# ku222/Attention-GAN

Hardware: AMD Instinct MI355X
Metric: train images/sec at 256×256 stage-3, batch 24/GPU, 1/2/4/8 MI355X (higher is better)
Workload: dtype f32; 1 GPU; full 3-stage AttnGAN 64->128->256 train step: G + 3xD updates + word attention + DAMSM words/sentence loss + KL + 4x fused Adam (BASELINE.json configs[2]); workload_key=full3, batch_per_gpu=24, global_batch=24, gf_dim=32, df_dim=64, emb_dim=256, seq_len=10, text_encoder=bypassed (frozen; N(0,1) embeddings), parallelism=dp1, discriminator_streams=3, launch=eager, gradient_exchange=none (one rank), losses_finite=True

## Files before the change

### attention-gan_amd/backend/functional.py

```python
from __future__ import annotations

import ctypes
import math
from ctypes import byref, c_void_p
from typing import Dict, Optional, Tuple

import contextlib
import os
import weakref

import torch
from torch import Tensor
from torch.autograd import Function
from torch.autograd.function import once_differentiable

from . import lib as L

_PRECISION = [L.PREC_F32]


def set_precision(p: int) -> None:
    if int(p) != _PRECISION[0]:
        for rng in _FLAT_RANGES:
            rng[3], rng[4] = [], None
# ... 35 lines not shown
def set_activation_storage(kind) -> None:
    dt = {None: L.DT_F32, "f32": L.DT_F32, "bf16": L.DT_BF16, "f16": L.DT_F16}[kind]
    _STORAGE[0] = dt


def get_activation_storage() -> int:
    dt = _STORAGE[0]
    if dt == L.DT_BF16 and _PRECISION[0] == L.PREC_BF16:
        return dt
    if dt == L.DT_F16 and _PRECISION[0] == L.PREC_F16:
        return dt
    return L.DT_F32


def _dt(t: Tensor) -> int:
    return L.DT_F32 if t.dtype == torch.float32 else _DT_OF[t.dtype]


def _act(t: Tensor, what: str) -> Tensor:
    if not t.is_cuda:
        raise L.AganError(f"{what}: tensor is on {t.device}; the AttnGAN HIP path runs on an MI355X only (no CPU fallback)")
    if t.dtype != torch.float32 and t.dtype not in _DT_OF:
        raise L.AganError(f"{what}: expected float32 / bfloat16 / float16, got {t.dtype}")
    return t.contiguous()


_DT_SUPPORT: dict = {}


def _gather_types(g: "L.ConvGeom", pe: int, x: Tensor, want_out: int):
    def ok(xin, out):
        if xin == L.DT_F32 and out == L.DT_F32:
            return True
        key = (g.B, g.Cin, g.IH, g.IW, g.Cout, g.OH, g.OW, g.R, g.S, g.OS, g.SY, g.DY, g.OY[0], g.OY[1], pe, xin, out)
        hit = _DT_SUPPORT.get(key)
        if hit is None:
            hit = _DT_SUPPORT[key] = bool(L.load().agan_conv_gather_dt_supported(byref(g), pe, xin, out))
        return hit
    outs = [want_out, L.DT_F32] if want_out != L.DT_F32 else [L.DT_F32]
    for out in outs:
        if ok(_dt(x), out):
            return x, out
    x = x.float()
    for out in outs:
        if ok(L.DT_F32, out):
            return x, out
    return x, L.DT_F32


def _ws(nbytes: int, like: Tensor) -> Tuple[Optional[Tensor], Optional[c_void_p]]:
    if nbytes <= 0:
        return None, None
    t = torch.empty(nbytes, dtype=torch.uint8, device=like.device)
    return t, c_void_p(t.data_ptr())


def grad_dst(param):
    return getattr(param, "_agan_grad_dst", None)


def _grad_out(dst, shape, like: Tensor):
    if dst is None:
        t = torch.empty(shape, dtype=torch.float32, device=like.device)
        return t, 0, t
    if dst.locked:
        raise L.AganError("a backward kernel is about to write into a flat gradient slice whose bucket is already being all-reduced: "
                          "call zero_grad() (and GradBuckets.arm()) before running another backward under data parallelism")
    view = dst.flat[dst.offset:dst.offset + dst.numel].view(shape)
    dst.edges += 1
    if dst.written:
        return view, 1, None
    dst.written = True
    return view, 0, view


class GradDst:
    __slots__ = ("flat", "offset", "numel", "written", "edges", "locked")

    def __init__(self, flat: Tensor, offset: int, numel: int):
        self.flat, self.offset, self.numel, self.written, self.edges, self.locked = flat, offset, numel, False, 0, False

    def reset(self) -> None:
        self.written, self.edges, self.locked = False, 0, False


def _geom(B, Cin, IH, IW, Cout, OH, OW, R, S, OS, SY, DY, OY) -> L.ConvGeom:
    g = L.ConvGeom()
    g.B, g.Cin, g.IH, g.IW, g.Cout, g.OH, g.OW = B, Cin, IH, IW, Cout, OH, OW
    g.R, g.S, g.OS, g.SY, g.DY = R, S, OS, SY, DY
    g.OY[0], g.OY[1] = OY
    return g


_GEOM_CACHE = {}


def conv_geoms(kind: str, B: int, Cin: int, H: int, W: int, Cout: int, k: int):
    key = (kind, B, Cin, H, W, Cout, k)
    hit = _GEOM_CACHE.get(key)
    if hit is not None:
        return hit
    if kind == "same":
        p = (k - 1) // 2
        out = (_geom(B, Cin, H, W, Cout, H, W, k, k, 1, 1, 1, (-p, -p)), L.PACK_FWD,
               _geom(B, Cout, H, W, Cin, H, W, k, k, 1, 1, 1, (-p, -p)), L.PACK_DGRAD_S1, (H, W))
    elif kind == "down":
        if k != 4 or H % 2 or W % 2:
            raise L.AganError(f"down conv needs k=4 and even H,W (got k={k}, {H}x{W})")
        out = (_geom(B, Cin, H, W, Cout, H // 2, W // 2, 4, 4, 1, 2, 1, (-1, -1)), L.PACK_FWD,
               _geom(B, Cout, H // 2, W // 2, Cin, H, W, 2, 2, 2, 1, -1, (0, 1)), L.PACK_DGRAD_4x4S2, (H // 2, W // 2))
    elif kind == "up":
        if k != 3:
            raise L.AganError("upsample conv needs k=3")
        out = (_geom(B, Cin, H, W, Cout, 2 * H, 2 * W, 2, 2, 2, 1, 1, (-1, 0)), L.PACK_UP_FWD,
               _geom(B, Cout, 2 * H, 2 * W, Cin, H, W, 4, 4, 1, 2, 1, (-1, -1)), L.PACK_UP_DGRAD, (2 * H, 2 * W))
    else:
        raise L.AganError(f"unknown conv kind {kind!r}")
    _GEOM_CACHE[key] = out
    return out


_WEIGHT_EPOCH = [0]
_FLAT_RANGES: list = []


def bump_weight_epoch() -> None:
    _WEIGHT_EPOCH[0] += 1


def register_flat(flat: Tensor) -> None:
    start = flat.data_ptr()
    end = start + flat.numel() * flat.element_size()
    top = max([r[2] for r in _FLAT_RANGES] + [0])
    _FLAT_RANGES[:] = [r for r in _FLAT_RANGES if r[1] <= start or r[0] >= end]
    _FLAT_RANGES.append([start, end, top + 1, [], None])


def unregister_flat(flat: Tensor) -> None:
    start = flat.data_ptr()
    _FLAT_RANGES[:] = [r for r in _FLAT_RANGES if r[0] != start]


def _flat_range(ptr: int):
    for r in _FLAT_RANGES:
        if r[0] <= ptr < r[1]:
            return r
    return None


_PACK_JOB_DTYPE = [("w", "<u8"), ("wk", "<u8"), ("mode", "<i4"), ("cout", "<i4"), ("cin", "<i4"), ("kh", "<i4"), ("kw", "<i4"),
                   ("first_block", "<i4")]


def _pack_table(rng, prec: int):
    import numpy as np
    entries = [e for e in rng[3] if e["prec"] == prec]
    if rng[4] is None:
        rng[4] = {}
    hit = rng[4].get(prec)
    if hit is None or hit[1] != len(entries):
        if torch.cuda.is_current_stream_capturing():
            raise L.AganError("packed-weight job table missing during HIP-graph capture: run a warm-up step and "
                              "build_pack_tables() first (GanTrainStep.capture does)")
        lib = L.load()
        jobs = np.zeros(len(entries), dtype=_PACK_JOB_DTYPE)
        first = 0
        for i, e in enumerate(entries):
            cout, cin, kh, kw = e["dims"]
            jobs[i] = (e["ptr"], e["wk"].data_ptr(), e["mode"], cout, cin, kh, kw, first)
            first += lib.agan_pack_job_blocks_prec(e["mode"], cout, cin, kh, kw, prec)
        table = torch.from_numpy(jobs.view(np.uint8).copy()).to(entries[0]["wk"].device)
        hit = rng[4][prec] = (table, len(entries), first)
    return hit


def build_pack_tables() -> None:
    for rng in _FLAT_RANGES:
        for prec in sorted({e["prec"] for e in rng[3]}):
            _pack_table(rng, prec)


def _repack_group(rng, prec: int) -> None:
    table, n, total = _pack_table(rng, prec)
    L.call("agan_pack_weights", _p(table), n, total, prec, _stream())
    for e in rng[3]:
        if e["prec"] == prec:
            e["cache"][e["key"]] = ((e["ptr"], e["tver"], _WEIGHT_EPOCH[0], rng[2]) + e["dims"], e["wk"], rng)


_EFF_PREC = {}


def effective_precision(g: L.ConvGeom) -> int:
    prec = _PRECISION[0]
    if prec == L.PREC_F32:
        return prec
    key = (prec, g.B, g.Cin, g.IH, g.IW, g.Cout, g.OH, g.OW, g.R, g.S, g.OS, g.SY, g.DY, g.OY[0], g.OY[1])
    hit = _EFF_PREC.get(key)
    if hit is None:
        hit = _EFF_PREC[key] = int(L.load().agan_conv_effective_prec(byref(g), prec))
    return hit


_EFF_WPREC = {}


def wgrad_effective_precision(g: L.ConvGeom, pack_mode: int) -> int:
    prec = _PRECISION[0]
    if prec == L.PREC_F32:
        return prec
    key = (prec, pack_mode, g.B, g.Cin, g.IH, g.IW, g.Cout, g.OH, g.OW, g.R, g.S, g.OS, g.SY, g.DY, g.OY[0], g.OY[1])
    hit = _EFF_WPREC.get(key)
    if hit is None:
        hit = _EFF_WPREC[key] = int(L.load().agan_conv_wgrad_effective_prec(byref(g), pack_mode, prec))
    return hit


def packed_weight(w: Tensor, mode: int, cache: Optional[dict] = None, prec: Optional[int] = None) -> Tensor:
    cout, cin, kh, kw = w.shape
    if prec is None:
        prec = _PRECISION[0]
    key = (mode, prec)
    hit = cache.get(key) if cache is not None else None
    ptr = w.data_ptr()
    rng = hit[2] if (hit is not None and hit[0][0] == ptr) else _flat_range(ptr)
    ver = (ptr, w._version, _WEIGHT_EPOCH[0], rng[2] if rng is not None else -1, cout, cin, kh, kw)
    if hit is not None and hit[0] == ver:
        return hit[1]
    if hit is not None and rng is not None and hit[0][:2] == ver[:2] and hit[0][4:] == ver[4:] \
            and any(e["cache"] is cache and e["key"] == key for e in rng[3]):
        _repack_group(rng, prec)
        hit = cache[key]
        if hit[0] == ver:
            return hit[1]
    n = L.load().agan_packed_weight_bytes(mode, cout, cin, kh, kw, prec)
    if n == 0:
        raise L.AganError(f"pack mode {mode} / precision {prec} does not take a {kh}x{kw} kernel")
    reuse = hit is not None and hit[1].numel() == n and hit[1].device == w.device
    wk = hit[1] if reuse else torch.empty(n, dtype=torch.uint8, device=w.device)
    L.call("agan_pack_weight", _p(w), _p(wk), mode, cout, cin, kh, kw, prec, _stream())
    if cache is not None:
        cache[key] = (ver, wk, rng)
        if rng is not None:
            ent = next((e for e in rng[3] if e["cache"] is cache and e["key"] == key), None)
            if ent is None:
                ent = {"cache": cache, "key": key}
                rng[3].append(ent)
            ent.update(ptr=ptr, tver=w._version, dims=(cout, cin, kh, kw), mode=mode, wk=wk, prec=prec)
            rng[4] = None
    return wk


_KTABLE_CACHE = {}


def ktable(g: L.ConvGeom, device) -> Tensor:
    key = (g.Cin, g.IH, g.IW, g.R, g.S, g.DY, str(device))
    t = _KTABLE_CACHE.get(key)
    if t is None:
        n = L.load().agan_conv_ktable_elems(byref(g))
        t = torch.empty(n, dtype=torch.int32, device=device)
        L.call("agan_conv_ktable", byref(g), _p(t), _stream())
        _KTABLE_CACHE[key] = t
    return t


_OBSERVER = [None]


def set_launch_observer(obs) -> None:
    _OBSERVER[0] = obs


_AMAX_REG: dict = {}
_AMAX_ARENA: dict = {}
_AMAX_WINDOW, _AMAX_WINDOWS = 1024, 4


def _needs_amax() -> bool:
    return _PRECISION[0] in (L.PREC_F16X3, L.PREC_BF16X6)


def amax_begin_step(device) -> None:
    if not _needs_amax():
        return
    ent = _AMAX_ARENA.get(device)
    if ent is None:
        ent = _AMAX_ARENA[device] = [torch.zeros(_AMAX_WINDOWS * _AMAX_WINDOW * L.AMAX_SLOT, dtype=torch.float32, device=device), -1, 0, 0]
    ent[1] = (ent[1] + 1) % _AMAX_WINDOWS
    lo = ent[1] * _AMAX_WINDOW * L.AMAX_SLOT
    ent[0][lo:lo + _AMAX_WINDOW * L.AMAX_SLOT].zero_()
    ent[2], ent[3] = ent[1] * _AMAX_WINDOW, (ent[1] + 1) * _AMAX_WINDOW


def _amax_new(device) -> Tensor:
    ent = _AMAX_ARENA.get(device)
    if ent is not None and ent[2] < ent[3]:
        i = ent[2]
        ent[2] += 1
        return ent[0][i * L.AMAX_SLOT:(i + 1) * L.AMAX_SLOT]
    return torch.zeros(L.AMAX_SLOT, dtype=torch.float32, device=device)


def _amax_put(t: Tensor, slot: Tensor) -> None:
    k = id(t)
    _AMAX_REG[k] = (weakref.ref(t, lambda _r, k=k: _AMAX_REG.pop(k, None)), slot)


def amax_of(t: Tensor) -> Tensor:
    e = _AMAX_REG.get(id(t))
    if e is not None and e[0]() is t:
        return e[1]
    slot = _amax_new(t.device)
    L.call("agan_absmax", _p(t), t.numel(), _p(slot), _stream())
    _amax_put(t, slot)
    return slot


_AMAX_FUSE_MIN = int(os.environ.get("AGAN_AMAX_FUSE_MIN", 1 << 22))


def _amax_out(t: Tensor) -> Optional[Tensor]:
    if not _needs_amax() or t.numel() < _AMAX_FUSE_MIN:
        return None
    slot = _amax_new(t.device)
    _amax_put(t, slot)
    return slot


def _gather(x: Tensor, wk: Tensor, bias: Optional[Tensor], g: L.ConvGeom, out: Tensor, kind: str = "", phase: str = "",
            act: int = 0, lrelu_mask: Optional[Tensor] = None, prec: int = L.PREC_F32, in_amax: Optional[Tensor] = None) -> None:
    lib = L.load()
    nbytes = lib.agan_conv_gather_ws_bytes(byref(g), prec)
    ws, wsp = _ws(nbytes, x)
    kt = ktable(g, x.device)
    obs = _OBSERVER[0]
    if obs is not None:
        obs.begin(kind, phase, g, x.element_size(), out.element_size())
    out_amax = _amax_out(out) if prec != L.PREC_F32 else None
    L.call("agan_conv_gather_dt", _p(x), _p(wk), _p(bias), _p(out), byref(g), _p(kt), prec, act, _p(lrelu_mask), wsp, nbytes,
           _stream(), _p(in_amax), _p(out_amax), _dt(x), _dt(out))
    if obs is not None:
        obs.end()


_SIDE_STREAMS: Dict[int, "torch.cuda.Stream"] = {}
_SIDE_DIRTY: Dict[int, bool] = {}
_WGRAD_SIDE = [False]


def set_wgrad_side_stream(flag: bool) -> bool:
    old = _WGRAD_SIDE[0]
    _WGRAD_SIDE[0] = bool(flag)
    return old


def wgrad_side_stream_enabled() -> bool:
    return _WGRAD_SIDE[0]


def join_all_side_streams(target) -> None:
    for key, side in _SIDE_STREAMS.items():
        if _SIDE_DIRTY.get(key):
            target.wait_stream(side)


def set_side_stream_for(stream, side) -> None:
    _SIDE_STREAMS[stream.cuda_stream] = side


def _fork_side_stream():
    cur = torch.cuda.current_stream()
    key = cur.cuda_stream
    side = _SIDE_STREAMS.get(key)
    if side is None:
        side = _SIDE_STREAMS[key] = torch.cuda.Stream(device=cur.device)
    side.wait_stream(cur)
    _SIDE_DIRTY[key] = True
    return side


def join_side_stream() -> None:
    if not torch.cuda.is_available():
        return
    cur = torch.cuda.current_stream()
    key = cur.cuda_stream
    if _SIDE_DIRTY.get(key):
        cur.wait_stream(_SIDE_STREAMS[key])
        _SIDE_DIRTY[key] = False


class ActHandoff:
    __slots__ = ("masked",)

    def __init__(self):
        self.masked = False


class _ConvFn(Function):
    @staticmethod
    def forward(ctx, x: Tensor, weight: Tensor, bias: Optional[Tensor], kind: str, cache: Optional[dict], wdst, bdst, act: int = 0,
                handoff_out: Optional[ActHandoff] = None, handoff_in: Optional[ActHandoff] = None):
        x = _act(x, "conv input")
        w = _dev(weight.detach(), "conv weight")
        B, Cin, H, W = x.shape
        Cout, Cin_w, kh, kw = w.shape
        if Cin != Cin_w or kh != kw:
            raise L.AganError(f"conv: input has {Cin} channels, weight {tuple(w.shape)}")
        gf, pf, gd, pd, (OH, OW) = conv_geoms(kind, B, Cin, H, W, Cout, kh)
        pe = effective_precision(gf)
        x, odt = _gather_types(gf, pe, x, get_activation_storage())
        out = torch.empty((B, Cout, OH, OW), dtype=_TORCH_OF[odt], device=x.device)
        b = _dev(bias.detach(), "conv bias") if bias is not None else None
        need_xs = pe == L.PREC_F16X3 or (ctx.needs_input_grad[1] and _needs_amax() and wgrad_effective_precision(gf, pf) == L.PREC_F16X3)
        xs = amax_of(x) if need_xs else None
        _gather(x, packed_weight(w, pf, cache, pe), b, gf, out, kind, "fwd", act, None, pe, xs)
        ctx.x_scale = xs
        if act == L.ACT_NONE:
            ctx.save_for_backward(x, w)
        else:
            ctx.save_for_backward(x, w, out)
        ctx.kind, ctx.has_bias, ctx.cache, ctx.wdst, ctx.bdst, ctx.act = kind, bias is not None, cache, wdst, bdst, act
        ctx.handoff_out = handoff_out if act != L.ACT_NONE else None
        ctx.handoff_in = handoff_in if (handoff_in is not None and Cin > 4) else None
        return out

    @staticmethod
    @once_differentiable
    def backward(ctx, dy: Tensor):
        x, w = ctx.saved_tensors[:2]
        dy = _act(dy, "conv grad")
        if ctx.act != L.ACT_NONE:
            if ctx.handoff_out is not None and ctx.handoff_out.masked:
                ctx.handoff_out.masked = False
            else:
                out = _dev(ctx.saved_tensors[2], "conv output")
                dy = _dev(dy, "conv grad")
                dz = torch.empty_like(dy)
                L.call("agan_act_bwd", _p(out), _p(dy), _p(dz), out.numel(), ctx.act, _stream())
                dy = dz
        B, Cin, H, W = x.shape
        Cout, _, kh, kw = w.shape
        gf, pf, gd, pd, _ = conv_geoms(ctx.kind, B, Cin, H, W, Cout, kh)
        dx = dw = db = None
        want_w, want_b = ctx.needs_input_grad[1], ctx.has_bias and ctx.needs_input_grad[2]
        pe_d = effective_precision(gd) if ctx.needs_input_grad[0] else L.PREC_F32
        pe_w = wgrad_effective_precision(gf, pf)
        scaled_w = want_w and pe_w == L.PREC_F16X3
        dys = amax_of(dy) if (pe_d == L.PREC_F16X3 or scaled_w) else None
        side = None
        if _WGRAD_SIDE[0] and want_w and ctx.wdst is not None and (not want_b or ctx.bdst is not None):
            kt = ktable(gf, x.device)
            side = _fork_side_stream()
            x.record_stream(side)
            dy.record_stream(side)
        with (torch.cuda.stream(side) if side is not None else contextlib.nullcontext()):
            if want_w:
                dwbuf, wacc, dw = _grad_out(ctx.wdst, w.shape, x)
                lib = L.load()
                nbytes = lib.agan_conv_wgrad_ws_bytes(byref(gf))
                ws, wsp = _ws(nbytes, x)
                kt = ktable(gf, x.device)
                obs = _OBSERVER[0]
                if obs is not None:
                    obs.begin(ctx.kind, "wgrad", gf, x.element_size(), dy.element_size())
                xs = None
                if scaled_w:
                    xs = ctx.x_scale if ctx.x_scale is not None else amax_of(x)
                xw, dyw = x, dy
                if (xw.dtype != torch.float32 or dyw.dtype != torch.float32) and not lib.agan_conv_wgrad_dt_supported(
                        byref(gf), pf, _PRECISION[0], _dt(xw), _dt(dyw)):
                    xw, dyw = xw.float(), dyw.float()
                L.call("agan_conv_wgrad_dt", _p(xw), _p(dyw), _p(dwbuf), byref(gf), _p(kt), pf, kh, kw, pe_w, wacc, wsp, nbytes,
                       _stream(), _p(xs), _p(dys if scaled_w else None), _dt(xw), _dt(dyw))
                if obs is not None:
                    obs.end()
            if want_b:
                dbbuf, bacc, db = _grad_out(ctx.bdst, (Cout,), x)
                L.call("agan_bias_grad", _p(_dev(dy, "conv grad")), _p(dbbuf), B, Cout, dy.shape[2] * dy.shape[3], bacc, _stream())
        if ctx.needs_input_grad[0]:
            dyg, ddt = _gather_types(gd, pe_d, dy, _dt(x))
            dx = torch.empty(x.shape, dtype=_TORCH_OF[ddt], device=x.device)
            mask = x if ctx.handoff_in is not None else None
            if mask is not None and mask.dtype != dx.dtype:
                mask = mask.to(dx.dtype)
            _gather(dyg, packed_weight(w, pd, ctx.cache, pe_d), None, gd, dx, ctx.kind, "dgrad", L.ACT_NONE, mask, pe_d,
                    dys if pe_d == L.PREC_F16X3 else None)
            if mask is not None:
                ctx.handoff_in.masked = True
        return dx, dw, db, None, None, None, None, None, None, None


_ANY_DESCS = {}


def conv_any_desc(B: int, Cin: int, H: int, W: int, Cout: int, k, stride, padding):
    key = (B, Cin, H, W, Cout, tuple(k), tuple(stride), tuple(padding))
    hit = _ANY_DESCS.get(key)
    if hit is not None:
        return hit
    (kh, kw), (sh, sw), (ph, pw) = k, stride, padding
    oh, ow = (H + 2 * ph - kh) // sh + 1, (W + 2 * pw - kw) // sw + 1
    d = L.Conv2dDesc(B, Cin, H, W, Cout, oh, ow, kh, kw, sh, sw, ph, pw, 0, Cin, 0, Cout)
    lib = L.load()
    if not lib.agan_conv2d_train_supported(byref(d)):
        raise L.AganError(f"conv k={k} s={stride} p={padding} on {Cin}x{H}x{W}: {lib.agan_last_error().decode()}")
    g = _geom(B, Cin, H, W, Cout, oh, ow, kh, kw, 1, sh, 1, (-ph, -pw))
    hit = _ANY_DESCS[key] = (d, g, tuple(lib.agan_conv2d_train_ws_bytes(byref(d), i) for i in range(3)))
    return hit


class _ConvAnyFn(Function):

    @staticmethod
    def forward(ctx, x: Tensor, weight: Tensor, bias: Optional[Tensor], stride, padding, wdst, bdst):
        ctx.x_dtype = x.dtype
        x = _dev(x, "conv input")
        w = _dev(weight.detach(), "conv weight")
        B, Cin, H, W = x.shape
        Cout, Cin_w, kh, kw = w.shape
        if Cin != Cin_w:
            raise L.AganError(f"conv: input has {Cin} channels, weight {tuple(w.shape)}")
        d, g, nbytes = conv_any_desc(B, Cin, H, W, Cout, (kh, kw), stride, padding)
        b = _dev(bias.detach(), "conv bias") if bias is not None else None
        out = torch.empty((B, Cout, d.OH, d.OW), dtype=torch.float32, device=x.device)
        ws, wsp = _ws(nbytes[0], x)
        obs = _OBSERVER[0]
        if obs is not None:
            obs.begin("any", "fwd", g, 4, 4)
        L.call("agan_conv2d_train_fwd", _p(x), _p(w), _p(b), _p(out), byref(d), wsp, nbytes[0], _stream())
        if obs is not None:
            obs.end()
        ctx.save_for_backward(x, w)
        ctx.stride, ctx.padding, ctx.has_bias, ctx.wdst, ctx.bdst = stride, padding, bias is not None, wdst, bdst
        return out

    @staticmethod
    @once_differentiable
    def backward(ctx, dy: Tensor):
        x, w = ctx.saved_tensors
        dy = _dev(dy, "conv grad")
        B, Cin, H, W = x.shape
        Cout, _, kh, kw = w.shape
        d, g, nbytes = conv_any_desc(B, Cin, H, W, Cout, (kh, kw), ctx.stride, ctx.padding)
        dx = dw = db = None
        want_w, want_b = ctx.needs_input_grad[1], ctx.has_bias and ctx.needs_input_grad[2]
        obs = _OBSERVER[0]
        side = None
        if _WGRAD_SIDE[0] and want_w and ctx.wdst is not None and (not want_b or ctx.bdst is not None):
            side = _fork_side_stream()
            x.record_stream(side)
            dy.record_stream(side)
        with (torch.cuda.stream(side) if side is not None else contextlib.nullcontext()):
            if want_w:
                dwbuf, wacc, dw = _grad_out(ctx.wdst, w.shape, x)
                ws, wsp = _ws(nbytes[2], x)
                if obs is not None:
                    obs.begin("any", "wgrad", g, 4, 4)
                L.call("agan_conv2d_train_wgrad", _p(x), _p(dy), _p(dwbuf), byref(d), wacc, wsp, nbytes[2], _stream())
                if obs is not None:
                    obs.end()
            if want_b:
                dbbuf, bacc, db = _grad_out(ctx.bdst, (Cout,), x)
                L.call("agan_bias_grad", _p(dy), _p(dbbuf), B, Cout, dy.shape[2] * dy.shape[3], bacc, _stream())
        if ctx.needs_input_grad[0]:
            dx = torch.empty(x.shape, dtype=torch.float32, device=x.device)
            ws, wsp = _ws(nbytes[1], x)
            if obs is not None:
                obs.begin("any", "dgrad", g, 4, 4)
            L.call("agan_conv2d_train_dgrad", _p(dy), _p(w), _p(dx), byref(d), 0, wsp, nbytes[1], _stream())
            if obs is not None:
                obs.end()
            if ctx.x_dtype != torch.float32:
                dx = dx.to(ctx.x_dtype)
        return dx, dw, db, None, None, None, None


def conv_fuses_activation(act: int, cout: int, kind: Optional[str] = None) -> bool:
    return act == L.ACT_LRELU and cout > 4 and kind != "any"


def conv2d(x: Tensor, weight: Tensor, bias: Optional[Tensor] = None, kind: str = "same", cache: Optional[dict] = None,
           wdst=None, bdst=None, act: int = 0, handoff_out: Optional[ActHandoff] = None,
           handoff_in: Optional[ActHandoff] = None, stride=(1, 1), padding=(0, 0)) -> Tensor:
    if kind == "any":
        if act != L.ACT_NONE or handoff_out is not None:
            raise L.AganError("conv2d(kind='any') has no fused activation: run HF.activation / HF.bn_act after it")
        return _ConvAnyFn.apply(x, weight, bias, tuple(stride), tuple(padding), wdst, bdst)
    return _ConvFn.apply(x, weight, bias, kind, cache, wdst, bdst, act, handoff_out, handoff_in)


def linear(x: Tensor, weight: Tensor, bias: Optional[Tensor] = None, cache: Optional[dict] = None, wdst=None, bdst=None) -> Tensor:
    B, Cin = x.shape
    y = _ConvFn.apply(x.reshape(B, Cin, 1, 1), weight.view(weight.shape[0], Cin, 1, 1), bias, "same", cache, wdst, bdst)
    return y.view(B, weight.shape[0])


_BN_GROUPS = [1]


@contextlib.contextmanager
def bn_groups(groups: int):
    old = _BN_GROUPS[0]
    _BN_GROUPS[0] = int(groups)
    try:
        yield
    finally:
        _BN_GROUPS[0] = old


class _BnActFn(Function):
    @staticmethod
    def forward(ctx, x, gamma, beta, residual, running_mean, running_var, nbt, training, act, eps, momentum, gdst, bdst, groups):
        x = _act(x, "bn input")
        shape = x.shape
        B, C = shape[0], shape[1]
        HW = x.numel() // (B * C)
        if not training:
            groups = 1
        if B % groups:
            raise L.AganError(f"BatchNorm: batch {B} does not split into {groups} groups")
        Bg = B // groups
        g, b = _dev(gamma.detach(), "bn weight"), _dev(beta.detach(), "bn bias")
        lib = L.load()
        co = C // 2 if act == L.ACT_GLU else C
        odt = get_activation_storage() if HW > 1 else L.DT_F32
        if x.dtype != torch.float32 and _dt(x) != odt:
            x = x.float()
        xdt = _dt(x)
        out = torch.empty((B, co) + tuple(shape[2:]), dtype=_TORCH_OF[odt], device=x.device)
        res = _act(residual, "bn residual") if residual is not None else None
        if res is not None and res.dtype != out.dtype:
            res = res.to(out.dtype)
        if training:
            mean = torch.empty((groups, C), dtype=torch.float32, device=x.device)
            invstd = torch.empty_like(mean)
            nbytes = lib.agan_bn_train_fwd_ws_bytes(Bg, C, HW)
            ws, wsp = _ws(nbytes, x)
            L.call("agan_bn_train_fwd_dt", _p(x), _p(g), _p(b), _p(res), _p(out), _p(mean), _p(invstd), _p(running_mean),
                   _p(running_var), _p(nbt), B, C, HW, float(eps), float(momentum), act, groups, wsp, nbytes, _stream(),
# ... 1191 lines not shown
```

### attention-gan_amd/backend/lib.py

```python
from __future__ import annotations

import ctypes
import os
from ctypes import POINTER, Structure, c_char_p, c_double, c_float, c_int, c_int32, c_int64, c_size_t, c_void_p

_HERE = os.path.dirname(os.path.abspath(__file__))
LIB_PATH = os.environ.get("AGAN_LIB") or os.path.join(os.path.dirname(_HERE), "csrc", "libagan_hip.so")

PREC_F32, PREC_BF16, PREC_BF16X3, PREC_F16, PREC_BF16X6, PREC_F16X3 = 0, 1, 2, 3, 4, 5
PRECISIONS = {"f32": PREC_F32, "bf16": PREC_BF16, "bf16x3": PREC_BF16X3, "f16": PREC_F16, "bf16x6": PREC_BF16X6, "f16x3": PREC_F16X3}
PACK_FWD, PACK_DGRAD_S1, PACK_DGRAD_4x4S2, PACK_UP_FWD, PACK_UP_DGRAD, PACK_DGRAD_3x3S2 = 0, 1, 2, 3, 4, 5
ACT_NONE, ACT_GLU, ACT_LRELU, ACT_TANH, ACT_SIGMOID, ACT_RELU = 0, 1, 2, 3, 4, 5
COMM_ID_BYTES = 128
DT_F32, DT_BF16, DT_F16 = 0, 1, 2
AMAX_SLOT = 256
EINVAL, EWORKSPACE = -1, -2
DIFFAUG_COLOR, DIFFAUG_TRANSLATION, DIFFAUG_CUTOUT = 1, 2, 4
ADA_STATE_WORDS, ADA_P_WORD, ADA_SLOT_WORD = 16, 4, 8
ABI_VERSION = 101


class ConvGeom(Structure):
    _fields_ = [("B", c_int32), ("Cin", c_int32), ("IH", c_int32), ("IW", c_int32),
                ("Cout", c_int32), ("OH", c_int32), ("OW", c_int32), ("R", c_int32), ("S", c_int32),
                ("OS", c_int32), ("SY", c_int32), ("DY", c_int32), ("OY", c_int32 * 2)]


class Conv2dDesc(Structure):
    _fields_ = [(n, c_int32) for n in ("B", "Cin", "IH", "IW", "Cout", "OH", "OW", "KH", "KW", "SH", "SW", "PH", "PW",
                                       "in_c0", "in_ctot", "out_c0", "out_ctot")]


class ImagePlane(Structure):
    _fields_ = [("src", c_void_p), ("dst", c_void_p), ("H", c_int32), ("W", c_int32)]


_P = c_void_p
_SIGNATURES = {
    "agan_version": (c_int, []),
    "agan_last_error": (c_char_p, []),
    "agan_packed_weight_bytes": (c_size_t, [c_int] * 6),
    "agan_timer_create": (c_int, [_P]),
    "agan_timer_destroy": (c_int, [_P]),
    "agan_timer_arm": (c_int, [_P, _P]),
    "agan_timer_elapsed_ms": (c_int, [_P, _P, _P]),
    "agan_timer_last_kernel": (c_int, [_P, c_size_t]),
    "agan_timer_last_split": (c_int, []),
    "agan_comm_unique_id": (c_int, [_P]),
    "agan_comm_init": (c_int, [_P, c_int, c_int, _P]),
    "agan_comm_destroy": (c_int, [_P]),
    "agan_allreduce_bucket": (c_int, [_P, _P, c_size_t, _P]),
    "agan_allreduce_chunk_elems": (c_size_t, [c_size_t, c_int]),
    "agan_allreduce_scratch_bytes": (c_size_t, [c_size_t, c_int, c_int]),
    "agan_allreduce_bucket_dt": (c_int, [_P, _P, c_size_t, c_int, _P, c_size_t, _P]),
    "agan_exchange_wire_elems": (c_size_t, [c_size_t, c_int]),
    "agan_exchange_pack_bf16": (c_int, [_P, _P, c_size_t, c_size_t, _P]),
    "agan_exchange_sum_bf16": (c_int, [_P, c_int, c_size_t, _P, _P]),
    "agan_exchange_unpack_bf16": (c_int, [_P, _P, c_size_t, _P]),
    "agan_pack_job_blocks": (c_int, [c_int] * 5),
    "agan_pack_job_blocks_prec": (c_int, [c_int] * 6),
    "agan_pack_weights": (c_int, [_P, c_int, c_int, c_int, _P]),
    "agan_pack_weight": (c_int, [_P, _P, c_int, c_int, c_int, c_int, c_int, c_int, _P]),
    "agan_conv_effective_prec": (c_int, [POINTER(ConvGeom), c_int]),
    "agan_conv_wgrad_effective_prec": (c_int, [POINTER(ConvGeom), c_int, c_int]),
    "agan_conv_executed_fraction": (c_double, [POINTER(ConvGeom), c_int, c_int, c_int]),
    "agan_conv_gather_ws_bytes": (c_size_t, [POINTER(ConvGeom), c_int]),
    "agan_conv_ktable_elems": (c_size_t, [POINTER(ConvGeom)]),
    "agan_conv_ktable": (c_int, [POINTER(ConvGeom), _P, _P]),
    "agan_conv_gather": (c_int, [_P, _P, _P, _P, POINTER(ConvGeom), _P, c_int, c_int, _P, _P, c_size_t, _P, _P, _P]),
    "agan_conv_gather_dt": (c_int, [_P, _P, _P, _P, POINTER(ConvGeom), _P, c_int, c_int, _P, _P, c_size_t, _P, _P, _P, c_int, c_int]),
    "agan_conv_gather_dt_supported": (c_int, [POINTER(ConvGeom), c_int, c_int, c_int]),
    "agan_conv_wgrad_dt_supported": (c_int, [POINTER(ConvGeom), c_int, c_int, c_int, c_int]),
    "agan_conv_wgrad_dt": (c_int, [_P, _P, _P, POINTER(ConvGeom), _P, c_int, c_int, c_int, c_int, c_int, _P, c_size_t, _P, _P, _P, c_int, c_int]),
    "agan_bn_stats_dt": (c_int, [_P, c_int, c_int, c_int, c_float, _P, _P, _P, _P, _P, c_float, _P, c_size_t, _P, c_int]),
    "agan_bn_act_fwd_dt": (c_int, [_P, _P, _P, _P, _P, _P, _P, c_int, c_int, c_int, c_int, _P, _P, c_int, c_int]),
    "agan_bn_train_fwd_dt": (c_int, [_P, _P, _P, _P, _P, _P, _P, _P, _P, _P, c_int, c_int, c_int, c_float, c_float, c_int, c_int, _P, c_size_t, _P, _P, c_int, c_int]),
    "agan_bn_act_bwd_dt": (c_int, [_P, _P, _P, _P, _P, _P, _P, _P, _P, c_int, c_int, c_int, c_int, c_int, c_int, _P, c_size_t, _P, _P, c_int, c_int]),
    "agan_absmax": (c_int, [_P, c_size_t, _P, _P]),
    "agan_conv_wgrad_ws_bytes": (c_size_t, [POINTER(ConvGeom)]),
    "agan_conv_wgrad": (c_int, [_P, _P, _P, POINTER(ConvGeom), _P, c_int, c_int, c_int, c_int, c_int, _P, c_size_t, _P, _P, _P]),
    "agan_bias_grad": (c_int, [_P, _P, c_int, c_int, c_int, c_int, _P]),
    "agan_bn_stats_ws_bytes": (c_size_t, [c_int, c_int, c_int]),
    "agan_bn_stats": (c_int, [_P, c_int, c_int, c_int, c_float, _P, _P, _P, _P, _P, c_float, _P, c_size_t, _P]),
    "agan_bn_train_fwd_ws_bytes": (c_size_t, [c_int, c_int, c_int]),
    "agan_bn_train_fwd": (c_int, [_P] * 10 + [c_int, c_int, c_int, c_float, c_float, c_int, c_int, _P, c_size_t, _P, _P]),
    "agan_bn_act_fwd": (c_int, [_P, _P, _P, _P, _P, _P, _P, c_int, c_int, c_int, c_int, _P, _P]),
    "agan_bn_act_bwd_ws_bytes": (c_size_t, [c_int, c_int, c_int]),
    "agan_bn_act_bwd": (c_int, [_P] * 9 + [c_int, c_int, c_int, c_int, c_int, c_int, _P, c_size_t, _P, _P]),
    "agan_act_fwd": (c_int, [_P, _P, c_size_t, c_int, _P]),
    "agan_act_bwd": (c_int, [_P, _P, _P, c_size_t, c_int, _P]),
    "agan_glu_fwd": (c_int, [_P, _P, c_int, c_int, c_int, _P]),
    "agan_glu_bwd": (c_int, [_P, _P, _P, c_int, c_int, c_int, _P]),
    "agan_bn_last_launch": (c_int, [_P, c_int]),
    "agan_attn_fwd": (c_int, [_P, _P, _P, _P, c_float, _P, _P, _P, c_int, c_int, c_int, c_int, c_int, _P]),
    "agan_attn_bwd_ws_bytes": (c_size_t, [c_int, c_int, c_int, c_int]),
    "agan_attn_bwd": (c_int, [_P] * 7 + [c_float, _P, _P, _P, c_int, c_int, c_int, c_int, c_int, c_int, _P, c_size_t, _P]),
    "agan_attn_fwd_dt": (c_int, [_P, _P, _P, _P, c_float, _P, _P, _P, c_int, c_int, c_int, c_int, c_int, _P, c_int]),
    "agan_attn_bwd_dt": (c_int, [_P] * 7 + [c_float, _P, _P, _P, c_int, c_int, c_int, c_int, c_int, c_int, _P, c_size_t, _P, c_int]),
    "agan_func_attention_fwd": (c_int, [_P, _P, c_float, c_float, _P, _P, c_int, c_int, c_int, c_int, _P]),
    "agan_func_attention_bwd": (c_int, [_P, _P, _P, _P, c_float, c_float, _P, _P, c_int, c_int, c_int, c_int, _P]),
    "agan_words_loss_save_elems": (c_size_t, [c_int, c_int, c_int, c_int]),
    "agan_words_loss_fwd": (c_int, [_P, _P, _P, _P, _P, c_float, c_float, c_float, c_float, _P, _P, _P, _P, c_int, c_int, c_int, c_int, _P]),
    "agan_words_loss_bwd_ws_bytes": (c_size_t, [c_int, c_int, c_int, c_int]),
    "agan_words_loss_bwd": (c_int, [_P, _P, _P, _P, _P, c_float, c_float, c_float, c_float, _P, _P, c_int, c_int, c_int, c_int, _P, c_size_t, _P]),
    "agan_sent_loss_fwd": (c_int, [_P, _P, _P, _P, c_float, c_float, c_float, _P, _P, c_int, c_int, _P]),
    "agan_sent_loss_bwd": (c_int, [_P, _P, _P, _P, c_float, c_float, c_float, _P, _P, c_int, c_int, _P]),
    "agan_disc_loss": (c_int, [_P, _P, _P, _P, _P, c_int, _P]),
    "agan_gen_loss": (c_int, [_P, _P, _P, c_int, _P]),
    "agan_kl_loss": (c_int, [_P, _P, _P, _P, _P, c_int, _P]),
    "agan_reparam_fwd": (c_int, [_P, _P, _P, _P, c_int, _P]),
    "agan_reparam_bwd": (c_int, [_P, _P, _P, _P, _P, c_int, _P]),
    "agan_conv2d_pack_mode": (c_int, [POINTER(Conv2dDesc), c_int]),
    "agan_conv2d_effective_prec": (c_int, [POINTER(Conv2dDesc), c_int]),
    "agan_conv2d_ws_bytes": (c_size_t, [POINTER(Conv2dDesc), c_int]),
    "agan_conv2d_ktable_elems": (c_size_t, [POINTER(Conv2dDesc), c_int]),
    "agan_conv2d_ktable": (c_int, [POINTER(Conv2dDesc), c_int, _P, _P]),
    "agan_conv2d_fwd": (c_int, [_P, _P, _P, _P, POINTER(Conv2dDesc), _P, c_int, _P, c_size_t, _P]),
    "agan_conv2d_dgrad": (c_int, [_P, _P, _P, POINTER(Conv2dDesc), _P, _P, c_int, _P, c_size_t, _P]),
    "agan_conv2d_train_supported": (c_int, [POINTER(Conv2dDesc)]),
    "agan_conv2d_train_slabs": (c_int, [POINTER(Conv2dDesc)]),
    "agan_conv2d_train_ws_bytes": (c_size_t, [POINTER(Conv2dDesc), c_int]),
    "agan_conv2d_train_fwd": (c_int, [_P, _P, _P, _P, POINTER(Conv2dDesc), _P, c_size_t, _P]),
    "agan_conv2d_train_dgrad": (c_int, [_P, _P, _P, POINTER(Conv2dDesc), c_int, _P, c_size_t, _P]),
    "agan_conv2d_train_wgrad": (c_int, [_P, _P, _P, POINTER(Conv2dDesc), c_int, _P, c_size_t, _P]),
    "agan_maxpool3s2_fwd": (c_int, [_P, _P, _P] + [c_int] * 6 + [_P]),
    "agan_maxpool3s2_bwd": (c_int, [_P, _P, _P, _P] + [c_int] * 7 + [_P]),
    "agan_avgpool3s1_fwd": (c_int, [_P, _P] + [c_int] * 4 + [_P]),
    "agan_avgpool3s1_bwd": (c_int, [_P, _P, _P] + [c_int] * 5 + [_P]),
    "agan_global_avgpool_fwd": (c_int, [_P, _P] + [c_int] * 3 + [_P]),
    "agan_global_avgpool_bwd": (c_int, [_P, _P, _P] + [c_int] * 4 + [_P]),
    "agan_resize_bilinear_fwd": (c_int, [_P, _P] + [c_int] * 6 + [_P]),
    "agan_resize_bilinear_bwd": (c_int, [_P, _P] + [c_int] * 6 + [_P]),
    "agan_relu_bwd": (c_int, [_P, _P, _P, c_size_t, c_int, _P]),
    "agan_bn_relu_slice_fwd_ws_bytes": (c_size_t, [c_int] * 3),
    "agan_bn_relu_slice_fwd": (c_int, [_P] * 4 + [c_int] * 2 + [_P] * 5 + [c_int] * 3 + [c_float] * 2 + [_P, c_size_t, _P]),
    "agan_bn_slice_bwd_ws_bytes": (c_size_t, [c_int] * 3),
    "agan_bn_slice_bwd": (c_int, [_P, _P, c_int, c_int, _P, _P, _P, _P] + [c_int] * 3 + [_P, c_size_t, _P]),
    "agan_embedding_fwd": (c_int, [_P, c_int, _P, _P] + [c_int] * 4 + [_P]),
    "agan_embedding_bwd": (c_int, [_P, c_int, _P, _P] + [c_int] * 4 + [_P]),
    "agan_lstm_fwd": (c_int, [_P] * 11 + [c_int] * 4 + [_P]),
    "agan_lstm_bwd": (c_int, [_P] * 9 + [c_int] * 4 + [_P]),
    "agan_lstm_wgrad": (c_int, [_P] * 5 + [c_int] * 4 + [_P]),
    "agan_image_prep": (c_int, [POINTER(ImagePlane), c_int, _P, _P, c_int, c_int, c_int, _P]),
    "agan_kmeans_assign_ws_bytes": (c_size_t, [c_int] * 3),
    "agan_kmeans_assign": (c_int, [_P] * 6 + [c_int] * 3 + [_P, c_size_t, _P]),
    "agan_kmeans_update_ws_bytes": (c_size_t, [c_int] * 3),
    "agan_kmeans_update": (c_int, [_P] * 4 + [c_int] * 3 + [_P, c_size_t, _P]),
    "agan_moments_update_ws_bytes": (c_size_t, [c_int] * 2),
    "agan_moments_update": (c_int, [_P, c_int, c_int, _P, _P, _P, c_size_t, _P]),
    "agan_moments_finish": (c_int, [_P, _P, c_int64, c_int, _P, _P, _P]),
    "agan_retrieval_rank": (c_int, [_P, _P, _P] + [c_int] * 4 + [_P, _P, _P]),
    "agan_diffaug_ws_bytes": (c_size_t, [c_int] * 4),
    "agan_diffaug_fwd": (c_int, [_P, _P, c_int, c_int, _P, c_int, _P, c_int, c_int, c_int, _P, c_size_t, _P]),
    "agan_diffaug_bwd": (c_int, [_P, _P, c_int, _P, c_int, c_int, c_int, c_int, _P, c_size_t, _P]),
    "agan_diffaug_gated_fwd": (c_int, [_P, _P, c_int, c_int, _P, _P, _P, c_int, _P, c_int, c_int, c_int, _P, c_size_t, _P]),
    "agan_diffaug_gated_bwd": (c_int, [_P, _P, _P, _P, c_int, _P, c_int, c_int, c_int, c_int, _P, c_size_t, _P]),
    "agan_ada_observe": (c_int, [_P, c_int, c_float, _P, _P]),
    "agan_ada_update": (c_int, [_P, c_int, c_int, c_double, c_double, c_double, _P]),
    "agan_ema_plan": (c_int, [_P, c_int]),
    "agan_ema_update": (c_int, [_P, c_int, c_int, _P, c_double, c_int, _P]),
    "agan_adam_step": (c_int, [_P, _P, _P, _P, c_size_t, _P, c_double, c_double, c_double, c_double, c_float, _P]),
    "agan_knn_radius_ws_bytes": (c_size_t, [c_int] * 3),
    "agan_knn_radius": (c_int, [_P, c_int, c_int, c_int, _P, _P, c_size_t, _P]),
    "agan_manifold_scan_ws_bytes": (c_size_t, [c_int] * 3),
    "agan_manifold_scan": (c_int, [_P, _P, _P] + [c_int] * 3 + [_P, _P, _P, _P, c_size_t, _P]),
    "agan_poly_kernel_sum_ws_bytes": (c_size_t, [c_int] * 3),
    "agan_poly_kernel_sum": (c_int, [_P, _P] + [c_int] * 4 + [_P, _P, c_size_t, _P]),
}

EXPORTED_SYMBOLS = tuple(_SIGNATURES)

_lib = None


class AganError(RuntimeError):
    pass


def load():
    global _lib
    if _lib is not None:
        return _lib
    if not os.path.exists(LIB_PATH):
        raise AganError(f"{LIB_PATH} not found: build it with `python -c 'import __graft_entry__ as g; g.build()'` "
                        f"(or `make -C attention-gan_amd/csrc`). There is no CPU fallback.")
    lib = ctypes.CDLL(LIB_PATH)
    for name, (res, args) in _SIGNATURES.items():
        fn = getattr(lib, name)
        fn.restype, fn.argtypes = res, args
    if lib.agan_version() != ABI_VERSION:
        raise AganError(f"{LIB_PATH} reports C-ABI version {lib.agan_version()}, this binding is written against {ABI_VERSION} "
                        f"(include/agan.h: argument lists differ between versions) -- rebuild with `make -C attention-gan_amd/csrc`")
    _lib = lib
    return lib


def check(code: int, what: str = "") -> None:
    if code != 0:
        msg = load().agan_last_error()
        raise AganError(f"{what or 'agan'} failed ({code}): {msg.decode() if msg else ''}")


def call(name: str, *args) -> None:
    check(getattr(load(), name)(*args), name)
```

### attention-gan_amd/csrc/conv.hip

```cpp
#include "conv_common.h"

#include <cxxabi.h>
#include <cstdlib>


using namespace agan;

using namespace agan::conv;

namespace {

__global__ __launch_bounds__(256) void ktable_kernel(int2* __restrict__ tab, int n, int K, int RS, int S, int IHW, int IW, int DY) {
    const int k = blockIdx.x * 256 + threadIdx.x;
    if (k >= n) return;
    int2 a, b;
    if (k < K) {
        const int c = k / RS, rs = k - c * RS, r = rs / S, q = rs - r * S;
        const int dy = r * DY, dx = q * DY;
        a.x = c * IHW + dy * IW + dx;
        a.y = (dy & 0xFFFF) | (dx << 16);
        b.x = c * IHW * 4;
        b.y = rs * kTapRowBytes;
    } else {
        a.x = 0;
// ... 505 lines not shown
#pragma unroll
        for (int t = 0; t < TI; ++t) av[0][t] = Xs[buf][wi * (BI / 2) + t * 32 + pl][half];
#pragma unroll
        for (int t = 0; t < TJ; ++t) bv[0][t] = Ys[buf][wj * (BJ / 2) + t * 32 + pl][half];
#pragma unroll
        for (int pp = 0; pp < BP; pp += 2) {
            const int c = (pp >> 1) & 1, q = pp >> 1;
            if (pp + 2 < BP) {
#pragma unroll
                for (int t = 0; t < TI; ++t) av[c ^ 1][t] = Xs[buf][wi * (BI / 2) + t * 32 + pl][pp + 2 + half];
#pragma unroll
                for (int t = 0; t < TJ; ++t) bv[c ^ 1][t] = Ys[buf][wj * (BJ / 2) + t * 32 + pl][pp + 2 + half];
            }
#pragma unroll
            for (int a = 0; a < TJ; ++a)
#pragma unroll
                for (int b = 0; b < TI; ++b)
                    acc[a][b] = __builtin_amdgcn_mfma_f32_32x32x2f32(bv[c][a], av[c][b], acc[a][b], 0, 0, 0);
#pragma unroll
            for (int it = q * L / NS; it < (q + 1) * L / NS; ++it) {
                if (it < XR) {
                    if (do_store) Xs[buf ^ 1][wave * (BI / 4) + 2 * it + half][pl] = xreg[PN][it];
                    if (do_load) xreg[PC][it] = buf_load(rx, xo[it]);
                } else {
                    const int jj = it - XR;
                    if (do_store) Ys[buf ^ 1][wave * (BJ / 4) + 2 * jj + half][pl] = yreg[PN][jj];
                    if (do_load) yreg[PC][jj] = buf_load(rdy, doff + ynoff[jj]);
                }
            }
        }
        __syncthreads();
    };

    fill_offsets(0);
    fill_offsets(1);
    __syncthreads();
    if (npt > 0) load_tile(S0{}, 0);
    if (npt > 1) load_tile(S1{}, 1);
    __syncthreads();
    fill_offsets(2);
    if (npt > 0) store_tile(S0{}, 0);
    __syncthreads();
    int pt = 0;
    for (; pt + 3 < npt; pt += 2) {
        step(std::true_type{}, S0{}, S1{}, pt, 0);
        step(std::true_type{}, S1{}, S0{}, pt + 1, 1);
    }
    for (; pt < npt; pt += 2) {
        step(std::false_type{}, S0{}, S1{}, pt, 0);
        if (pt + 1 < npt) step(std::false_type{}, S1{}, S0{}, pt + 1, 1);
    }

    float* o = dst + (size_t)split * slab + (size_t)cls * g.Cout * g.K;
    const __amdgpu_buffer_rsrc_t ro = make_rsrc(o, (size_t)g.Cout * g.K * sizeof(float));
#pragma unroll
    for (int tj = 0; tj < TJ; ++tj)
#pragma unroll
        for (int ti = 0; ti < TI; ++ti) {
            const int i = i0 + wi * (BI / 2) + ti * 32 + pl;
#pragma unroll
            for (int r = 0; r < 16; ++r) {
                const int n = j0 + wj * (BJ / 2) + tj * 32 + (r & 3) + 8 * (r >> 2) + 4 * half;
                const unsigned off = ((i < g.K) & (n < g.Cout)) ? (unsigned)(n * g.K + i) * 4u : kOOB;
                float v = acc[tj][ti][r];
                if (accumulate) v += buf_load(ro, off);
                buf_store(ro, off, v);
            }
        }
}

__device__ __forceinline__ void pack_fwd_tile(const float* __restrict__ w, float* __restrict__ wk, int cout, int K, int Nld, int bx, int by,
                                              float (*tile)[65]) {
    const int k0 = bx * 64, n0 = by * 64;
    const int tx = threadIdx.x & 63, ty = threadIdx.x >> 6;
    float v[16];
#pragma unroll
    for (int j = 0; j < 16; ++j) {
        const int n = n0 + ty + j * 4, k = k0 + tx;
        v[j] = (n < cout && k < K) ? w[(size_t)n * K + k] : 0.f;
    }
#pragma unroll
    for (int j = 0; j < 16; ++j) tile[ty + j * 4][tx] = v[j];
    __syncthreads();
#pragma unroll
    for (int j = 0; j < 16; ++j) {
        const int k = k0 + ty + j * 4, n = n0 + tx;
        if (k < K && n < Nld) wk[(size_t)k * Nld + n] = tile[tx][ty + j * 4];
    }
}
__global__ __launch_bounds__(256) void pack_fwd_tiled_kernel(const float* __restrict__ w, float* __restrict__ wk, int cout, int K, int Nld) {
    __shared__ float tile[64][65];
    pack_fwd_tile(w, wk, cout, K, Nld, blockIdx.x, blockIdx.y, tile);
}

constexpr int kPackCo = 4;
constexpr int kPackSlab = 64 * 16 + 64;
template <int MODE>
__device__ __forceinline__ void pack_dgrad_tile(const float* __restrict__ w, float* __restrict__ wk, int cout, int cin, int kh, int kw, int Nld,
                                                int cog, int cblk, float* sl , bool zero_pad) {
    const int T = kh * kw;
    const int c0 = cblk * 64;
    const int nc = min(64, cin - c0);
#pragma unroll
    for (int q = 0; q < kPackCo; ++q) {
        const int co = cog * kPackCo + q;
        if (co < cout) {
            const float* src = w + ((size_t)co * cin + c0) * T;
            for (int i = threadIdx.x; i < nc * T; i += 256) sl[q * kPackSlab + (i / T) * (T + 1) + (i % T)] = src[i];
        }
    }
    __syncthreads();
    const int cend = (zero_pad && c0 + 64 >= cin) ? Nld - c0 : nc;
#pragma unroll
    for (int q = 0; q < kPackCo; ++q) {
        const int co = cog * kPackCo + q;
        if (co >= cout) break;
        const float* s1 = sl + q * kPackSlab;
        if (MODE == AGAN_PACK_DGRAD_S1) {
            for (int i = threadIdx.x; i < T * 64; i += 256) {
                const int t = i / 64, c = i - t * 64;
                if (c < cend) wk[((size_t)co * T + t) * Nld + c0 + c] = c < nc ? s1[c * (T + 1) + (T - 1 - t)] : 0.f;
            }
        } else {
            const int K = cout * 4;
            for (int i = threadIdx.x; i < 16 * 64; i += 256) {
                const int qq = i / 64, c = i - qq * 64;
                const int cls = qq >> 2, r = (qq >> 1) & 1, sx = qq & 1, py = cls >> 1, px = cls & 1;
                const int th = ((py + 1) & 1) + 2 * r, tw = ((px + 1) & 1) + 2 * sx;
                if (c < cend) wk[((size_t)cls * K + co * 4 + r * 2 + sx) * Nld + c0 + c] = c < nc ? s1[c * 17 + th * 4 + tw] : 0.f;
            }
        }
    }
}
template <int MODE>
__global__ __launch_bounds__(256) void pack_dgrad_tiled_kernel(const float* __restrict__ w, float* __restrict__ wk, int cout, int cin,
                                                               int kh, int kw, int Nld) {
    __shared__ float sl[kPackCo * kPackSlab];
    pack_dgrad_tile<MODE>(w, wk, cout, cin, kh, kw, Nld, blockIdx.x, blockIdx.y, sl, false);
}

__global__ __launch_bounds__(256) void pack_weight_kernel(const float* __restrict__ w, float* __restrict__ wk, int mode,
                                                          int cout, int cin, int kh, int kw, int K, int Nld, int ncls) {
    const size_t total = (size_t)ncls * K * Nld;
    for (size_t e = (size_t)blockIdx.x * blockDim.x + threadIdx.x; e < total; e += (size_t)gridDim.x * blockDim.x) {
        const int n = (int)(e % Nld);
        const size_t t = e / Nld;
        const int k = (int)(t % K), cls = (int)(t / K);
        wk[e] = packed_weight_value(w, mode, cls, k, n, cout, cin, kh, kw);
    }
}

__host__ __device__ inline int pack_job_blocks(int mode, int cout, int cin, int kh, int kw) {
    int ncls, K, N;
    if (pack_dims(mode, cout, cin, kh, kw, ncls, K, N)) return 0;
    const int Nld = ((N + 31) / 32 * 32);
    if (mode == AGAN_PACK_FWD) return cdiv(K, 64) * cdiv(Nld, 64);
    if ((mode == AGAN_PACK_DGRAD_S1 && kh * kw <= 16) || mode == AGAN_PACK_DGRAD_4x4S2) return cdiv(cout, kPackCo) * cdiv(cin, 64);
    const size_t total = (size_t)ncls * K * Nld;
    return (int)(total / 1024 < 1 ? 1 : (total / 1024 > 2048 ? 2048 : total / 1024));
}

__global__ __launch_bounds__(256) void pack_jobs_kernel(const agan_pack_job* __restrict__ jobs, int njobs) {
    __shared__ float buf[kPackCo * kPackSlab > 64 * 65 ? kPackCo * kPackSlab : 64 * 65];
    __shared__ int which;
    const int b = blockIdx.x;
    for (int t = threadIdx.x; t < njobs; t += 256) {
        const int lo = jobs[t].first_block, hi = t + 1 < njobs ? jobs[t + 1].first_block : 0x7fffffff;
        if (b >= lo && b < hi) which = t;
    }
    __syncthreads();
    const agan_pack_job j = jobs[which];
    const int local = b - j.first_block;
    float* wk = static_cast<float*>(j.wk);
    int ncls, K, N;
    pack_dims(j.mode, j.cout, j.cin, j.kh, j.kw, ncls, K, N);
    const int Nld = ((N + 31) / 32 * 32);
    if (j.mode == AGAN_PACK_FWD) {
        const int kt = cdiv(K, 64);
        pack_fwd_tile(j.w, wk, j.cout, K, Nld, local % kt, local / kt, reinterpret_cast<float (*)[65]>(buf));
    } else if (j.mode == AGAN_PACK_DGRAD_S1 && j.kh * j.kw <= 16) {
        const int cg = cdiv(j.cout, kPackCo);
        pack_dgrad_tile<AGAN_PACK_DGRAD_S1>(j.w, wk, j.cout, j.cin, j.kh, j.kw, Nld, local % cg, local / cg, buf, true);
    } else if (j.mode == AGAN_PACK_DGRAD_4x4S2) {
        const int cg = cdiv(j.cout, kPackCo);
        pack_dgrad_tile<AGAN_PACK_DGRAD_4x4S2>(j.w, wk, j.cout, j.cin, j.kh, j.kw, Nld, local % cg, local / cg, buf, true);
    } else {
        const int nb = pack_job_blocks(j.mode, j.cout, j.cin, j.kh, j.kw);
        const size_t total = (size_t)ncls * K * Nld;
        for (size_t e = (size_t)local * 256 + threadIdx.x; e < total; e += (size_t)nb * 256) {
            const int n = (int)(e % Nld);
            const size_t t = e / Nld;
            wk[e] = packed_weight_value(j.w, j.mode, (int)(t / K), (int)(t % K), n, j.cout, j.cin, j.kh, j.kw);
        }
    }
}

__global__ __launch_bounds__(256) void unpack_wgrad_up_kernel(const float* __restrict__ dwk, float* __restrict__ dw, int cout, int cin,
                                                              int accumulate) {
    const int K = cin * 4;
    const size_t total = (size_t)cout * cin * 9;
    for (size_t e = (size_t)blockIdx.x * blockDim.x + threadIdx.x; e < total; e += (size_t)gridDim.x * blockDim.x) {
        const int ab = (int)(e % 9), a = ab / 3, b = ab - a * 3;
        const size_t t = e / 9;
        const int ci = (int)(t % cin), co = (int)(t / cin);
        float v = 0.f;
        for (int py = 0; py < 2; ++py)
            for (int r = 0; r < 2; ++r) {
                int rl, rh;
                up_fwd_taps(py, r, rl, rh);
                if (a < rl || a > rh) continue;
                for (int px = 0; px < 2; ++px)
                    for (int q = 0; q < 2; ++q) {
                        int sl, sh;
                        up_fwd_taps(px, q, sl, sh);
                        if (b < sl || b > sh) continue;
                        v += dwk[((size_t)(py * 2 + px) * cout + co) * K + (ci * 4 + r * 2 + q)];
                    }
            }
        dw[e] = accumulate ? dw[e] + v : v;
    }
}

__global__ __launch_bounds__(256) void bias_grad_kernel(const float* __restrict__ dy, float* __restrict__ db, int B, int C,
                                                        int HW, int accumulate) {
    __shared__ float red[4];
    const int c = blockIdx.x;
    float s = 0.f;
    for (int b = 0; b < B; ++b) {
        const float* p = dy + ((size_t)b * C + c) * HW;
        for (int i = threadIdx.x; i < HW; i += 256) s += p[i];
    }
    s = block_sum<256>(s, red);
    if (threadIdx.x == 0) db[c] = accumulate ? db[c] + s : s;
}

}

static thread_local hipEvent_t g_timer_start = nullptr, g_timer_stop = nullptr;
static thread_local const void* g_timed_kernel = nullptr;
static thread_local int g_timed_split = 0;
namespace agan { namespace conv { thread_local const void* g_noted_kernel = nullptr; } }
static inline void timer_begin(hipStream_t st) {
    if (g_timer_start) (void)hipEventRecord(g_timer_start, st);
}
static inline void timer_end(hipStream_t st, int split) {
    if (g_timer_stop) {
        (void)hipEventRecord(g_timer_stop, st);
        g_timed_kernel = agan::conv::g_noted_kernel;
        g_timed_split = split;
    }
    g_timer_start = g_timer_stop = nullptr;
}
namespace agan { namespace conv {
void timed_begin(hipStream_t st) { timer_begin(st); }
void timed_end(hipStream_t st, int split) { timer_end(st, split); }
} }

static bool dt16(int dt) { return dt == AGAN_DT_BF16 || dt == AGAN_DT_F16; }
static int mode_dtype(int mode) { return mode == AGAN_PREC_BF16 ? AGAN_DT_BF16 : (mode == AGAN_PREC_F16 ? AGAN_DT_F16 : AGAN_DT_F32); }

enum class GatherPath { none, p16, patch, winograd, small_n, direct };
struct GatherRoute {
    int mode = AGAN_PREC_F32;
    GatherPath path = GatherPath::none;
    P16Plan p16{};
    PatchPlan pp{};
    PatchGather patch{};
    WinoPlan wino{};
    GatherPlan direct{};
    size_t ws_bytes = 0;
    int split = 1;
};

static GatherRoute route_gather(const agan_conv_geom* gg, int prec, int in_dtype, int out_dtype, bool epilogue) {
    GatherRoute r;
    auto take = [&r](GatherPath path, size_t ws_bytes, int split) {
        r.path = path;
        r.ws_bytes = ws_bytes;
        r.split = split;
        return r;
    };
    if (check_geom(gg)) return r;
    const Geom g = make_geom(gg);
    if (prec_planes(prec) > 0 && patch_supported(g)) r.mode = prec;
    const bool f32io = in_dtype == AGAN_DT_F32 && out_dtype == AGAN_DT_F32;
    if (const int want = mode_dtype(r.mode)) {
        if ((in_dtype == AGAN_DT_F32 || in_dtype == want) && (out_dtype == AGAN_DT_F32 || out_dtype == want)) {
            r.p16 = plan_p16(g, in_dtype != AGAN_DT_F32);
            if (r.p16.ok) return take(GatherPath::p16, r.p16.ws_bytes, r.p16.ksplit);
        }
    }
    if (r.mode != AGAN_PREC_F32) {
        if (!f32io) return r;
        r.pp = make_patch_plan(g);
        r.patch = plan_patch_gather(g, r.pp);
        return take(GatherPath::patch, r.patch.ws_bytes, r.patch.ksplit);
    }
    if (f32io && !epilogue) {
        r.wino = plan_wino(g);
        if (r.wino.ok) return take(GatherPath::winograd, r.wino.ws_bytes, r.wino.ksplit);
    }
    if (small_n_gather_supported(g)) {
        const bool linear = g.RS == 1 && g.IH == 1 && g.IW == 1;
        if ((in_dtype == AGAN_DT_F32 || (dt16(in_dtype) && !linear)) && out_dtype == AGAN_DT_F32) return take(GatherPath::small_n, 0, 1);
        return r;
    }
    if (in_dtype == AGAN_DT_F32 && (out_dtype == AGAN_DT_F32 || dt16(out_dtype))) {
        r.direct = plan_gather(g, AGAN_PREC_F32);
        return take(GatherPath::direct, r.direct.ws_bytes, r.direct.ksplit);
    }
    return r;
}

enum class WgradPath { none, winograd, rows, patch, small_n, direct };
struct WgradRoute {
    int mode = AGAN_PREC_F32;
    WgradPath path = WgradPath::none;
    WinoWgradPlan wino{};
    RowsPlan rows{};
    PatchPlan pp{};
    PatchWgrad patch{};
    SmallWgradPlan small{};
    WgradPlan direct{};
    size_t ws_bytes = 0;
    int split = 1;
};

static WgradRoute route_wgrad(const agan_conv_geom* gg, int pack_mode, int prec, int x_dtype, int dy_dtype) {
    WgradRoute r;
    auto take = [&r](WgradPath path, size_t ws_bytes, int split) {
        r.path = path;
        r.ws_bytes = ws_bytes;
        r.split = split;
        return r;
    };
    if (check_geom(gg)) return r;
    const Geom g = make_geom(gg);
    const bool up = pack_mode == AGAN_PACK_UP_FWD, x16 = x_dtype != AGAN_DT_F32, y16 = dy_dtype != AGAN_DT_F32;
    if (prec_planes(prec) > 0 && patch_supported(g)) {
        r.mode = prec;
        if (prec == AGAN_PREC_BF16X6) r.mode = AGAN_PREC_F16X3;
        if (up && !plan_rows_wgrad(g, r.mode, false, false, true).ok) r.mode = AGAN_PREC_F32;
    }
    if (x16 || y16) {
        const int want = mode_dtype(r.mode);
        const bool ok = r.mode == AGAN_PREC_F32
                            ? pack_mode == AGAN_PACK_FWD && small_n_wgrad_supported(g) && dt16(x_dtype) && !y16
                            : want != AGAN_DT_F32 && (!x16 || x_dtype == want) && (!y16 || dy_dtype == want);
        if (!ok) return r;
    }
    if (r.mode == AGAN_PREC_F32 && !up && !x16 && !y16) {
        r.wino = plan_wino_wgrad(g);
        if (r.wino.ok) return take(WgradPath::winograd, r.wino.ws_bytes, r.wino.psplit);
    }
    if (!(r.mode == AGAN_PREC_F32 && small_n_wgrad_supported(g))) {
        r.rows = plan_rows_wgrad(g, r.mode, x16, y16, up);
        if (r.rows.ok) return take(WgradPath::rows, r.rows.ws_bytes, r.rows.psplit);
    }
    if (r.mode != AGAN_PREC_F32) {
        r.pp = make_patch_plan(g);
        r.patch = plan_patch_wgrad(g, r.pp, r.mode);
        return take(WgradPath::patch, r.patch.ws_bytes, r.patch.psplit);
    }
    if (!up && small_n_wgrad_supported(g)) {
        r.small = plan_wgrad_small_n(g);
        return take(WgradPath::small_n, r.small.ws_bytes, r.small.nchunk);
    }
    if (!x16 && !y16) {
        r.direct = plan_wgrad(g, up);
        return take(WgradPath::direct, r.direct.ws_bytes, r.direct.psplit);
    }
    return r;
}

static int check_ws(const char* who, size_t need, const void* ws, size_t ws_bytes) {
    if (need > ws_bytes || (need && !ws)) {
        set_error("%s: workspace %zu < %zu", who, ws_bytes, need);
        return AGAN_EWORKSPACE;
    }
    return AGAN_OK;
}

template <class Launch>
static int launch_main(hipStream_t st, int split, const char* what, Launch&& launch) {
    timer_begin(st);
    launch();
    timer_end(st, split);
    return check_launch(what);
}

extern "C" {

int agan_timer_last_kernel(char* name, size_t capacity) {
    AGAN_REQUIRE(name && capacity > 1, "timer_last_kernel: bad argument");
    name[0] = 0;
    if (!g_timed_kernel) return AGAN_OK;
    const char* mangled = hipKernelNameRefByPtr(g_timed_kernel, nullptr);
    if (!mangled) return AGAN_OK;
    int status = 0;
    char* dem = abi::__cxa_demangle(mangled, nullptr, nullptr, &status);
    const char* src = (status == 0 && dem) ? dem : mangled;
    strncpy(name, src, capacity - 1);
    name[capacity - 1] = 0;
    free(dem);
    return AGAN_OK;
}

int agan_timer_last_split(void) { return g_timed_kernel ? g_timed_split : 0; }

int agan_timer_create(void** event) {
    AGAN_REQUIRE(event != nullptr, "timer_create: null pointer");
    hipEvent_t e;
    if (hipEventCreate(&e) != hipSuccess) {
        set_error("timer_create: hipEventCreate failed");
        return AGAN_ELAUNCH;
    }
    *event = e;
    return AGAN_OK;
}
int agan_timer_destroy(void* event) { return (event && hipEventDestroy(static_cast<hipEvent_t>(event)) != hipSuccess) ? AGAN_ELAUNCH : AGAN_OK; }
int agan_timer_arm(void* start, void* stop) {
    g_timer_start = static_cast<hipEvent_t>(start);
    g_timer_stop = static_cast<hipEvent_t>(stop);
    return AGAN_OK;
}
int agan_timer_elapsed_ms(void* start, void* stop, float* ms) {
    AGAN_REQUIRE(start && stop && ms, "timer_elapsed_ms: null pointer");
    if (hipEventElapsedTime(ms, static_cast<hipEvent_t>(start), static_cast<hipEvent_t>(stop)) != hipSuccess) {
        set_error("timer_elapsed_ms: events not complete");
        return AGAN_ELAUNCH;
    }
    return AGAN_OK;
}

size_t agan_packed_weight_bytes(int mode, int cout, int cin, int kh, int kw, int prec) {
    int ncls, K, N;
    if (pack_dims(mode, cout, cin, kh, kw, ncls, K, N)) return 0;
    if (prec == AGAN_PREC_F32) return (size_t)ncls * K * ((N + 31) / 32 * 32) * sizeof(float);
    if (mode == AGAN_PACK_DGRAD_3x3S2) return 0;
    if (prec_planes(prec) > 0) return patch_packed_weight_bytes(mode, cout, cin, kh, kw, prec);
    return 0;
}

int agan_pack_weight(const float* w, void* wkv, int mode, int cout, int cin, int kh, int kw, int prec, void* stream) {
    int ncls, K, N;
    AGAN_REQUIRE(w && wkv, "pack_weight: null pointer");
    AGAN_REQUIRE(prec == AGAN_PREC_F32 || prec_planes(prec) > 0, "pack_weight: unknown precision mode %d", prec);
    if (prec != AGAN_PREC_F32) {
        AGAN_REQUIRE(mode != AGAN_PACK_DGRAD_3x3S2, "pack_weight: AGAN_PACK_DGRAD_3x3S2 has an fp32 layout only");
        AGAN_REQUIRE(pack_dims(mode, cout, cin, kh, kw, ncls, K, N) == 0, "pack_weight: mode %d does not take %dx%d", mode, kh, kw);
        return pack_weight_patch(w, wkv, mode, cout, cin, kh, kw, prec, as_stream(stream));
    }
    float* wk = static_cast<float*>(wkv);
    AGAN_REQUIRE(pack_dims(mode, cout, cin, kh, kw, ncls, K, N) == 0, "pack_weight: mode %d does not take %dx%d", mode, kh, kw);
    const int Nld = ((N + 31) / 32 * 32);
    const size_t total = (size_t)ncls * K * Nld;
    const int blocks = (int)std::min<size_t>(cdivz(total, 256), 8192);
    hipStream_t pst = as_stream(stream);
    if (mode == AGAN_PACK_FWD) {
        AGAN_LAUNCH(pack_fwd_tiled_kernel, dim3(cdiv(K, 64), cdiv(Nld, 64)), dim3(256), 0, pst, w, wk, cout, K, Nld);
        return check_launch("pack_weight/fwd");
    }
    if ((mode == AGAN_PACK_DGRAD_S1 && kh * kw <= 16) || mode == AGAN_PACK_DGRAD_4x4S2) {
        if (Nld != cin) (void)hipMemsetAsync(wk, 0, total * sizeof(float), pst);
        dim3 grid(cdiv(cout, kPackCo), cdiv(cin, 64));
        if (mode == AGAN_PACK_DGRAD_S1) AGAN_LAUNCH((pack_dgrad_tiled_kernel<AGAN_PACK_DGRAD_S1>), grid, dim3(256), 0, pst, w, wk, cout, cin, kh, kw, Nld);
        else AGAN_LAUNCH((pack_dgrad_tiled_kernel<AGAN_PACK_DGRAD_4x4S2>), grid, dim3(256), 0, pst, w, wk, cout, cin, kh, kw, Nld);
        return check_launch("pack_weight/dgrad");
    }
    AGAN_LAUNCH(pack_weight_kernel, dim3(blocks), dim3(256), 0, as_stream(stream), w, wk, mode, cout, cin, kh, kw, K,
                       Nld, ncls);
    return check_launch("pack_weight");
}

int agan_pack_job_blocks(int mode, int cout, int cin, int kh, int kw) { return pack_job_blocks(mode, cout, cin, kh, kw); }
int agan_pack_job_blocks_prec(int mode, int cout, int cin, int kh, int kw, int prec) {
    return prec == AGAN_PREC_F32 ? pack_job_blocks(mode, cout, cin, kh, kw) : (prec_planes(prec) > 0 ? pack_job_blocks_patch(mode, cout, cin, kh, kw) : 0);
}

int agan_pack_weights(const agan_pack_job* jobs, int njobs, int total_blocks, int prec, void* stream) {
    AGAN_REQUIRE(jobs && njobs > 0 && total_blocks > 0, "pack_weights: empty job list");
    AGAN_REQUIRE(prec == AGAN_PREC_F32 || prec_planes(prec) > 0, "pack_weights: unknown precision mode %d", prec);
    if (prec != AGAN_PREC_F32) return pack_weights_patch(jobs, njobs, total_blocks, prec, as_stream(stream));
    AGAN_LAUNCH(pack_jobs_kernel, dim3(total_blocks), dim3(256), 0, as_stream(stream), jobs, njobs);
    return check_launch("pack_weights");
}

int agan_conv_effective_prec(const agan_conv_geom* g, int prec) { return route_gather(g, prec, AGAN_DT_F32, AGAN_DT_F32, false).mode; }

int agan_conv_wgrad_effective_prec(const agan_conv_geom* g, int pack_mode, int prec) {
    return route_wgrad(g, pack_mode, prec, AGAN_DT_F32, AGAN_DT_F32).mode;
}

double agan_conv_executed_fraction(const agan_conv_geom* g, int prec, int wgrad, int plain_epilogue) {
    if (prec != AGAN_PREC_F32) return 1.0;
    if (wgrad)
        return route_wgrad(g, AGAN_PACK_FWD, prec, AGAN_DT_F32, AGAN_DT_F32).path == WgradPath::winograd ? 16.0 / 36.0 : 1.0;
    const GatherRoute r = route_gather(g, prec, AGAN_DT_F32, AGAN_DT_F32, !plain_epilogue);
    if (r.path != GatherPath::winograd) return 1.0;
    switch (r.wino.kind) {
    case WinoKind::conv4x4_s2: return 36.0 / 64.0;
    case WinoKind::dgrad2x2_class: return 9.0 / 16.0;
    case WinoKind::conv3x3:
    case WinoKind::conv3x3_half: break;
    }
    return 16.0 / 36.0;
}

static const int kDtypes[] = {AGAN_DT_F32, AGAN_DT_BF16, AGAN_DT_F16};

size_t agan_conv_gather_ws_bytes(const agan_conv_geom* g, int prec) {
    size_t a = 0;
    for (int in_dtype : kDtypes)
        for (int out_dtype : kDtypes)
            for (int epilogue = 0; epilogue < 2; ++epilogue) a = std::max(a, route_gather(g, prec, in_dtype, out_dtype, epilogue != 0).ws_bytes);
    return a;
}

size_t agan_conv_ktable_elems(const agan_conv_geom* g) {
    if (check_geom(g)) return 0;
    return (size_t)ktable_entries(g->Cin * g->R * g->S) * 4;
}

int agan_conv_ktable(const agan_conv_geom* gg, int32_t* table, void* stream) {
    if (int e = check_geom(gg)) return e;
    AGAN_REQUIRE(table != nullptr, "conv_ktable: null pointer");
    const Geom g = make_geom(gg);
    const int n = ktable_entries(g.K);
    AGAN_LAUNCH(ktable_kernel, dim3(cdiv(n, 256)), dim3(256), 0, as_stream(stream), reinterpret_cast<int2*>(table), n, g.K, g.RS,
                       g.S, g.IH * g.IW, g.IW, g.DY);
    return check_launch("conv_ktable");
}

int agan_conv_gather_dt_supported(const agan_conv_geom* gg, int prec, int in_dtype, int out_dtype) {
    return route_gather(gg, prec, in_dtype, out_dtype, false).path != GatherPath::none ? 1 : 0;
}

int agan_conv_gather_dt(const void* in_v, const void* wkv, const float* bias, void* out_v, const agan_conv_geom* gg, const int32_t* ktable,
                        int prec, int act, const void* lrelu_mask_v, void* ws, size_t ws_bytes, void* stream, const float* in_scale,
                        float* out_amax, int in_dtype, int out_dtype) {
    if (int e = check_geom(gg)) return e;
    AGAN_REQUIRE(in_v && wkv && out_v && ktable, "conv_gather: null pointer");
    AGAN_REQUIRE(act == AGAN_ACT_NONE || (act == AGAN_ACT_LRELU && gg->Cout > 4),
                 "conv_gather: fused activation %d not available for this call (MFMA paths, LeakyReLU only)", act);
    AGAN_REQUIRE(!lrelu_mask_v || (gg->Cout > 4 && act == AGAN_ACT_NONE),
                 "conv_gather: the LeakyReLU-derivative mask needs an MFMA path and no other activation");
    AGAN_REQUIRE(prec == AGAN_PREC_F32 || prec_planes(prec) > 0, "conv_gather: unknown precision mode %d", prec);
    const GatherRoute r = route_gather(gg, prec, in_dtype, out_dtype, bias || act != AGAN_ACT_NONE || lrelu_mask_v);
    AGAN_REQUIRE(r.mode == prec,
                 "conv_gather: precision mode %d does not take this geometry (agan_conv_effective_prec says which one does)", prec);
    AGAN_REQUIRE(r.path != GatherPath::none,
                 "conv_gather: 16-bit activation storage (%d -> %d) is not available for this geometry / precision %d "
                 "(agan_conv_gather_dt_supported)", in_dtype, out_dtype, prec);
    AGAN_REQUIRE(prec != AGAN_PREC_F16X3 || in_scale != nullptr, "conv_gather: AGAN_PREC_F16X3 needs the operand's agan_absmax_scale pair");
    if (int e = check_ws("conv_gather", r.ws_bytes, ws, ws_bytes)) return e;
    const Geom g = make_geom(gg);
    hipStream_t st = as_stream(stream);
    const float* in = static_cast<const float*>(in_v);
    const float* wk = static_cast<const float*>(wkv);
    const float* lrelu_mask = static_cast<const float*>(lrelu_mask_v);
    void* dst = r.split > 1 ? ws : out_v;
    const float* slabs = static_cast<const float*>(ws);
    size_t slab = 0;
    float* sum_amax = nullptr;
    int e = AGAN_OK;
    switch (r.path) {
        case GatherPath::p16:
            slab = r.p16.slab;
            e = launch_main(st, r.split, "conv_gather/p16", [&] {
                launch_p16_gather(in_v, wkv, bias, dst, g, r.p16, prec, act, lrelu_mask_v, st, in_dtype != AGAN_DT_F32, out_dtype != AGAN_DT_F32);
            });
            break;
        case GatherPath::patch:
            slab = r.patch.slab;
            sum_amax = out_amax;
            e = launch_main(st, r.split, "conv_gather/patch", [&] {
                launch_patch_gather(in, wkv, bias, static_cast<float*>(dst), g, r.pp, r.patch, prec, act, lrelu_mask, st, in_scale, out_amax);
            });
            break;
        case GatherPath::winograd:
            slab = r.wino.slab;
            slabs = reinterpret_cast<const float*>(static_cast<const char*>(ws) + r.wino.u_bytes);
            e = launch_main(st, r.split, "conv_gather/winograd", [&] { launch_wino(in, wk, static_cast<float*>(out_v), g, r.wino, ws, st); });
            break;
        case GatherPath::small_n:
            e = launch_main(st, r.split, "conv_gather/small_n", [&] { launch_gather_small_n(in_v, wk, bias, static_cast<float*>(out_v), g, st, in_dtype); });
            break;
        default: {
            const GatherPlan& p = r.direct;
            slab = p.slab;
            const int2* ktab = reinterpret_cast<const int2*>(ktable);
            e = launch_main(st, r.split, "conv_gather", [&] { launch_gather(in, wk, bias, dst, ktab, g, p, act, lrelu_mask_v, st, out_dtype); });
        }
    }
    if (e || r.split == 1) return e;
    launch_sum_slabs(slabs, r.split, (size_t)g.B * g.Cout * g.OH * g.OW, slab, bias, g.Cout, g.OH * g.OW, out_v, 0, act, lrelu_mask_v, sum_amax, st,
                     out_dtype);
    return check_launch("conv_gather/sum_slabs");
}

int agan_conv_gather(const float* in, const void* wkv, const float* bias, float* out, const agan_conv_geom* gg, const int32_t* ktable,
                     int prec, int act, const float* lrelu_mask, void* ws, size_t ws_bytes, void* stream, const float* in_scale,
                     float* out_amax) {
    return agan_conv_gather_dt(in, wkv, bias, out, gg, ktable, prec, act, lrelu_mask, ws, ws_bytes, stream, in_scale, out_amax,
                               AGAN_DT_F32, AGAN_DT_F32);
}

static const int kPrecs[] = {AGAN_PREC_F32, AGAN_PREC_BF16, AGAN_PREC_BF16X3, AGAN_PREC_F16, AGAN_PREC_BF16X6, AGAN_PREC_F16X3};

size_t agan_conv_wgrad_ws_bytes(const agan_conv_geom* g) {
    if (check_geom(g)) return 0;
    const int pack_mode = g->OS == 2 ? AGAN_PACK_UP_FWD : AGAN_PACK_FWD;
    size_t a = 0;
    for (int prec : kPrecs)
        for (int x_dtype : kDtypes)
            for (int dy_dtype : kDtypes) a = std::max(a, route_wgrad(g, pack_mode, prec, x_dtype, dy_dtype).ws_bytes);
    return a;
}

int agan_conv_wgrad_dt_supported(const agan_conv_geom* gg, int pack_mode, int prec, int x_dtype, int dy_dtype) {
    return route_wgrad(gg, pack_mode, prec, x_dtype, dy_dtype).path != WgradPath::none ? 1 : 0;
}

int agan_conv_wgrad(const float* x, const float* dy, float* dw, const agan_conv_geom* gg, const int32_t* ktable, int pack_mode,
                    int kh, int kw, int prec, int accumulate, void* ws, size_t ws_bytes, void* stream, const float* x_scale,
                    const float* dy_scale) {
    return agan_conv_wgrad_dt(x, dy, dw, gg, ktable, pack_mode, kh, kw, prec, accumulate, ws, ws_bytes, stream, x_scale, dy_scale,
                              AGAN_DT_F32, AGAN_DT_F32);
}

int agan_conv_wgrad_dt(const void* x_v, const void* dy_v, float* dw, const agan_conv_geom* gg, const int32_t* ktable, int pack_mode,
                       int kh, int kw, int prec, int accumulate, void* ws, size_t ws_bytes, void* stream, const float* x_scale,
                       const float* dy_scale, int x_dtype, int dy_dtype) {
    const WgradRoute r = route_wgrad(gg, pack_mode, prec, x_dtype, dy_dtype);
    AGAN_REQUIRE(r.path != WgradPath::none,
                 "conv_wgrad: 16-bit activation storage (%d, %d) is not available for this geometry / precision %d", x_dtype, dy_dtype, prec);
    AGAN_REQUIRE(x_v && dy_v && dw && ktable, "conv_wgrad: null pointer");
    AGAN_REQUIRE(prec == AGAN_PREC_F32 || prec_planes(prec) > 0, "conv_wgrad: unknown precision mode %d", prec);
    AGAN_REQUIRE(pack_mode == AGAN_PACK_FWD || pack_mode == AGAN_PACK_UP_FWD, "conv_wgrad: pack mode %d is not a forward mode", pack_mode);
    const Geom g = make_geom(gg);
    const bool up = pack_mode == AGAN_PACK_UP_FWD;
    AGAN_REQUIRE(1LL * g.B * g.Cin * g.IH * g.IW < (1LL << 29) && 1LL * g.B * g.Cout * g.OH * g.OW < (1LL << 29),
                 "conv_wgrad: tensor exceeds 2^29 elements");
    if (!up) AGAN_REQUIRE(g.R == kh && g.S == kw && g.OS == 1, "conv_wgrad: geometry is not a direct %dx%d conv", kh, kw);
    else AGAN_REQUIRE(g.R == 2 && g.S == 2 && g.OS == 2 && kh == 3 && kw == 3, "conv_wgrad: geometry is not the folded upsample conv");
    AGAN_REQUIRE(r.mode != AGAN_PREC_F16X3 || (x_scale && dy_scale),
                 "conv_wgrad: precision mode %d runs this weight gradient as AGAN_PREC_F16X3 (agan_conv_wgrad_effective_prec), which needs the "
                 "amax slots of x and dy (x_amax / dy_amax)", prec);
    if (int e = check_ws("conv_wgrad", r.ws_bytes, ws, ws_bytes)) return e;
    hipStream_t st = as_stream(stream);
    const float* x = static_cast<const float*>(x_v);
    const float* dy = static_cast<const float*>(dy_v);
    float* wsf = static_cast<float*>(ws);
    const bool x16 = x_dtype != AGAN_DT_F32, y16 = dy_dtype != AGAN_DT_F32;
    switch (r.path) {
        case WgradPath::winograd:
            if (int e = launch_main(st, r.split, "conv_wgrad/winograd", [&] { launch_wino_wgrad(x, dy, wsf, g, r.wino, st); })) return e;
            launch_wino_wgrad_sum(wsf, g, r.wino, dw, accumulate ? 1 : 0, st);
            return check_launch("conv_wgrad/winograd/sum");
        case WgradPath::rows:
        case WgradPath::patch: {
            const bool rows = r.path == WgradPath::rows;
            int e;
            if (rows) e = launch_main(st, r.split, "conv_wgrad/rows", [&] {
                launch_rows_wgrad(x_v, dy_v, wsf, g, r.rows, r.mode, st, x_scale, dy_scale, x16, y16);
            });
            else e = launch_main(st, r.split, "conv_wgrad/patch", [&] {
                launch_patch_wgrad(x_v, dy_v, wsf, g, r.pp, r.patch, r.mode, st, x_scale, dy_scale, x16, y16);
            });
            if (e) return e;
            const size_t slab = rows ? r.rows.slab : r.patch.slab;
            const int NPH = rows ? r.rows.NPH : r.pp.NPH, NT = rows ? r.rows.NT : r.pp.NT, Kp = rows ? r.rows.Kp : r.patch.Kp;
            const int ncls = rows ? 1 : r.patch.ncls;
            const bool unfold = up && !rows;
            float* reduced = r.split > 1 ? wsf + slab * r.split : wsf;
            const bool sum_first = unfold ? r.split > 1 : r.split > 4;
            if (sum_first) {
                launch_sum_slabs(wsf, r.split, (size_t)ncls * g.Cout * Kp, slab, nullptr, 1, 1, reduced, 0, AGAN_ACT_NONE, nullptr, nullptr, st);
                if (int e2 = check_launch("conv_wgrad/sum_slabs")) return e2;
            }
            if (unfold) launch_patch_wgrad_unpack(reduced, dw, g.Cout, g.Cin, kh, kw, up, r.pp, r.patch, accumulate, st);
            else launch_wgrad_sum_unpack(sum_first ? reduced : wsf, sum_first ? 1 : r.split, slab, dw, g.Cout, g.Cin, kh, kw, NPH, NT, Kp, accumulate, st);
            return check_launch("conv_wgrad/unpack");
        }
        case WgradPath::small_n: {
            if (int e = launch_main(st, r.split, "conv_wgrad/small_n", [&] { launch_wgrad_small_n(x_v, dy, wsf, g, r.small, st, x_dtype); })) return e;
            launch_sum_slabs(wsf, r.split, (size_t)g.Cout * g.K, r.small.slab, nullptr, 1, 1, dw, accumulate, AGAN_ACT_NONE, nullptr, nullptr, st);
            return check_launch("conv_wgrad/small_n/sum_slabs");
        }
        default: {
            const WgradPlan& p = r.direct;
            const int acc_in_kernel = (accumulate && !up && p.psplit == 1) ? 1 : 0;
            const bool via_sum = p.psplit > 1 || (accumulate && !up && !acc_in_kernel);
            float* reduced = up ? wsf + (p.psplit > 1 ? p.slab * p.psplit : 0) : dw;
            float* part = via_sum ? wsf : reduced;
            const int2* ktab = reinterpret_cast<const int2*>(ktable);
            dim3 grid(p.itiles, p.jtiles, p.ncls * p.psplit);
            const int e = launch_main(st, r.split, "conv_wgrad", [&] {
                with_bool(p.bi == 128, [&](auto I128) { with_bool(p.bj == 128, [&](auto J128) {
                    AGAN_LAUNCH((conv_wgrad_f32_kernel<I128() ? 128 : 64, J128() ? 128 : 64>), grid, dim3(256), 0, st, x, dy, part, ktab, g, p.psplit, p.pchunk,
                                p.slab, acc_in_kernel);
                }); });
            });
            if (e) return e;
            if (via_sum) {
                launch_sum_slabs(part, p.psplit, (size_t)p.ncls * g.Cout * g.K, p.slab, nullptr, 1, 1, reduced, (accumulate && !up) ? 1 : 0,
                                 AGAN_ACT_NONE, nullptr, nullptr, st);
                if (int e2 = check_launch("conv_wgrad/sum_slabs")) return e2;
            }
            if (up) {
                const size_t total = (size_t)g.Cout * g.Cin * 9;
                AGAN_LAUNCH(unpack_wgrad_up_kernel, dim3((unsigned)std::min<size_t>(cdivz(total, 256), 4096)), dim3(256), 0, st,
                            reduced, dw, g.Cout, g.Cin, accumulate);
                return check_launch("conv_wgrad/unpack");
            }
            return AGAN_OK;
        }
    }
}

int agan_bias_grad(const float* dy, float* dbias, int B, int C, int HW, int accumulate, void* stream) {
    AGAN_REQUIRE(dy && dbias && B > 0 && C > 0 && HW > 0, "bias_grad: bad argument");
    AGAN_LAUNCH(bias_grad_kernel, dim3(C), dim3(256), 0, as_stream(stream), dy, dbias, B, C, HW, accumulate);
    return check_launch("bias_grad");
}

static int conv2d_geom(const agan_conv2d_desc* d, int dgrad, Geom& g, int& pack_mode) {
    AGAN_REQUIRE(d != nullptr, "conv2d: null descriptor");
    AGAN_REQUIRE(d->B > 0 && d->Cin > 0 && d->IH > 0 && d->IW > 0 && d->Cout > 0 && d->OH > 0 && d->OW > 0, "conv2d: non-positive dimension");
    AGAN_REQUIRE(d->KH > 0 && d->KW > 0 && d->KH * d->KW <= kMaxTaps2d, "conv2d: %dx%d taps unsupported (at most %d)", d->KH, d->KW, kMaxTaps2d);
    AGAN_REQUIRE((d->SH == 1 || d->SH == 2) && (d->SW == 1 || d->SW == 2), "conv2d: strides %dx%d unsupported (1 or 2 per axis)", d->SH, d->SW);
    AGAN_REQUIRE(d->PH >= 0 && d->PW >= 0 && d->PH < d->KH && d->PW < d->KW, "conv2d: padding %dx%d unsupported for %dx%d taps", d->PH, d->PW,
                 d->KH, d->KW);
    AGAN_REQUIRE(d->OH == (d->IH + 2 * d->PH - d->KH) / d->SH + 1 && d->OW == (d->IW + 2 * d->PW - d->KW) / d->SW + 1 &&
                     d->IH + 2 * d->PH >= d->KH && d->IW + 2 * d->PW >= d->KW,
                 "conv2d: output %dx%d does not match input %dx%d, taps %dx%d, stride %dx%d, padding %dx%d", d->OH, d->OW, d->IH, d->IW, d->KH,
// ... 107 lines not shown
```

### attention-gan_amd/csrc/conv_common.h

```cpp
#pragma once
#include "agan_common.h"
#include "dispatch.h"

#include <algorithm>

namespace agan {
namespace conv {

typedef float f32x16 __attribute__((ext_vector_type(16)));

extern thread_local const void* g_noted_kernel;
#define AGAN_LAUNCH(kernel, ...)                                                   \
    do {                                                                           \
        ::agan::conv::g_noted_kernel = reinterpret_cast<const void*>(kernel);      \
        hipLaunchKernelGGL(kernel, __VA_ARGS__);                                   \
    } while (0)
void timed_begin(hipStream_t st);
void timed_end(hipStream_t st, int split);


struct FastDiv {
    unsigned mul, shift;
    __device__ __forceinline__ int div(int n) const { return (int)((__umulhi(mul, (unsigned)n) + (unsigned)n) >> shift); }
};
// ... 151 lines not shown
}

struct GatherPlan {
    int bn, mtiles, ntiles, ncls, ksplit, kchunk;
    size_t slab, ws_bytes;
};

inline GatherPlan plan_gather(const Geom& g, int prec) {
    const int bk = prec == AGAN_PREC_F32 ? 16 : 32;
    const int slots = prec == AGAN_PREC_F32 ? 768 : 512;
    GatherPlan p;
    p.bn = g.Cout >= 96 ? 128 : (g.Cout >= 48 ? 64 : 32);
    p.mtiles = cdiv(g.Mtot, 128);
    p.ntiles = cdiv(g.Cout, p.bn);
    p.ncls = g.OS * g.OS;
    const int tiles = p.mtiles * p.ntiles * p.ncls;
    const int ktiles = cdiv(g.K, bk);
    int ks = 1;
    if (tiles < slots) ks = std::max(1, std::min({slots / tiles, std::max(1, ktiles / 16), 32}));
    p.kchunk = cdiv(ktiles, ks) * bk;
    p.ksplit = cdiv(g.K, p.kchunk);
    p.slab = (size_t)g.B * g.Cout * g.OH * g.OW;
    p.slab = (p.slab + 3) / 4 * 4;
    p.ws_bytes = p.ksplit > 1 ? p.slab * p.ksplit * sizeof(float) : 0;
    return p;
}

struct WgradPlan {
    int bi, bj, itiles, jtiles, ncls, psplit, pchunk;
    size_t slab, ws_bytes;
};

inline WgradPlan plan_wgrad(const Geom& g, bool needs_combine) {
    WgradPlan p;
    p.bi = (g.K >= 96 && cdiv(g.K, 128) * 128 <= cdiv(g.K, 64) * 64) ? 128 : 64;
    p.bj = g.Cout >= 96 ? 128 : 64;
    p.itiles = cdiv(g.K, p.bi);
    p.jtiles = cdiv(g.Cout, p.bj);
    p.ncls = g.OS * g.OS;
    const int tiles = p.itiles * p.jtiles * p.ncls;
    const int ptiles = cdiv(g.Mtot, 32);
    int ps = 1;
    if (tiles < 512) {
        const int cap = std::max(1, ptiles / 4);
        const int ps1 = std::max(1, std::min(512 / tiles, cap)), ps2 = std::max(1, std::min(1024 / tiles, cap));
        const double fill1 = (double)tiles * ps1 / 512.0, fill2 = (double)tiles * ps2 / 1024.0;
        ps = std::min(fill2 > fill1 + 1e-9 ? ps2 : ps1, 2048);
    }
    p.pchunk = cdiv(ptiles, ps) * 32;
    p.psplit = cdiv(g.Mtot, p.pchunk);
    p.slab = ((size_t)p.ncls * g.Cout * g.K + 3) / 4 * 4;
    const size_t nslabs = p.psplit + (needs_combine ? 1 : 0);
    p.ws_bytes = p.slab * nslabs * sizeof(float);
    return p;
}

struct SmallWgradPlan {
    int pchunk, nchunk;
    size_t slab, ws_bytes;
};
bool small_n_gather_supported(const Geom& g);
void launch_gather_small_n(const void* in, const float* wk, const float* bias, float* out, const Geom& g, hipStream_t st, int in_dtype = AGAN_DT_F32);
bool small_n_wgrad_supported(const Geom& g);
SmallWgradPlan plan_wgrad_small_n(const Geom& g);
void launch_wgrad_small_n(const void* x, const float* dy, float* part, const Geom& g, const SmallWgradPlan& p, hipStream_t st, int x_dtype = AGAN_DT_F32);

__host__ __device__ inline void pack_taps(int mode, int kh, int kw, int& R, int& S, int& SY) {
    switch (mode) {
        case AGAN_PACK_DGRAD_4x4S2: case AGAN_PACK_UP_FWD: R = S = 2; SY = 1; return;
        case AGAN_PACK_UP_DGRAD: R = S = 4; SY = 2; return;
        default: R = kh; S = kw; SY = (kh == 4) ? 2 : 1; return;
    }
}
struct PatchPlan {
    int twl, thl;
    int tiles_x, tiles_y, tiles_b, mtiles;
    int PW, PH, PHW, PP;
    int NPH, NT, IS;
    int nchunks, nstages, nsteps;
    int tapoff[9];
    int tappos[9];
    int base_y[2][2], base_x[2][2];
    FastDiv dPP, dPHW, dPW;
    FastDiv dNT, dNCLS, dMT, dTX, dTY, dNPH, dNPH2;
    int g_ntiles, g_ncls;
};
struct PatchGather {
    int bn, ntiles, ncls, ksplit, stages_per_split;
    size_t slab, ws_bytes;
};
struct PatchWgrad {
    int bj, jtiles, ncls, psplit, tiles_per_split, Kp;
    size_t slab, ws_bytes;
};
struct P16Plan {
    int ok;
    int gk;
    int twl, thl, TB;
    int tiles_x, tiles_y, tiles_b, mtiles;
    int PH, PW, LW, NXB, PXB, CHS;
    int nitems, NI;
    int nstages, wsteps;
    int bn, ntiles, ncls, ksplit, stages_per_split;
    int buf_bytes, smem_bytes;
    int lds_epi;
    int px2;
    int wc, lp;
    size_t slab, ws_bytes;
    FastDiv dNXB, dPH, dTB, dNT, dNCLS, dMT, dTX, dTY;
};
P16Plan plan_p16(const Geom& g, bool in16);
void launch_p16_gather(const void* in, const void* wk, const float* bias, void* dst, const Geom& g, const P16Plan& p, int prec, int act,
                       const void* lrelu_mask, hipStream_t st, bool in16, bool out16);
struct RowsPlan {
    int ok, gk, ci2, ups;
    int twl, thl, tbl;
    int tiles_x, tiles_y, tiles_b, mtiles;
    int XR, XRT;
    int rowb, cpitch;
    int halo, NBY, drowb, dpitch;
    int plane_bytes, smem_bytes, pc;
    int nxbl, nxitems, nyitems;
    int bj, jtiles, nchunks, ngroups, psplit, tiles_per_split;
    int NPH, NT, Kp;
    size_t slab, ws_bytes;
    FastDiv dXRT, dXR, dNBY;
};
enum class WinoKind : int {
    conv3x3,
    conv3x3_half,
    conv4x4_s2,
    dgrad2x2_class,
};
struct WinoPlan {
    int ok;
    WinoKind kind;
    int txl, tyl;
    int blocks_x, blocks_y, blocks_b, mtiles;
    int nf, ntiles;
    int pcp, raw_items, raw_bytes;
    int mpc, mpr;
    int smem_bytes;
    int ksplit, chunks_per_split;
    size_t u_bytes, slab, ws_bytes;
};
struct WinoWgradPlan {
    int ok, noct, jtiles, itiles, psplit, octs_per_split, smem_bytes;
    size_t slab, ws_bytes;
};
WinoWgradPlan plan_wino_wgrad(const Geom& g);
void launch_wino_wgrad(const float* x, const float* dy, float* part, const Geom& g, const WinoWgradPlan& p, hipStream_t st);
void launch_wino_wgrad_sum(const float* part, const Geom& g, const WinoWgradPlan& p, float* dw, int accumulate, hipStream_t st);
WinoPlan plan_wino(const Geom& g);
void launch_wino(const float* in, const float* wk, float* out, const Geom& g, const WinoPlan& p, void* ws, hipStream_t st);
int prec_planes(int prec);
RowsPlan plan_rows_wgrad(const Geom& g, int prec, bool x16, bool y16, bool up = false);
void launch_rows_wgrad(const void* x, const void* dy, float* part, const Geom& g, const RowsPlan& p, int prec, hipStream_t st,
                       const float* x_scale, const float* dy_scale, bool x16, bool y16);
void launch_patch_wgrad_unpack(const float* red, float* dw, int cout, int cin, int kh, int kw, bool up, int NPH, int NT, int Kp, int accumulate,
                               hipStream_t st);
void launch_wgrad_sum_unpack(const float* slabs, int nslabs, size_t slab, float* dw, int cout, int cin, int kh, int kw, int NPH, int NT, int Kp,
                             int accumulate, hipStream_t st);
PatchWgrad plan_patch_wgrad(const Geom& g, const PatchPlan& pp, int prec);
void launch_patch_wgrad(const void* x, const void* dy, float* part, const Geom& g, const PatchPlan& pp, const PatchWgrad& p, int prec,
                        hipStream_t st, const float* x_scale = nullptr, const float* dy_scale = nullptr, bool x16 = false, bool y16 = false);
constexpr float kF16WeightScale = 2048.f;
void launch_patch_wgrad_unpack(const float* red, float* dw, int cout, int cin, int kh, int kw, bool up, const PatchPlan& pp, const PatchWgrad& p,
                               int accumulate, hipStream_t st);
bool patch_supported(const Geom& g);
PatchPlan make_patch_plan(const Geom& g);
PatchGather plan_patch_gather(const Geom& g, const PatchPlan& pp);
size_t patch_packed_weight_bytes(int mode, int cout, int cin, int kh, int kw, int prec);
int pack_weight_patch(const float* w, void* wk, int mode, int cout, int cin, int kh, int kw, int prec, hipStream_t st);
int pack_job_blocks_patch(int mode, int cout, int cin, int kh, int kw);
int pack_weights_patch(const agan_pack_job* jobs, int njobs, int total_blocks, int prec, hipStream_t st);
void launch_patch_gather(const float* in, const void* wk, const float* bias, float* dst, const Geom& g, const PatchPlan& pp,
                         const PatchGather& p, int prec, int act, const float* lrelu_mask, hipStream_t st, const float* in_amax = nullptr,
                         float* out_amax = nullptr);

}
}
```

### attention-gan_amd/csrc/conv_wino.hip

```cpp
#include "conv_common.h"

#include <cstring>

using namespace agan;
using namespace agan::conv;

namespace {

typedef unsigned u32x4 __attribute__((ext_vector_type(4)));

__device__ __forceinline__ void lds_barrier_w() { asm volatile("s_waitcnt lgkmcnt(0)\n\ts_barrier" ::: "memory"); }

__global__ __launch_bounds__(256) void wino_weight_transform_kernel(const float* __restrict__ wk, float* __restrict__ U, int Kin, int Nld, int N) {
    const int total = Kin * Nld;
    for (int e = blockIdx.x * 256 + threadIdx.x; e < total; e += gridDim.x * 256) {
        const int n = e % Nld, c = e / Nld;
        float gk[3][3];
#pragma unroll
        for (int r = 0; r < 3; ++r)
#pragma unroll
            for (int s = 0; s < 3; ++s) gk[r][s] = n < N ? wk[(size_t)(c * 9 + r * 3 + s) * Nld + n] : 0.f;
        float t[4][3];
#pragma unroll
        for (int s = 0; s < 3; ++s) {
            t[0][s] = gk[0][s];
            t[1][s] = 0.5f * (gk[0][s] + gk[1][s] + gk[2][s]);
            t[2][s] = 0.5f * (gk[0][s] - gk[1][s] + gk[2][s]);
            t[3][s] = gk[2][s];
        }
        const int nch8 = Kin >> 3;
#pragma unroll
        for (int xi = 0; xi < 4; ++xi) {
            const float u0 = t[xi][0], u1 = 0.5f * (t[xi][0] + t[xi][1] + t[xi][2]), u2 = 0.5f * (t[xi][0] - t[xi][1] + t[xi][2]), u3 = t[xi][2];
            const float u[4] = {u0, u1, u2, u3};
#pragma unroll
            for (int nu = 0; nu < 4; ++nu) U[((size_t)((xi * 4 + nu) * nch8 + (c >> 3)) * Nld + n) * 8 + (c & 7)] = u[nu];
        }
    }
}

struct WinoTraits {
    int step, extra, origin;
    int cch;
    int planes, classes;
    int stages, nacc;
    int vfrags;
    int pieces;
    int ni32, ni64;
    int lds_cap;
    int s_u_second, s_raw_load, s_u_next, s_transform, s_raw_store;
    bool mulshift;
    bool store1_late;
};
constexpr WinoTraits wino_traits(WinoKind k) {
    WinoTraits t{};
    t.origin = -1; t.classes = 1; t.lds_cap = 160 * 1024; t.s_u_second = 0; t.s_raw_load = 1;
    switch (k) {
    case WinoKind::conv3x3:
        t.step = 2; t.extra = 2; t.cch = 8; t.planes = 16; t.stages = 16; t.nacc = 16; t.vfrags = 16; t.pieces = 4; t.ni32 = 7; t.ni64 = 11;
        t.s_u_next = 8; t.s_transform = 1; t.s_raw_store = 14;
        break;
    case WinoKind::conv3x3_half:
        t.step = 2; t.extra = 2; t.cch = 8; t.planes = 16; t.stages = 8; t.nacc = 8; t.vfrags = 16; t.pieces = 4; t.ni32 = 7;
        t.s_u_next = 4; t.s_transform = 1; t.s_raw_store = 6; t.lds_cap = 80 * 1024; t.mulshift = true;
        break;
    case WinoKind::conv4x4_s2:
        t.step = 4; t.extra = 2; t.cch = 8; t.planes = 36; t.stages = 36; t.nacc = 9; t.vfrags = 36; t.pieces = 4; t.ni32 = 21;
        t.s_u_next = 18; t.s_transform = 2; t.s_raw_store = 32; t.store1_late = true;
        break;
    case WinoKind::dgrad2x2_class:
        t.step = 2; t.extra = 1; t.cch = 16; t.planes = 36; t.classes = 4; t.stages = 18; t.nacc = 9; t.vfrags = 18; t.pieces = 2; t.ni32 = 11;
        t.s_u_next = 9; t.s_transform = 2; t.s_raw_store = 15; t.store1_late = true;
        break;
    }
    return t;
}

template <int D>
__device__ __forceinline__ void wino_input_f22(const float* src, int pcp, float* o, int pp) {
    float t[3][3];
#pragma unroll
    for (int j = 0; j < 3; ++j) {
        const float d0 = src[D * j], d1 = src[D * pcp + D * j], d2 = src[2 * D * pcp + D * j];
        t[0][j] = d0 - d1; t[1][j] = d1; t[2][j] = d2 - d1;
    }
#pragma unroll
    for (int xi = 0; xi < 3; ++xi) {
        o[(xi * 3 + 0) * pp] = t[xi][0] - t[xi][1]; o[(xi * 3 + 1) * pp] = t[xi][1]; o[(xi * 3 + 2) * pp] = t[xi][2] - t[xi][1];
    }
}

template <int NACC>
__device__ __forceinline__ void wino_output_2x2(const f32x16 (&acc)[NACC], int r, float (&y)[4]) {
    if constexpr (NACC == 16) {
        float c0[4], c1[4];
#pragma unroll
        for (int nu = 0; nu < 4; ++nu) {
            c0[nu] = acc[0 + nu][r] + acc[4 + nu][r] + acc[8 + nu][r];
            c1[nu] = acc[4 + nu][r] - acc[8 + nu][r] - acc[12 + nu][r];
        }
        y[0] = c0[0] + c0[1] + c0[2]; y[1] = c0[1] - c0[2] - c0[3];
        y[2] = c1[0] + c1[1] + c1[2]; y[3] = c1[1] - c1[2] - c1[3];
    } else {
        static_assert(NACC == 9, "F(2x2, 3x3) or F(2x2, 2x2)");
        float c0[3], c1[3];
#pragma unroll
        for (int nu = 0; nu < 3; ++nu) {
            c0[nu] = acc[nu][r] + acc[3 + nu][r];
            c1[nu] = acc[3 + nu][r] + acc[6 + nu][r];
        }
        y[0] = c0[0] + c0[1]; y[1] = c0[1] + c0[2];
        y[2] = c1[0] + c1[1]; y[3] = c1[1] + c1[2];
    }
}

template <WinoKind K, int NTG>
struct WinoGather {
    static constexpr WinoTraits T = wino_traits(K);
    static constexpr bool kHalf = K == WinoKind::conv3x3_half, kS2 = K == WinoKind::conv4x4_s2, kCls = K == WinoKind::dgrad2x2_class;
    static constexpr bool k3x3 = T.nacc != 9;
    static constexpr int NFW = kHalf ? 2 : 4 / NTG;
    static constexpr int NTL = 32 * NTG, LT = NTG == 1 ? 5 : 6;
    static constexpr int NI = NTG == 1 ? T.ni32 : T.ni64;
    static constexpr int CCH = T.cch, C8 = T.cch / 8;
    static constexpr int S = T.stages, SH = T.stages / 2, NACC = T.nacc;
    static constexpr int NPIECE = T.pieces * NTG;
    static constexpr int VBUF = T.vfrags * NTL * 8;
    static constexpr int STEP = T.step;
    static_assert(NI > 0, "this block size of the variant is not built: plan_wino must not route to it");
    static_assert(T.s_u_next == SH && T.s_transform + NPIECE <= S && T.s_raw_store < S, "slots of the chunk loop");

    const Geom& g;
    const WinoPlan& wp;
    int tid, lane, w, fw, tg, hh, l31, lh;
    int mt, nt, ks, py, px;
    int n0, txl, tyl, TX, TY, tx0, ty0, tb0, ihw, ohw, PR, PC, PCP, RAWBUF;
    float *raw, *V;
    __amdgpu_buffer_rsrc_t rx, rU;
    int nch8, c_beg, nch;
    int iy0, ix0;

    __device__ __forceinline__ WinoGather(const float* x, const float* U, const Geom& g_, const WinoPlan& wp_) : g(g_), wp(wp_) {
        extern __shared__ __attribute__((aligned(16))) unsigned char lds[];
        tid = threadIdx.x; lane = tid & 63;
        w = __builtin_amdgcn_readfirstlane(tid >> 6);
        fw = w % NFW; tg = kHalf ? 0 : w / NFW; hh = kHalf ? w / NFW : 0;
        l31 = lane & 31; lh = lane >> 5;
        ks = py = px = 0;
        {
            int F = xcd_contiguous(linear_block_id(), wp.mtiles * wp.ntiles * (kS2 ? wp.ksplit : T.classes));
            nt = F % wp.ntiles; F /= wp.ntiles;
            if constexpr (kS2) { mt = F % wp.mtiles; ks = F / wp.mtiles; }
            else if constexpr (kCls) { py = (F & 3) >> 1; px = F & 1; mt = F >> 2; }
            else mt = F;
        }
        n0 = nt * (NFW * 32);
        txl = wp.txl; tyl = wp.tyl;
        TX = 1 << txl; TY = 1 << tyl;
        const int bxi = mt % wp.blocks_x, byi = (mt / wp.blocks_x) % wp.blocks_y, bbi = mt / (wp.blocks_x * wp.blocks_y);
        tx0 = bxi << txl; ty0 = byi << tyl; tb0 = bbi << (LT - txl - tyl);
        ihw = g.IH * g.IW; ohw = g.OH * g.OW;
        PR = STEP * TY + T.extra; PC = STEP * TX + T.extra;
        PCP = wp.pcp;
        raw = reinterpret_cast<float*>(lds);
        RAWBUF = wp.raw_bytes >> 2;
        V = reinterpret_cast<float*>(lds + 2 * wp.raw_bytes);
        nch8 = g.Cin >> 3;
        if constexpr (kS2) { c_beg = ks * wp.chunks_per_split; nch = min(nch8, c_beg + wp.chunks_per_split) - c_beg; }
        else { c_beg = 0; nch = g.Cin >> (CCH == 8 ? 3 : 4); }
        constexpr int PPC = T.planes / T.classes;
        rx = make_rsrc(x, (size_t)g.B * g.Cin * ihw * sizeof(float));
        rU = make_rsrc(U + (size_t)(py * 2 + px) * PPC * nch8 * g.Nld * 8, (size_t)PPC * nch8 * g.Nld * 8 * sizeof(float));
        iy0 = STEP * ty0 + T.origin + py; ix0 = STEP * tx0 + T.origin + px;
    }

    __device__ __forceinline__ void stage_items(int (&it_off)[NI], unsigned (&it_lds)[NI]) const {
#pragma unroll
        for (int i = 0; i < NI; ++i) {
            const int e = tid + i * 256;
            int col, row, t2;
            if constexpr (T.mulshift) {
                const int t1 = (int)(__umul24(e, wp.mpc) >> 16);
                col = e - (int)__umul24(t1, PC);
                t2 = (int)(__umul24(t1, wp.mpr) >> 16); row = t1 - (int)__umul24(t2, PR);
            } else {
                col = e % PC; const int t1 = e / PC;
                row = t1 % PR; t2 = t1 / PR;
            }
            const int ci = t2 & (CCH - 1), b = tb0 + (t2 >> (CCH == 8 ? 3 : 4)), iy = iy0 + row, ix = ix0 + col;
            const bool ok = (e < wp.raw_items) & (b < g.B) & ((unsigned)iy < (unsigned)g.IH) & ((unsigned)ix < (unsigned)g.IW);
            if constexpr (T.mulshift) {
// ... 84 lines not shown
            for (int pi = 0; pi < NPIECE; ++pi) transform_piece(raw, V, pi, td);
            if (T.store1_late && nch > 1) store_raw(it_lds, 1, rawv);
            lds_barrier_w();
        }
#pragma unroll 1
        for (int ch = 0; ch < nch; ++ch) {
            const float* Vc = V + (ch & 1) * VBUF;
            float* Vn = V + ((ch + 1) & 1) * VBUF;
            const float* rn = raw + ((ch + 1) & 1) * RAWBUF;
            const bool more = ch + 1 < nch;
            const unsigned vlane = (unsigned)(hh * S * NTL * 8 + (tg * 32 + l31) * CCH + lh * 4);
            u32x4 vf[2];
            vf[0] = *reinterpret_cast<const u32x4*>(Vc + vlane);
#pragma unroll
            for (int st = 0; st < S; ++st) {
                if (st + 1 < S) vf[(st + 1) & 1] = *reinterpret_cast<const u32x4*>(Vc + ((st + 1) / C8) * NTL * CCH + ((st + 1) % C8) * 8 + vlane);
                if (st == T.s_u_second) load_u(ch, 1, ub);
                if (st == T.s_raw_load && ch + 2 < nch) load_raw(it_off, ch + 2, rawv);
                if (st == T.s_u_next) load_u(ch + 1, 0, ua);
                if (more && st >= T.s_transform && st < T.s_transform + NPIECE) transform_piece(rn, Vn, st - T.s_transform, td);
                if (st == T.s_raw_store && ch + 2 < nch) store_raw(it_lds, ch + 2, rawv);
                const u32x4 uf = st < SH ? ua[st % SH] : ub[st % SH];
                const int a = kS2 ? st % NACC : st / C8;
#pragma unroll
                for (int j = 0; j < 4; ++j)
                    acc[a] = __builtin_amdgcn_mfma_f32_32x32x2f32(__uint_as_float(uf[j]), __uint_as_float(vf[st & 1][j]), acc[a], 0, 0, 0);
                __builtin_amdgcn_sched_barrier(0);
            }
            lds_barrier_w();
        }
    }

    __device__ __forceinline__ void epilogue(const f32x16 (&acc)[NACC], float* out) const {
        typedef float f32x2_ __attribute__((ext_vector_type(2)));
        typedef unsigned u32x2_ __attribute__((ext_vector_type(2)));
        const int lt = tg * 32 + l31;
        const int tx = lt & (TX - 1), ty = (lt >> txl) & (TY - 1), tb = lt >> (txl + tyl);
        const int b = tb0 + tb, oy = 2 * (ty0 + ty), ox = 2 * (tx0 + tx);
        const bool pvalid = (b < g.B) & (oy < (kCls ? g.OHs : g.OH)) & (ox < (kCls ? g.OWs : g.OW));
        const __amdgpu_buffer_rsrc_t ro = make_rsrc(out + (size_t)ks * wp.slab, (size_t)g.B * g.Cout * ohw * sizeof(float));
        const int nw = n0 + fw * 32;
#pragma unroll
        for (int r = 0; r < 16; ++r) {
            float y[4];
            wino_output_2x2(acc, r, y);
            const int n = nw + (r & 3) + 8 * (r >> 2) + 4 * lh;
            const bool ok = pvalid & (n < g.Cout);
            if constexpr (kCls) {
                const unsigned off = (unsigned)((b * g.Cout + n) * ohw + (2 * oy + py) * g.OW + 2 * ox + px) * 4u;
                buf_store(ro, ok ? off : kOOB, y[0]);
                buf_store(ro, ok ? off + 8u : kOOB, y[1]);
                buf_store(ro, ok ? off + (unsigned)(2 * g.OW) * 4u : kOOB, y[2]);
                buf_store(ro, ok ? off + (unsigned)(2 * g.OW + 2) * 4u : kOOB, y[3]);
            } else {
                const unsigned off = (unsigned)((b * g.Cout + n) * ohw + oy * g.OW + ox) * 4u;
                __builtin_amdgcn_raw_buffer_store_b64(__builtin_bit_cast(u32x2_, f32x2_{y[0], y[1]}), ro, ok ? off : kOOB, 0, 0);
                __builtin_amdgcn_raw_buffer_store_b64(__builtin_bit_cast(u32x2_, f32x2_{y[2], y[3]}), ro, ok ? off + (unsigned)g.OW * 4u : kOOB, 0, 0);
            }
        }
    }
};

template <int NFW>
__global__ __launch_bounds__(256, 1) void conv_wino_f32_kernel(const float* __restrict__ x, const float* __restrict__ U, float* __restrict__ out,
                                                               const Geom g, const WinoPlan wp) {
    WinoGather<WinoKind::conv3x3, 4 / NFW> k(x, U, g, wp);
    f32x16 acc[k.NACC];
    k.accumulate(acc);
    k.epilogue(acc, out);
}

__global__ __launch_bounds__(256, 2) void conv_wino_h_f32_kernel(const float* __restrict__ x, const float* __restrict__ U, float* __restrict__ out,
                                                                 const Geom g, const WinoPlan wp) {
    WinoGather<WinoKind::conv3x3_half, 1> k(x, U, g, wp);
    f32x16 acc[8];
    k.accumulate(acc);

    const int w = k.w, lane = k.lane, hh = k.hh, ohw = k.ohw;
    float* const X = k.raw;
    typedef float f32x2_ __attribute__((ext_vector_type(2)));
    typedef unsigned u32x2_ __attribute__((ext_vector_type(2)));
    const int tx = k.l31 & (k.TX - 1), ty = (k.l31 >> k.txl) & (k.TY - 1), tb = k.l31 >> (k.txl + k.tyl);
    const int b = k.tb0 + tb, oy = 2 * (k.ty0 + ty) + hh, ox = 2 * (k.tx0 + tx);
    const bool pvalid = (b < g.B) & (oy < g.OH) & (ox < g.OW);
    const __amdgpu_buffer_rsrc_t ro = make_rsrc(out, (size_t)g.B * g.Cout * ohw * sizeof(float));
    const int nw = k.n0 + k.fw * 32, pw = w ^ 2;
    const unsigned vo = pvalid ? (unsigned)((b * g.Cout + nw + 4 * k.lh) * ohw + oy * g.OW + ox) * 4u : kOOB;
    auto finish = [&](auto hc) {
        constexpr int HH = decltype(hc)::value;
        f32x2_ keep[8][2];
#pragma unroll
        for (int rp = 0; rp < 8; ++rp) {
            f32x2_ t[2][2];
#pragma unroll
            for (int x2 = 0; x2 < 2; ++x2) {
                const f32x2_ m0 = {acc[x2 * 4 + 0][2 * rp], acc[x2 * 4 + 0][2 * rp + 1]};
                const f32x2_ m1 = {acc[x2 * 4 + 1][2 * rp], acc[x2 * 4 + 1][2 * rp + 1]};
                const f32x2_ m2 = {acc[x2 * 4 + 2][2 * rp], acc[x2 * 4 + 2][2 * rp + 1]};
                const f32x2_ m3 = {acc[x2 * 4 + 3][2 * rp], acc[x2 * 4 + 3][2 * rp + 1]};
                t[x2][0] = m0 + m1 + m2;
                t[x2][1] = m1 - m2 - m3;
            }
#pragma unroll
            for (int c = 0; c < 2; ++c) {
                keep[rp][c] = t[0][c] + t[1][c];
                const f32x2_ send = HH == 0 ? t[1][c] : t[0][c];
                X[(w * 32 + (2 * rp) * 2 + c) * 64 + lane] = send[0];
                X[(w * 32 + (2 * rp + 1) * 2 + c) * 64 + lane] = send[1];
            }
        }
        lds_barrier_w();
#pragma unroll
        for (int r = 0; r < 16; ++r) {
            if (nw + 8 * (r >> 2) < g.Cout) {
                const float x0 = X[(pw * 32 + r * 2 + 0) * 64 + lane], x1 = X[(pw * 32 + r * 2 + 1) * 64 + lane];
                const float k0 = keep[r >> 1][0][r & 1], k1 = keep[r >> 1][1][r & 1];
                const f32x2_ y = HH == 0 ? f32x2_{x0 + k0, x1 + k1} : f32x2_{x0 - k0, x1 - k1};
                __builtin_amdgcn_raw_buffer_store_b64(__builtin_bit_cast(u32x2_, y), ro, vo, (unsigned)(((r & 3) + 8 * (r >> 2)) * ohw) * 4u, 0);
            }
        }
    };
    if (hh == 0) finish(std::integral_constant<int, 0>{});
    else finish(std::integral_constant<int, 1>{});
}

template <int NFW>
__global__ __launch_bounds__(256, 1) void conv_wino_s2_f32_kernel(const float* __restrict__ x, const float* __restrict__ U, float* __restrict__ out,
                                                                  const Geom g, const WinoPlan wp) {
    WinoGather<WinoKind::conv4x4_s2, 4 / NFW> k(x, U, g, wp);
    f32x16 acc[k.NACC];
    k.accumulate(acc);
    k.epilogue(acc, out);
}

template <int NFW>
__global__ __launch_bounds__(256, 1) void conv_wino_cls_f32_kernel(const float* __restrict__ x, const float* __restrict__ U, float* __restrict__ out,
                                                                   const Geom g, const WinoPlan wp) {
    WinoGather<WinoKind::dgrad2x2_class, 4 / NFW> k(x, U, g, wp);
    f32x16 acc[k.NACC];
    k.accumulate(acc);
    k.epilogue(acc, out);
}

__device__ __forceinline__ void wino_weights_f22(const float (&gk)[2][2], float* o, size_t pp) {
    const float t[3][2] = {{gk[0][0], gk[0][1]}, {gk[0][0] + gk[1][0], gk[0][1] + gk[1][1]}, {gk[1][0], gk[1][1]}};
#pragma unroll
    for (int xi = 0; xi < 3; ++xi) {
        const float u[3] = {t[xi][0], t[xi][0] + t[xi][1], t[xi][1]};
#pragma unroll
        for (int nu = 0; nu < 3; ++nu) o[(xi * 3 + nu) * pp] = u[nu];
    }
}

__global__ __launch_bounds__(256) void wino_cls_weight_transform_kernel(const float* __restrict__ wk, float* __restrict__ U, int Kin, int Nld, int N) {
    const int total = 4 * Kin * Nld, nch8 = Kin >> 3;
    for (int e = blockIdx.x * 256 + threadIdx.x; e < total; e += gridDim.x * 256) {
        const int n = e % Nld, t1 = e / Nld, c = t1 % Kin, cls = t1 / Kin;
        const float* wc = wk + (size_t)cls * Kin * 4 * Nld;
        float gk[2][2];
#pragma unroll
        for (int a = 0; a < 2; ++a)
#pragma unroll
            for (int b = 0; b < 2; ++b) gk[a][b] = n < N ? wc[(size_t)(c * 4 + (1 - a) * 2 + (1 - b)) * Nld + n] : 0.f;
        wino_weights_f22(gk, U + ((size_t)(cls * 9 * nch8 + (c >> 3)) * Nld + n) * 8 + (c & 7), (size_t)nch8 * Nld * 8);
    }
}

__global__ __launch_bounds__(256) void wino_s2_weight_transform_kernel(const float* __restrict__ wk, float* __restrict__ U, int Kin, int Nld, int N) {
    const int total = Kin * Nld, nch8 = Kin >> 3;
    for (int e = blockIdx.x * 256 + threadIdx.x; e < total; e += gridDim.x * 256) {
        const int n = e % Nld, c = e / Nld;
#pragma unroll
        for (int p = 0; p < 2; ++p)
#pragma unroll
            for (int q = 0; q < 2; ++q) {
                float gk[2][2];
#pragma unroll
                for (int a = 0; a < 2; ++a)
#pragma unroll
                    for (int b = 0; b < 2; ++b) gk[a][b] = n < N ? wk[(size_t)(c * 16 + (2 * a + p) * 4 + 2 * b + q) * Nld + n] : 0.f;
                wino_weights_f22(gk, U + ((size_t)((p * 2 + q) * 9 * nch8 + (c >> 3)) * Nld + n) * 8 + (c & 7), (size_t)nch8 * Nld * 8);
            }
    }
}

__global__ __launch_bounds__(256, 1) void conv_wino_wgrad_f32_kernel(const float* __restrict__ x, const float* __restrict__ dy, float* __restrict__ part,
                                                                     const Geom g, const WinoWgradPlan wp) {
    extern __shared__ __attribute__((aligned(16))) unsigned char lds[];
    constexpr int ZV = 16 * 64 * 8;
    float* const L = reinterpret_cast<float*>(lds);
    const int tid = threadIdx.x, lane = tid & 63;
    const int w = __builtin_amdgcn_readfirstlane(tid >> 6);
    const int fj = w & 1, fi = w >> 1;
    const int l31 = lane & 31, lh = lane >> 5;
    int jt, it, split;
    {
        int F = xcd_contiguous(linear_block_id(), wp.jtiles * wp.itiles * wp.psplit);
        jt = F % wp.jtiles; F /= wp.jtiles;
        it = F % wp.itiles; split = F / wp.itiles;
    }
    const int j0 = jt * 64, i0 = it * 64;
    const int ihw = g.IH * g.IW;
    const int o_beg = split * wp.octs_per_split, o_end = min(wp.noct, o_beg + wp.octs_per_split);
    const __amdgpu_buffer_rsrc_t rx = make_rsrc(x, (size_t)g.B * g.Cin * ihw * sizeof(float));
    const __amdgpu_buffer_rsrc_t rd = make_rsrc(dy, (size_t)g.B * g.Cout * ihw * sizeof(float));
    const int tw8 = g.OW >> 4, th = g.OH >> 1;

    const int tj = tid & 7, tc = tid >> 3;
    float xr[2][16];
    float2 dr[2][2];
    auto load_piece = [&](int o, int lp) {
        const bool ov = o < o_end;
        const int txo = o % tw8, t1 = o / tw8;
        const int ty = t1 % th, b = t1 / th;
        const int tx = txo * 8 + tj;
        const int k = lp >> 1, half = lp & 1;
        const int ci = i0 + tc + 32 * k, co = j0 + tc + 32 * k;
        const bool cv = ov & (ci < g.Cin);
        const int xbase = (b * g.Cin + ci) * ihw + 2 * tx - 1;
        const bool c0ok = tx > 0, c3ok = 2 * tx + 2 < g.IW;
#pragma unroll
        for (int ii = 0; ii < 2; ++ii) {
            const int i = 2 * half + ii;
            const int iy = 2 * ty - 1 + i;
            const bool rv = cv & ((unsigned)iy < (unsigned)g.IH);
            const unsigned ro = (unsigned)(xbase + iy * g.IW) * 4u;
            xr[k][i * 4 + 0] = buf_load(rx, (rv & c0ok) ? ro : kOOB);
            xr[k][i * 4 + 1] = buf_load(rx, rv ? ro + 4u : kOOB);
            xr[k][i * 4 + 2] = buf_load(rx, rv ? ro + 8u : kOOB);
            xr[k][i * 4 + 3] = buf_load(rx, (rv & c3ok) ? ro + 12u : kOOB);
        }
        if (half == 0) {
            const bool dv = ov & (co < g.Cout);
            const int dbase = (b * g.Cout + co) * ihw + 2 * ty * g.OW + 2 * tx;
#pragma unroll
            for (int a = 0; a < 2; ++a)
                dr[k][a] = __builtin_bit_cast(float2, __builtin_amdgcn_raw_buffer_load_b64(rd, dv ? (unsigned)(dbase + a * g.OW) * 4u : kOOB, 0, 0));
        }
    };
    auto load_oct = [&](int o) {
#pragma unroll
        for (int lp = 0; lp < 4; ++lp) load_piece(o, lp);
    };
    float tt_[2][4][4];
    auto transform_piece = [&](float* buf, int tp) {
        const int k = tp >> 2, sub = tp & 3;
        const int ch = tc + 32 * k;
        if (sub == 0) {
#pragma unroll
            for (int c = 0; c < 4; ++c) {
                const float d0 = xr[k][c], d1 = xr[k][4 + c], d2 = xr[k][8 + c], d3 = xr[k][12 + c];
                tt_[k][0][c] = d0 - d2; tt_[k][1][c] = d1 + d2; tt_[k][2][c] = d2 - d1; tt_[k][3][c] = d3 - d1;
            }
        }
        if (sub < 2) {
#pragma unroll
            for (int x2 = 0; x2 < 2; ++x2) {
                const int xi = 2 * sub + x2;
                const float* t = tt_[k][xi];
                float* o = buf + ZV + ((xi * 4) * 64 + ch) * 8 + tj;
                o[0] = t[0] - t[2]; o[64 * 8] = t[1] + t[2]; o[2 * 64 * 8] = t[2] - t[1]; o[3 * 64 * 8] = t[3] - t[1];
            }
        } else {
            const float e00 = dr[k][0].x, e01 = dr[k][0].y, e10 = dr[k][1].x, e11 = dr[k][1].y;
#pragma unroll
            for (int x2 = 0; x2 < 2; ++x2) {
                const int xi = 2 * (sub - 2) + x2;
                const float u0 = xi == 0 ? e00 : (xi == 1 ? 0.5f * (e00 + e10) : (xi == 2 ? 0.5f * (e00 - e10) : e10));
                const float u1 = xi == 0 ? e01 : (xi == 1 ? 0.5f * (e01 + e11) : (xi == 2 ? 0.5f * (e01 - e11) : e11));
                float* o = buf + ((xi * 4) * 64 + ch) * 8 + tj;
                o[0] = u0; o[64 * 8] = 0.5f * (u0 + u1); o[2 * 64 * 8] = 0.5f * (u0 - u1); o[3 * 64 * 8] = u1;
            }
        }
    };
    auto transform_store = [&](float* buf) {
#pragma unroll
        for (int tp = 0; tp < 8; ++tp) transform_piece(buf, tp);
    };

    f32x16 acc[16];
#pragma unroll
    for (int q = 0; q < 16; ++q)
#pragma unroll
        for (int r = 0; r < 16; ++r) acc[q][r] = 0.f;

    if (o_beg < o_end) {
        load_oct(o_beg);
        transform_store(L);
        load_oct(o_beg + 1);
        lds_barrier_w();
        const unsigned zl = (unsigned)((fj * 32 + l31) * 8 + lh * 4), vl = (unsigned)(ZV + (fi * 32 + l31) * 8 + lh * 4);
        for (int o = o_beg; o < o_end; ++o) {
            const float* cur = L + ((o - o_beg) & 1) * (2 * ZV);
            float* nxt = L + (((o - o_beg) & 1) ^ 1) * (2 * ZV);
            u32x4 zf[2], vf[2];
            zf[0] = *reinterpret_cast<const u32x4*>(cur + zl);
            vf[0] = *reinterpret_cast<const u32x4*>(cur + vl);
#pragma unroll
            for (int pos = 0; pos < 16; ++pos) {
                if (pos + 1 < 16) {
                    zf[(pos + 1) & 1] = *reinterpret_cast<const u32x4*>(cur + (pos + 1) * 64 * 8 + zl);
                    vf[(pos + 1) & 1] = *reinterpret_cast<const u32x4*>(cur + (pos + 1) * 64 * 8 + vl);
                }
                if (pos >= 1 && pos <= 8) transform_piece(nxt, pos - 1);
                if (pos >= 9 && pos <= 12) load_piece(o + 2, pos - 9);
#pragma unroll
                for (int j = 0; j < 4; ++j)
                    acc[pos] = __builtin_amdgcn_mfma_f32_32x32x2f32(__uint_as_float(zf[pos & 1][j]), __uint_as_float(vf[pos & 1][j]), acc[pos], 0, 0, 0);
#pragma unroll
                for (int j = 0; j < 4; ++j) {
                    __builtin_amdgcn_sched_group_barrier(0x008, 1, 0);
                    __builtin_amdgcn_sched_group_barrier(0x100, 1, 0);
                    __builtin_amdgcn_sched_group_barrier(0x002, 8, 0);
                    __builtin_amdgcn_sched_group_barrier(0x020, 3, 0);
                    __builtin_amdgcn_sched_group_barrier(0x200, 1, 0);
                }
                __builtin_amdgcn_sched_barrier(0);
            }
            lds_barrier_w();
        }
    }

    float* const o = part + (size_t)split * wp.slab;
    const __amdgpu_buffer_rsrc_t ro = make_rsrc(o, (size_t)9 * g.Cout * g.Cin * sizeof(float));
    const int ci = i0 + fi * 32 + l31;
    const int cob = j0 + fj * 32;
    const unsigned vo = ci < g.Cin ? (unsigned)(4 * lh * g.Cin + ci) * 4u : kOOB;
    const unsigned tapb = (unsigned)(g.Cout * g.Cin) * 4u;
#pragma unroll
    for (int r = 0; r < 16; ++r) {
        if (cob + 8 * (r >> 2) >= g.Cout) continue;
        float c[3][4];
#pragma unroll
        for (int nu = 0; nu < 4; ++nu) {
            const float m0 = acc[nu][r], m1 = acc[4 + nu][r], m2 = acc[8 + nu][r], m3 = acc[12 + nu][r];
            c[0][nu] = m0 + m1 + m2;
            c[1][nu] = m1 - m2;
            c[2][nu] = m1 + m2 + m3;
        }
        const unsigned so = (unsigned)((cob + (r & 3) + 8 * (r >> 2)) * g.Cin) * 4u;
#pragma unroll
        for (int rr = 0; rr < 3; ++rr) {
            __builtin_amdgcn_raw_buffer_store_b32(__builtin_bit_cast(unsigned, c[rr][0] + c[rr][1] + c[rr][2]), ro, vo, so + (unsigned)(rr * 3 + 0) * tapb, 0);
            __builtin_amdgcn_raw_buffer_store_b32(__builtin_bit_cast(unsigned, c[rr][1] - c[rr][2]), ro, vo, so + (unsigned)(rr * 3 + 1) * tapb, 0);
            __builtin_amdgcn_raw_buffer_store_b32(__builtin_bit_cast(unsigned, c[rr][1] + c[rr][2] + c[rr][3]), ro, vo, so + (unsigned)(rr * 3 + 2) * tapb, 0);
        }
    }
}

__global__ __launch_bounds__(256) void wino_wgrad_sum_kernel(const float* __restrict__ part, int nslabs, size_t slab, int cout, int cin,
                                                             float* __restrict__ dw, int accumulate) {
    __shared__ f32x4 red[8][32];
    const int q4 = cin >> 2, n4 = 9 * cout * q4;
    const int el = threadIdx.x & 31, grp = threadIdx.x >> 5;
    for (int base = blockIdx.x * 32; base < n4; base += gridDim.x * 32) {
        const int e = base + el;
        f32x4 a = {0.f, 0.f, 0.f, 0.f};
        if (e < n4) {
            const float* src = part + (size_t)e * 4;
            int sp = grp;
            for (; sp + 24 < nslabs; sp += 32) {
                const f32x4 v0 = *reinterpret_cast<const f32x4*>(src + (size_t)sp * slab);
                const f32x4 v1 = *reinterpret_cast<const f32x4*>(src + (size_t)(sp + 8) * slab);
                const f32x4 v2 = *reinterpret_cast<const f32x4*>(src + (size_t)(sp + 16) * slab);
                const f32x4 v3 = *reinterpret_cast<const f32x4*>(src + (size_t)(sp + 24) * slab);
                a += (v0 + v1) + (v2 + v3);
            }
            for (; sp < nslabs; sp += 8) a += *reinterpret_cast<const f32x4*>(src + (size_t)sp * slab);
        }
        red[grp][el] = a;
        __syncthreads();
        if (grp == 0 && e < n4) {
#pragma unroll
            for (int k = 1; k < 8; ++k) a += red[k][el];
            const int c4 = e % q4, t1 = e / q4;
            const int co = t1 % cout, tap = t1 / cout;
            float* dst = dw + ((size_t)co * cin + 4 * c4) * 9 + tap;
#pragma unroll
            for (int k = 0; k < 4; ++k) dst[k * 9] = accumulate ? dst[k * 9] + a[k] : a[k];
        }
        __syncthreads();
    }
}

int pow2floor_log(int v) {
    int l = 0;
    while ((2 << l) <= v) ++l;
    return l;
}

}

namespace agan {
namespace conv {

WinoPlan plan_wino(const Geom& g) {
    WinoPlan p;
    memset(&p, 0, sizeof(p));
    if (g.SY == 1 && g.R == 3 && g.S == 3 && g.DY == 1 && g.OS == 1 && g.OY0 == -1 && g.IH == g.OH && g.IW == g.OW)
        p.kind = (g.Cout & 7) == 0 ? WinoKind::conv3x3_half : WinoKind::conv3x3;
    else if (g.SY == 2 && g.R == 4 && g.S == 4 && g.DY == 1 && g.OS == 1 && g.OY0 == -1 && g.IH == 2 * g.OH && g.IW == 2 * g.OW) p.kind = WinoKind::conv4x4_s2;
    else if (g.SY == 1 && g.R == 2 && g.S == 2 && g.DY == -1 && g.OS == 2 && g.OY0 == 0 && g.OY1 == 1 && g.OH == 2 * g.IH && g.OW == 2 * g.IW) p.kind = WinoKind::dgrad2x2_class;
    else return p;
    const WinoTraits T = wino_traits(p.kind);
    const bool k3x3 = p.kind == WinoKind::conv3x3 || p.kind == WinoKind::conv3x3_half;
    if ((g.OHs & 1) || (g.OWs & 1) || (g.Cin & (T.cch - 1)) || g.Cout < 32) return p;
    if (!k3x3 && g.Cout < 96) return p;
    const int tw = g.OWs / 2, th = g.OHs / 2;
    if (tw < 4) return p;
    p.nf = (g.Cout >= 96 || p.kind == WinoKind::conv3x3_half) ? 4 : 2;
    const int lt = p.nf == 4 ? 5 : 6;
    p.txl = std::min(3, pow2floor_log(tw));
    p.tyl = std::min(lt - p.txl, pow2floor_log(th));
    const int TX = 1 << p.txl, TY = 1 << p.tyl, TB = (1 << lt) >> (p.txl + p.tyl);
    p.blocks_x = cdiv(tw, TX);
    p.blocks_y = cdiv(th, TY);
    p.blocks_b = cdiv(g.B, TB);
    p.mtiles = p.blocks_x * p.blocks_y * p.blocks_b;
    p.ntiles = p.kind == WinoKind::conv3x3_half ? cdiv(g.Cout, 64) : cdiv(g.Cout, p.nf * 32);
    p.ksplit = 1;
    if (p.kind == WinoKind::conv4x4_s2 && p.mtiles * p.ntiles < 512 && p.mtiles * p.ntiles >= 256 && g.Cin >= 128) p.ksplit = 2;
    if (p.mtiles * p.ntiles * p.ksplit * T.classes < (k3x3 ? 256 : 512)) return p;
    p.chunks_per_split = cdiv(g.Cin / 8, p.ksplit);
    p.slab = ((size_t)g.B * g.Cout * g.OH * g.OW + 3) / 4 * 4;
    const int PR = T.step * TY + T.extra, PC = T.step * TX + T.extra;
    p.pcp = (PC + 1) & ~1;
    p.mpc = (65536 + PC - 1) / PC;
    p.mpr = (65536 + PR - 1) / PR;
    p.raw_items = TB * T.cch * PR * PC;
    if (p.raw_items > (lt == 5 ? T.ni32 : T.ni64) * 256) return p;
    p.raw_bytes = (TB * T.cch * PR * p.pcp * 4 + 15) & ~15;
    p.smem_bytes = 2 * p.raw_bytes + 2 * T.vfrags * (1 << lt) * 8 * 4;
    if (p.smem_bytes > T.lds_cap) return p;
    p.u_bytes = ((size_t)T.planes * (g.Cin / 8) * g.Nld * 8 * sizeof(float) + 255) / 256 * 256;
    p.ws_bytes = p.u_bytes + (p.ksplit > 1 ? p.slab * p.ksplit * sizeof(float) : 0);
    p.ok = 1;
    return p;
}

namespace {
template <auto Kernel, WinoKind K>
void launch_gather_kernel(dim3 grid, const float* in, const float* U, float* out, const Geom& g, const WinoPlan& p, hipStream_t st) {
    allow_dynamic_lds<Kernel>(wino_traits(K).lds_cap);
    AGAN_LAUNCH(Kernel, grid, dim3(256), (size_t)p.smem_bytes, st, in, U, out, g, p);
}
}

void launch_wino(const float* in, const float* wk, float* out, const Geom& g, const WinoPlan& p, void* ws, hipStream_t st) {
    float* U = static_cast<float*>(ws);
    const int total = g.Cin * g.Nld;
    const dim3 grid(p.mtiles * p.ntiles * p.ksplit * wino_traits(p.kind).classes), tgrid(std::min(cdiv(total, 256), 2048));
    switch (p.kind) {
    case WinoKind::dgrad2x2_class:
        AGAN_LAUNCH(wino_cls_weight_transform_kernel, dim3(std::min(cdiv(4 * total, 256), 4096)), dim3(256), 0, st, wk, U, g.Cin, g.Nld, g.Cout);
        launch_gather_kernel<conv_wino_cls_f32_kernel<4>, WinoKind::dgrad2x2_class>(grid, in, U, out, g, p, st);
        break;
    case WinoKind::conv4x4_s2:
        AGAN_LAUNCH(wino_s2_weight_transform_kernel, tgrid, dim3(256), 0, st, wk, U, g.Cin, g.Nld, g.Cout);
        launch_gather_kernel<conv_wino_s2_f32_kernel<4>, WinoKind::conv4x4_s2>(
            grid, in, U, p.ksplit > 1 ? reinterpret_cast<float*>(static_cast<char*>(ws) + p.u_bytes) : out, g, p, st);
        break;
    case WinoKind::conv3x3_half:
        AGAN_LAUNCH(wino_weight_transform_kernel, tgrid, dim3(256), 0, st, wk, U, g.Cin, g.Nld, g.Cout);
        launch_gather_kernel<conv_wino_h_f32_kernel, WinoKind::conv3x3_half>(grid, in, U, out, g, p, st);
        break;
    case WinoKind::conv3x3:
        AGAN_LAUNCH(wino_weight_transform_kernel, tgrid, dim3(256), 0, st, wk, U, g.Cin, g.Nld, g.Cout);
        if (p.nf == 4) launch_gather_kernel<conv_wino_f32_kernel<4>, WinoKind::conv3x3>(grid, in, U, out, g, p, st);
        else launch_gather_kernel<conv_wino_f32_kernel<2>, WinoKind::conv3x3>(grid, in, U, out, g, p, st);
        break;
    }
}

WinoWgradPlan plan_wino_wgrad(const Geom& g) {
    WinoWgradPlan p;
    memset(&p, 0, sizeof(p));
    if (!(g.SY == 1 && g.R == 3 && g.S == 3 && g.DY == 1 && g.OS == 1 && g.OY0 == -1)) return p;
    if (g.IH != g.OH || g.IW != g.OW || (g.OH & 1) || (g.OW & 15) || g.Cin < 32 || g.Cout < 32 || (g.Cin & 3) || (g.Cout & 7)) return p;
    p.noct = g.B * (g.OH / 2) * (g.OW / 16);
    p.jtiles = cdiv(g.Cout, 64);
    p.itiles = cdiv(g.Cin, 64);
    const int wgs = p.jtiles * p.itiles;
    if (p.noct < 64 * 16 || wgs > 256) return p;
    const int ps = std::max(1, std::min(256 / wgs, p.noct / 16));
    p.octs_per_split = cdiv(p.noct, ps);
    p.psplit = cdiv(p.noct, p.octs_per_split);
    p.slab = ((size_t)g.Cout * g.Cin * 9 + 3) / 4 * 4;
    p.ws_bytes = p.slab * p.psplit * sizeof(float);
    p.smem_bytes = 2 * 2 * 16 * 64 * 8 * 4;
    p.ok = 1;
    return p;
}

void launch_wino_wgrad(const float* x, const float* dy, float* part, const Geom& g, const WinoWgradPlan& p, hipStream_t st) {
    allow_dynamic_lds<conv_wino_wgrad_f32_kernel>(160 * 1024);
    AGAN_LAUNCH(conv_wino_wgrad_f32_kernel, dim3(p.jtiles * p.itiles * p.psplit), dim3(256), (size_t)p.smem_bytes, st, x, dy, part, g, p);
}

void launch_wino_wgrad_sum(const float* part, const Geom& g, const WinoWgradPlan& p, float* dw, int accumulate, hipStream_t st) {
    const int n4 = 9 * g.Cout * (g.Cin >> 2);
    AGAN_LAUNCH(wino_wgrad_sum_kernel, dim3(std::min(cdiv(n4, 32), 8192)), dim3(256), 0, st, part, p.psplit, p.slab, g.Cout, g.Cin, dw, accumulate);
}

}
}
```

### include/agan.h

```cpp
#ifndef AGAN_H_
#define AGAN_H_

#include <stddef.h>
#include <stdint.h>

#ifdef __cplusplus
extern "C" {
#endif

#define AGAN_VERSION 101

enum {
    AGAN_OK = 0,
    AGAN_EINVAL = -1,
    AGAN_EWORKSPACE = -2,
    AGAN_ELAUNCH = -3
};

enum {
    AGAN_PREC_F32 = 0,
    AGAN_PREC_BF16 = 1,
    AGAN_PREC_BF16X3 = 2,
    AGAN_PREC_F16 = 3,
    AGAN_PREC_BF16X6 = 4,
    AGAN_PREC_F16X3 = 5
};

enum { AGAN_DT_F32 = 0, AGAN_DT_BF16 = 1, AGAN_DT_F16 = 2 };

int agan_version(void);
const char* agan_last_error(void);

typedef struct agan_conv_geom {
    int32_t B;
    int32_t Cin, IH, IW;
    int32_t Cout, OH, OW;
    int32_t R, S;
    int32_t OS;
    int32_t SY, DY;
    int32_t OY[2];
} agan_conv_geom;

enum {
    AGAN_PACK_FWD = 0,
    AGAN_PACK_DGRAD_S1 = 1,
    AGAN_PACK_DGRAD_4x4S2 = 2,
    AGAN_PACK_UP_FWD = 3,
    AGAN_PACK_UP_DGRAD = 4,
    AGAN_PACK_DGRAD_3x3S2 = 5
};

size_t agan_packed_weight_bytes(int mode, int cout, int cin, int kh, int kw, int prec);
int agan_pack_weight(const float* w, void* wk, int mode, int cout, int cin, int kh, int kw, int prec, void* stream);
typedef struct agan_pack_job {
    const float* w;
    void* wk;
    int32_t mode, cout, cin, kh, kw, first_block;
} agan_pack_job;
int agan_pack_job_blocks(int mode, int cout, int cin, int kh, int kw);
int agan_pack_job_blocks_prec(int mode, int cout, int cin, int kh, int kw, int prec);
int agan_pack_weights(const agan_pack_job* jobs, int njobs, int total_blocks, int prec, void* stream);

size_t agan_conv_ktable_elems(const agan_conv_geom* g);
int agan_conv_ktable(const agan_conv_geom* g, int32_t* table, void* stream);

int agan_conv_effective_prec(const agan_conv_geom* g, int prec);
int agan_conv_wgrad_effective_prec(const agan_conv_geom* g, int pack_mode, int prec);
double agan_conv_executed_fraction(const agan_conv_geom* g, int prec, int wgrad, int plain_epilogue);
size_t agan_conv_gather_ws_bytes(const agan_conv_geom* g, int prec);
int agan_conv_gather(const float* in, const void* wk, const float* bias, float* out, const agan_conv_geom* g,
                     const int32_t* ktable, int prec, int act, const float* lrelu_mask, void* ws, size_t ws_bytes, void* stream,
                     const float* in_amax ,
                     float* out_amax );

int agan_conv_gather_dt_supported(const agan_conv_geom* g, int prec, int in_dtype, int out_dtype);
int agan_conv_gather_dt(const void* in, const void* wk, const float* bias, void* out, const agan_conv_geom* g,
                        const int32_t* ktable, int prec, int act, const void* lrelu_mask, void* ws, size_t ws_bytes, void* stream,
                        const float* in_amax, float* out_amax, int in_dtype, int out_dtype);

#define AGAN_AMAX_SLOT 256
int agan_absmax(const float* x, size_t n, float* amax_slot, void* stream);

size_t agan_conv_wgrad_ws_bytes(const agan_conv_geom* g);
int agan_conv_wgrad(const float* x, const float* dy, float* dw, const agan_conv_geom* g, const int32_t* ktable, int pack_mode,
                    int kh, int kw, int prec, int accumulate, void* ws, size_t ws_bytes, void* stream,
                    const float* x_amax, const float* dy_amax);

int agan_conv_wgrad_dt_supported(const agan_conv_geom* g, int pack_mode, int prec, int x_dtype, int dy_dtype);
int agan_conv_wgrad_dt(const void* x, const void* dy, float* dw, const agan_conv_geom* g, const int32_t* ktable, int pack_mode,
                       int kh, int kw, int prec, int accumulate, void* ws, size_t ws_bytes, void* stream,
                       const float* x_amax, const float* dy_amax, int x_dtype, int dy_dtype);

int agan_bias_grad(const float* dy, float* dbias, int B, int C, int HW, int accumulate, void* stream);

enum { AGAN_ACT_NONE = 0, AGAN_ACT_GLU = 1, AGAN_ACT_LRELU = 2, AGAN_ACT_TANH = 3, AGAN_ACT_SIGMOID = 4, AGAN_ACT_RELU = 5 };

size_t agan_bn_stats_ws_bytes(int B, int C, int HW);
int agan_bn_stats(const float* x, int B, int C, int HW, float eps, float* mean, float* invstd,
                  float* running_mean, float* running_var, int64_t* num_batches_tracked, float momentum,
                  void* ws, size_t ws_bytes, void* stream);
int agan_bn_act_fwd(const float* x, const float* mean, const float* invstd, const float* gamma, const float* beta,
                    const float* residual, float* out, int B, int C, int HW, int act, void* stream, float* out_amax);
size_t agan_bn_train_fwd_ws_bytes(int B, int C, int HW);
int agan_bn_train_fwd(const float* x, const float* gamma, const float* beta, const float* residual, float* out, float* mean,
                      float* invstd, float* running_mean, float* running_var, int64_t* num_batches_tracked, int B, int C, int HW,
                      float eps, float momentum, int act, int groups, void* ws, size_t ws_bytes, void* stream, float* out_amax);
size_t agan_bn_act_bwd_ws_bytes(int B, int C, int HW);
int agan_bn_act_bwd(const float* x, const float* dout, const float* mean, const float* invstd, const float* gamma,
                    const float* beta, float* dx, float* dgamma, float* dbeta, int B, int C, int HW, int act, int accumulate,
                    int groups, void* ws, size_t ws_bytes, void* stream, float* dx_amax);
int agan_bn_stats_dt(const void* x, int B, int C, int HW, float eps, float* mean, float* invstd, float* running_mean,
                     float* running_var, int64_t* num_batches_tracked, float momentum, void* ws, size_t ws_bytes, void* stream,
                     int x_dtype);
int agan_bn_act_fwd_dt(const void* x, const float* mean, const float* invstd, const float* gamma, const float* beta,
                       const void* residual, void* out, int B, int C, int HW, int act, void* stream, float* out_amax, int x_dtype,
                       int out_dtype);
int agan_bn_train_fwd_dt(const void* x, const float* gamma, const float* beta, const void* residual, void* out, float* mean,
                         float* invstd, float* running_mean, float* running_var, int64_t* num_batches_tracked, int B, int C, int HW,
                         float eps, float momentum, int act, int groups, void* ws, size_t ws_bytes, void* stream, float* out_amax,
                         int x_dtype, int out_dtype);
int agan_bn_act_bwd_dt(const void* x, const void* dout, const float* mean, const float* invstd, const float* gamma,
                       const float* beta, void* dx, float* dgamma, float* dbeta, int B, int C, int HW, int act, int accumulate,
                       int groups, void* ws, size_t ws_bytes, void* stream, float* dx_amax, int x_dtype, int out_dtype);
int agan_act_fwd(const float* x, float* out, size_t n, int act, void* stream);
int agan_act_bwd(const float* out, const float* dout, float* dx, size_t n, int act, void* stream);
int agan_glu_fwd(const float* x, float* out, int B, int C, int HW, void* stream);
int agan_glu_bwd(const float* x, const float* dout, float* dx, int B, int C, int HW, void* stream);
int agan_bn_last_launch(int* codes, int capacity);

int agan_attn_fwd(const float* images, const float* words, const float* w, const int64_t* mask, float scale,
                  float* proj, float* ctx, float* attn, int B, int C, int E, int T, int HW, void* stream);
size_t agan_attn_bwd_ws_bytes(int B, int C, int T, int HW);
int agan_attn_bwd(const float* images, const float* words, const float* w, const float* proj, const float* attn,
                  const float* dctx, const float* dattn, float scale, float* dimages, float* dwords, float* dw,
                  int B, int C, int E, int T, int HW, int accumulate, void* ws, size_t ws_bytes, void* stream);
int agan_attn_fwd_dt(const void* images, const float* words, const float* w, const int64_t* mask, float scale, float* proj,
                     void* ctx, float* attn, int B, int C, int E, int T, int HW, void* stream, int dtype);
int agan_attn_bwd_dt(const void* images, const float* words, const float* w, const float* proj, const float* attn,
                     const void* dctx, const float* dattn, float scale, void* dimages, float* dwords, float* dw, int B, int C,
                     int E, int T, int HW, int accumulate, void* ws, size_t ws_bytes, void* stream, int dtype);

int agan_func_attention_fwd(const float* query, const float* context, float gamma1, float scale, float* wctx, float* attn,
                            int B, int D, int L, int S, void* stream);
int agan_func_attention_bwd(const float* query, const float* context, const float* dwctx, const float* dattn, float gamma1,
                            float scale, float* dquery, float* dcontext, int B, int D, int L, int S, void* stream);
size_t agan_words_loss_save_elems(int B, int D, int T, int S);
int agan_words_loss_fwd(const float* feat, const float* wemb, const int64_t* lens, const int64_t* class_ids, const int64_t* labels,
                        float gamma1, float gamma2, float gamma3, float lambda, float* loss, float* sim, float* attn_maps,
                        float* save, int B, int D, int T, int S, void* stream);
size_t agan_words_loss_bwd_ws_bytes(int B, int D, int T, int S);
int agan_words_loss_bwd(const float* feat, const float* wemb, const int64_t* lens, const float* save, const float* dloss,
                        float gamma1, float gamma2, float gamma3, float lambda, float* dfeat, float* dwemb,
                        int B, int D, int T, int S, void* ws, size_t ws_bytes, void* stream);
int agan_sent_loss_fwd(const float* cnn_code, const float* rnn_code, const int64_t* class_ids, const int64_t* labels, float gamma3, float lambda,
                       float eps, float* loss, float* save , int B, int D, void* stream);
int agan_sent_loss_bwd(const float* cnn_code, const float* rnn_code, const float* save, const float* dloss, float gamma3,
                       float lambda, float eps, float* dcnn, float* drnn, int B, int D, void* stream);

int agan_disc_loss(const float* p_real, const float* p_fake, float* loss, float* dp_real, float* dp_fake, int B, void* stream);
int agan_gen_loss(const float* p_fake, float* loss, float* dp_fake, int B, void* stream);
int agan_kl_loss(const float* mu, const float* logvar, float* loss, float* dmu, float* dlogvar, int n, void* stream);
int agan_reparam_fwd(const float* mu, const float* logvar, const float* eps, float* c, int n, void* stream);
int agan_reparam_bwd(const float* logvar, const float* eps, const float* dc, float* dmu, float* dlogvar, int n, void* stream);

int agan_adam_step(float* param, const float* grad, float* exp_avg, float* exp_avg_sq, size_t n, int32_t* step_state, double lr,
                   double beta1, double beta2, double eps, float grad_scale, void* stream);

int agan_timer_create(void** event);
int agan_timer_destroy(void* event);
int agan_timer_arm(void* start, void* stop);
int agan_timer_elapsed_ms(void* start, void* stop, float* ms);
int agan_timer_last_kernel(char* name, size_t capacity);
int agan_timer_last_split(void);

static inline int agan_round_up(int v, int m) { return (v + m - 1) / m * m; }

#define AGAN_COMM_ID_BYTES 128
int agan_comm_unique_id(void* id);
int agan_comm_init(void** comm, int rank, int world, const void* id);
int agan_comm_destroy(void* comm);
int agan_allreduce_bucket(void* comm, float* buf, size_t n, void* stream);
size_t agan_allreduce_scratch_bytes(size_t n, int world, int wire_dtype);
int agan_allreduce_bucket_dt(void* comm, float* buf, size_t n, int wire_dtype, void* scratch, size_t scratch_bytes, void* stream);
size_t agan_exchange_wire_elems(size_t n, int world);
int agan_exchange_pack_bf16(const float* g, void* wire, size_t n, size_t n_wire, void* stream);
int agan_exchange_sum_bf16(const void* pieces , int world, size_t per,
                           void* sum , void* stream);
int agan_exchange_unpack_bf16(const void* wire, float* g, size_t n, void* stream);
size_t agan_allreduce_chunk_elems(size_t n, int world);

typedef struct agan_conv2d_desc {
    int32_t B;
    int32_t Cin, IH, IW;
    int32_t Cout, OH, OW;
    int32_t KH, KW, SH, SW, PH, PW;
    int32_t in_c0, in_ctot;
    int32_t out_c0, out_ctot;
} agan_conv2d_desc;
int agan_conv2d_pack_mode(const agan_conv2d_desc* d, int dgrad);
int agan_conv2d_effective_prec(const agan_conv2d_desc* d, int prec);
size_t agan_conv2d_ws_bytes(const agan_conv2d_desc* d, int dgrad);
size_t agan_conv2d_ktable_elems(const agan_conv2d_desc* d, int dgrad);
int agan_conv2d_ktable(const agan_conv2d_desc* d, int dgrad, int32_t* table, void* stream);
int agan_conv2d_fwd(const float* x, const void* wk, const float* bias, float* y, const agan_conv2d_desc* d, const int32_t* ktable, int act,
                    void* ws, size_t ws_bytes, void* stream);
int agan_conv2d_dgrad(const float* dy, const void* wk, float* dx, const agan_conv2d_desc* d, const int32_t* ktable, const float* relu_mask,
                      int accumulate, void* ws, size_t ws_bytes, void* stream);

int agan_conv2d_train_supported(const agan_conv2d_desc* d);
int agan_conv2d_train_slabs(const agan_conv2d_desc* d);
size_t agan_conv2d_train_ws_bytes(const agan_conv2d_desc* d, int direction);
int agan_conv2d_train_fwd(const float* x, const float* w, const float* bias, float* y, const agan_conv2d_desc* d, void* ws, size_t ws_bytes,
                          void* stream);
int agan_conv2d_train_dgrad(const float* dy, const float* w, float* dx, const agan_conv2d_desc* d, int accumulate, void* ws, size_t ws_bytes,
                            void* stream);
int agan_conv2d_train_wgrad(const float* x, const float* dy, float* dw, const agan_conv2d_desc* d, int accumulate, void* ws, size_t ws_bytes,
                            void* stream);

int agan_maxpool3s2_fwd(const float* x, float* y, uint8_t* argmax, int B, int C, int H, int W, int out_c0, int out_ctot, void* stream);
int agan_maxpool3s2_bwd(const float* dy, const uint8_t* argmax, const float* relu_mask, float* dx, int B, int C, int H, int W, int out_c0,
                        int out_ctot, int accumulate, void* stream);
int agan_avgpool3s1_fwd(const float* x, float* y, int B, int C, int H, int W, void* stream);
int agan_avgpool3s1_bwd(const float* dy, const float* relu_mask, float* dx, int B, int C, int H, int W, int accumulate, void* stream);
int agan_global_avgpool_fwd(const float* x, float* y, int B, int C, int HW, void* stream);
int agan_global_avgpool_bwd(const float* dy, const float* relu_mask, float* dx, int B, int C, int HW, int accumulate, void* stream);
int agan_resize_bilinear_fwd(const float* x, float* y, int B, int C, int IH, int IW, int OH, int OW, void* stream);
int agan_resize_bilinear_bwd(const float* dy, float* dx, int B, int C, int IH, int IW, int OH, int OW, void* stream);
int agan_relu_bwd(const float* y, const float* dy, float* dx, size_t n, int accumulate, void* stream);

size_t agan_bn_relu_slice_fwd_ws_bytes(int B, int C, int HW);
int agan_bn_relu_slice_fwd(const float* x, const float* gamma, const float* beta, float* out, int out_c0, int out_ctot, float* mean,
// ... 82 lines not shown
```

Before: 1000 images/s.

## Cache Winograd-transformed weights in the packed-weight cache instead of per-call transform

Adds new pack modes that hold Winograd-domain weight tensors (U), built from the regular packed weights and cached per weight version. They are rebuilt in a batched job kernel when the flat parameter range is repacked after an optimizer step. Forward and dgrad Winograd convolutions then take U directly, skipping the weight-transform launch on every call and shrinking their workspace. The cost is extra memory for the cached U tensors, more pack-table bookkeeping, and a second repack kernel per weight update.

```diff
diff --git a/attention-gan_amd/backend/functional.py b/attention-gan_amd/backend/functional.py
--- a/attention-gan_amd/backend/functional.py
+++ b/attention-gan_amd/backend/functional.py
@@ -211,12 +211,19 @@
                    ("first_block", "<i4")]
 
 
-def _pack_table(rng, prec: int):
+def _is_wino(mode: int) -> bool:
+    return mode in L.WINO_PACK_SOURCE
+
+
+def _pack_table(rng, prec: int, wino: bool = False):
     import numpy as np
-    entries = [e for e in rng[3] if e["prec"] == prec]
+    entries = [e for e in rng[3] if e["prec"] == prec and _is_wino(e["mode"]) == wino]
+    if wino and not entries:
+        return None
     if rng[4] is None:
         rng[4] = {}
-    hit = rng[4].get(prec)
+    tkey = (prec, wino)
+    hit = rng[4].get(tkey)
     if hit is None or hit[1] != len(entries):
         if torch.cuda.is_current_stream_capturing():
             raise L.AganError("packed-weight job table missing during HIP-graph capture: run a warm-up step and "
@@ -226,10 +233,14 @@
         first = 0
         for i, e in enumerate(entries):
             cout, cin, kh, kw = e["dims"]
-            jobs[i] = (e["ptr"], e["wk"].data_ptr(), e["mode"], cout, cin, kh, kw, first)
+            src = e["ptr"]
+            if wino:
+                skey = (L.WINO_PACK_SOURCE[e["mode"]], prec)
+                src = next(s for s in rng[3] if s["cache"] is e["cache"] and s["key"] == skey)["wk"].data_ptr()
+            jobs[i] = (src, e["wk"].data_ptr(), e["mode"], cout, cin, kh, kw, first)
             first += lib.agan_pack_job_blocks_prec(e["mode"], cout, cin, kh, kw, prec)
         table = torch.from_numpy(jobs.view(np.uint8).copy()).to(entries[0]["wk"].device)
-        hit = rng[4][prec] = (table, len(entries), first)
+        hit = rng[4][tkey] = (table, len(entries), first)
     return hit
 
 
@@ -237,11 +248,15 @@
     for rng in _FLAT_RANGES:
         for prec in sorted({e["prec"] for e in rng[3]}):
             _pack_table(rng, prec)
+            _pack_table(rng, prec, True)
 
 
 def _repack_group(rng, prec: int) -> None:
     table, n, total = _pack_table(rng, prec)
     L.call("agan_pack_weights", _p(table), n, total, prec, _stream())
+    wino = _pack_table(rng, prec, True)
+    if wino is not None:
+        L.call("agan_pack_weights_wino", _p(wino[0]), wino[1], wino[2], _stream())
     for e in rng[3]:
         if e["prec"] == prec:
             e["cache"][e["key"]] = ((e["ptr"], e["tver"], _WEIGHT_EPOCH[0], rng[2]) + e["dims"], e["wk"], rng)
@@ -295,9 +310,13 @@
     n = L.load().agan_packed_weight_bytes(mode, cout, cin, kh, kw, prec)
     if n == 0:
         raise L.AganError(f"pack mode {mode} / precision {prec} does not take a {kh}x{kw} kernel")
+    src = packed_weight(w, L.WINO_PACK_SOURCE[mode], cache, prec) if _is_wino(mode) else None
     reuse = hit is not None and hit[1].numel() == n and hit[1].device == w.device
     wk = hit[1] if reuse else torch.empty(n, dtype=torch.uint8, device=w.device)
-    L.call("agan_pack_weight", _p(w), _p(wk), mode, cout, cin, kh, kw, prec, _stream())
+    if src is not None:
+        L.call("agan_wino_pack_weight", _p(src), _p(wk), mode, cout, cin, kh, kw, _stream())
+    else:
+        L.call("agan_pack_weight", _p(w), _p(wk), mode, cout, cin, kh, kw, prec, _stream())
     if cache is not None:
         cache[key] = (ver, wk, rng)
         if rng is not None:
@@ -387,18 +406,32 @@
     return slot
 
 
+_WEIGHT_FORM = {}
+
+
+def gather_weight_form(g: L.ConvGeom, pack_mode: int, prec: int, in_dt: int, out_dt: int, epilogue: bool) -> int:
+    if prec != L.PREC_F32:
+        return pack_mode
+    key = (pack_mode, in_dt, out_dt, epilogue, g.B, g.Cin, g.IH, g.IW, g.Cout, g.OH, g.OW, g.R, g.S, g.OS, g.SY, g.DY, g.OY[0], g.OY[1])
+    hit = _WEIGHT_FORM.get(key)
+    if hit is None:
+        hit = _WEIGHT_FORM[key] = int(L.load().agan_conv_gather_weight_form(byref(g), pack_mode, prec, in_dt, out_dt, int(epilogue)))
+    return hit
+
+
 def _gather(x: Tensor, wk: Tensor, bias: Optional[Tensor], g: L.ConvGeom, out: Tensor, kind: str = "", phase: str = "",
-            act: int = 0, lrelu_mask: Optional[Tensor] = None, prec: int = L.PREC_F32, in_amax: Optional[Tensor] = None) -> None:
+            act: int = 0, lrelu_mask: Optional[Tensor] = None, prec: int = L.PREC_F32, in_amax: Optional[Tensor] = None,
+            form: int = -1) -> None:
     lib = L.load()
-    nbytes = lib.agan_conv_gather_ws_bytes(byref(g), prec)
+    nbytes = lib.agan_conv_gather_form_ws_bytes(byref(g), prec, form) if _is_wino(form) else lib.agan_conv_gather_ws_bytes(byref(g), prec)
     ws, wsp = _ws(nbytes, x)
     kt = ktable(g, x.device)
     obs = _OBSERVER[0]
     if obs is not None:
         obs.begin(kind, phase, g, x.element_size(), out.element_size())
     out_amax = _amax_out(out) if prec != L.PREC_F32 else None
-    L.call("agan_conv_gather_dt", _p(x), _p(wk), _p(bias), _p(out), byref(g), _p(kt), prec, act, _p(lrelu_mask), wsp, nbytes,
-           _stream(), _p(in_amax), _p(out_amax), _dt(x), _dt(out))
+    L.call("agan_conv_gather_form", _p(x), _p(wk), _p(bias), _p(out), byref(g), _p(kt), prec, act, _p(lrelu_mask), wsp, nbytes,
+           _stream(), _p(in_amax), _p(out_amax), _dt(x), _dt(out), form)
     if obs is not None:
         obs.end()
 
@@ -473,7 +506,8 @@
         b = _dev(bias.detach(), "conv bias") if bias is not None else None
         need_xs = pe == L.PREC_F16X3 or (ctx.needs_input_grad[1] and _needs_amax() and wgrad_effective_precision(gf, pf) == L.PREC_F16X3)
         xs = amax_of(x) if need_xs else None
-        _gather(x, packed_weight(w, pf, cache, pe), b, gf, out, kind, "fwd", act, None, pe, xs)
+        fw = gather_weight_form(gf, pf, pe, _dt(x), odt, b is not None or act != L.ACT_NONE) if cache is not None else pf
+        _gather(x, packed_weight(w, fw, cache, pe), b, gf, out, kind, "fwd", act, None, pe, xs, fw)
         ctx.x_scale = xs
         if act == L.ACT_NONE:
             ctx.save_for_backward(x, w)
@@ -543,8 +577,9 @@
             mask = x if ctx.handoff_in is not None else None
             if mask is not None and mask.dtype != dx.dtype:
                 mask = mask.to(dx.dtype)
-            _gather(dyg, packed_weight(w, pd, ctx.cache, pe_d), None, gd, dx, ctx.kind, "dgrad", L.ACT_NONE, mask, pe_d,
-                    dys if pe_d == L.PREC_F16X3 else None)
+            fd = gather_weight_form(gd, pd, pe_d, _dt(dyg), ddt, mask is not None) if ctx.cache is not None else pd
+            _gather(dyg, packed_weight(w, fd, ctx.cache, pe_d), None, gd, dx, ctx.kind, "dgrad", L.ACT_NONE, mask, pe_d,
+                    dys if pe_d == L.PREC_F16X3 else None, fd)
             if mask is not None:
                 ctx.handoff_in.masked = True
         return dx, dw, db, None, None, None, None, None, None, None
diff --git a/attention-gan_amd/backend/lib.py b/attention-gan_amd/backend/lib.py
--- a/attention-gan_amd/backend/lib.py
+++ b/attention-gan_amd/backend/lib.py
@@ -10,6 +10,10 @@
 PREC_F32, PREC_BF16, PREC_BF16X3, PREC_F16, PREC_BF16X6, PREC_F16X3 = 0, 1, 2, 3, 4, 5
 PRECISIONS = {"f32": PREC_F32, "bf16": PREC_BF16, "bf16x3": PREC_BF16X3, "f16": PREC_F16, "bf16x6": PREC_BF16X6, "f16x3": PREC_F16X3}
 PACK_FWD, PACK_DGRAD_S1, PACK_DGRAD_4x4S2, PACK_UP_FWD, PACK_UP_DGRAD, PACK_DGRAD_3x3S2 = 0, 1, 2, 3, 4, 5
+PACK_WINO_FWD, PACK_WINO_DGRAD_S1, PACK_WINO_S2_FWD, PACK_WINO_CLS_DGRAD, PACK_WINO_S2_UP_DGRAD = 6, 7, 8, 9, 10
+WINO_PACK_SOURCE = {PACK_WINO_FWD: PACK_FWD, PACK_WINO_DGRAD_S1: PACK_DGRAD_S1, PACK_WINO_S2_FWD: PACK_FWD,
+                    PACK_WINO_CLS_DGRAD: PACK_DGRAD_4x4S2, PACK_WINO_S2_UP_DGRAD: PACK_UP_DGRAD}
+WINO_NONE, WINO_CONV3X3, WINO_CONV3X3_HALF, WINO_CONV4X4_S2, WINO_DGRAD2X2_CLASS = -1, 0, 1, 2, 3
 ACT_NONE, ACT_GLU, ACT_LRELU, ACT_TANH, ACT_SIGMOID, ACT_RELU = 0, 1, 2, 3, 4, 5
 COMM_ID_BYTES = 128
 DT_F32, DT_BF16, DT_F16 = 0, 1, 2
@@ -70,6 +74,13 @@
     "agan_conv_gather": (c_int, [_P, _P, _P, _P, POINTER(ConvGeom), _P, c_int, c_int, _P, _P, c_size_t, _P, _P, _P]),
     "agan_conv_gather_dt": (c_int, [_P, _P, _P, _P, POINTER(ConvGeom), _P, c_int, c_int, _P, _P, c_size_t, _P, _P, _P, c_int, c_int]),
     "agan_conv_gather_dt_supported": (c_int, [POINTER(ConvGeom), c_int, c_int, c_int]),
+    "agan_pack_source_mode": (c_int, [c_int]),
+    "agan_wino_pack_weight": (c_int, [_P, _P, c_int, c_int, c_int, c_int, c_int, _P]),
+    "agan_pack_weights_wino": (c_int, [_P, c_int, c_int, _P]),
+    "agan_conv_gather_weight_form": (c_int, [POINTER(ConvGeom), c_int, c_int, c_int, c_int, c_int]),
+    "agan_conv_gather_wino_kind": (c_int, [POINTER(ConvGeom), c_int, c_int, c_int, c_int]),
+    "agan_conv_gather_form_ws_bytes": (c_size_t, [POINTER(ConvGeom), c_int, c_int]),
+    "agan_conv_gather_form": (c_int, [_P, _P, _P, _P, POINTER(ConvGeom), _P, c_int, c_int, _P, _P, c_size_t, _P, _P, _P, c_int, c_int, c_int]),
     "agan_conv_wgrad_dt_supported": (c_int, [POINTER(ConvGeom), c_int, c_int, c_int, c_int]),
     "agan_conv_wgrad_dt": (c_int, [_P, _P, _P, POINTER(ConvGeom), _P, c_int, c_int, c_int, c_int, c_int, _P, c_size_t, _P, _P, _P, c_int, c_int]),
     "agan_bn_stats_dt": (c_int, [_P, c_int, c_int, c_int, c_float, _P, _P, _P, _P, _P, c_float, _P, c_size_t, _P, c_int]),
diff --git a/attention-gan_amd/csrc/conv.hip b/attention-gan_amd/csrc/conv.hip
--- a/attention-gan_amd/csrc/conv.hip
+++ b/attention-gan_amd/csrc/conv.hip
@@ -681,6 +681,10 @@
 
 __host__ __device__ inline int pack_job_blocks(int mode, int cout, int cin, int kh, int kw) {
     int ncls, K, N;
+    if (pack_is_wino(mode)) {
+        int planes;
+        return wino_form_dims(mode, cout, cin, kh, kw, planes, K, N) ? 0 : wino_form_blocks(mode, K, (N + 31) / 32 * 32);
+    }
     if (pack_dims(mode, cout, cin, kh, kw, ncls, K, N)) return 0;
     const int Nld = ((N + 31) / 32 * 32);
     if (mode == AGAN_PACK_FWD) return cdiv(K, 64) * cdiv(Nld, 64);
@@ -702,7 +706,7 @@
     const int local = b - j.first_block;
     float* wk = static_cast<float*>(j.wk);
     int ncls, K, N;
-    pack_dims(j.mode, j.cout, j.cin, j.kh, j.kw, ncls, K, N);
+    if (pack_dims(j.mode, j.cout, j.cin, j.kh, j.kw, ncls, K, N)) return;
     const int Nld = ((N + 31) / 32 * 32);
     if (j.mode == AGAN_PACK_FWD) {
         const int kt = cdiv(K, 64);
@@ -964,6 +968,11 @@
 
 size_t agan_packed_weight_bytes(int mode, int cout, int cin, int kh, int kw, int prec) {
     int ncls, K, N;
+    if (pack_is_wino(mode)) {
+        int planes;
+        if (prec != AGAN_PREC_F32 || wino_form_dims(mode, cout, cin, kh, kw, planes, K, N)) return 0;
+        return wino_u_bytes(planes, K, (N + 31) / 32 * 32);
+    }
     if (pack_dims(mode, cout, cin, kh, kw, ncls, K, N)) return 0;
     if (prec == AGAN_PREC_F32) return (size_t)ncls * K * ((N + 31) / 32 * 32) * sizeof(float);
     if (mode == AGAN_PACK_DGRAD_3x3S2) return 0;
@@ -1013,6 +1022,23 @@
     if (prec != AGAN_PREC_F32) return pack_weights_patch(jobs, njobs, total_blocks, prec, as_stream(stream));
     AGAN_LAUNCH(pack_jobs_kernel, dim3(total_blocks), dim3(256), 0, as_stream(stream), jobs, njobs);
     return check_launch("pack_weights");
+}
+
+int agan_pack_source_mode(int mode) { return pack_source_mode(mode); }
+
+int agan_wino_pack_weight(const float* src, void* u, int mode, int cout, int cin, int kh, int kw, void* stream) {
+    int planes, Kin, N;
+    AGAN_REQUIRE(src && u, "wino_pack_weight: null pointer");
+    AGAN_REQUIRE(pack_is_wino(mode) && wino_form_dims(mode, cout, cin, kh, kw, planes, Kin, N) == 0,
+                 "wino_pack_weight: mode %d does not take a %dx%d kernel on %d x %d channels (contraction channels in eights)", mode, kh, kw, cout, cin);
+    launch_wino_weight_form(src, static_cast<float*>(u), mode, Kin, N, as_stream(stream));
+    return check_launch("wino_pack_weight");
+}
+
+int agan_pack_weights_wino(const agan_pack_job* jobs, int njobs, int total_blocks, void* stream) {
+    AGAN_REQUIRE(jobs && njobs > 0 && total_blocks > 0, "pack_weights_wino: empty job list");
+    launch_wino_weight_jobs(jobs, njobs, total_blocks, as_stream(stream));
+    return check_launch("pack_weights_wino");
 }
 
 int agan_conv_effective_prec(const agan_conv_geom* g, int prec) { return route_gather(g, prec, AGAN_DT_F32, AGAN_DT_F32, false).mode; }
@@ -1065,9 +1091,39 @@
     return route_gather(gg, prec, in_dtype, out_dtype, false).path != GatherPath::none ? 1 : 0;
 }
 
+int agan_conv_gather_weight_form(const agan_conv_geom* gg, int pack_mode, int prec, int in_dtype, int out_dtype, int epilogue) {
+    const GatherRoute r = route_gather(gg, prec, in_dtype, out_dtype, epilogue != 0);
+    return r.path == GatherPath::winograd ? wino_form_of(r.wino.kind, pack_mode) : pack_mode;
+}
+
+int agan_conv_gather_wino_kind(const agan_conv_geom* gg, int prec, int in_dtype, int out_dtype, int epilogue) {
+    const GatherRoute r = route_gather(gg, prec, in_dtype, out_dtype, epilogue != 0);
+    if (r.path != GatherPath::winograd) return AGAN_WINO_NONE;
+    switch (r.wino.kind) {
+    case WinoKind::conv3x3: return AGAN_WINO_CONV3X3;
+    case WinoKind::conv3x3_half: return AGAN_WINO_CONV3X3_HALF;
+    case WinoKind::conv4x4_s2: return AGAN_WINO_CONV4X4_S2;
+    case WinoKind::dgrad2x2_class: return AGAN_WINO_DGRAD2X2_CLASS;
+    }
+    return AGAN_WINO_NONE;
+}
+
+size_t agan_conv_gather_form_ws_bytes(const agan_conv_geom* g, int prec, int weight_form) {
+    if (!pack_is_wino(weight_form)) return agan_conv_gather_ws_bytes(g, prec);
+    const GatherRoute r = route_gather(g, prec, AGAN_DT_F32, AGAN_DT_F32, false);
+    return r.path == GatherPath::winograd ? r.ws_bytes - r.wino.u_bytes : 0;
+}
+
 int agan_conv_gather_dt(const void* in_v, const void* wkv, const float* bias, void* out_v, const agan_conv_geom* gg, const int32_t* ktable,
                         int prec, int act, const void* lrelu_mask_v, void* ws, size_t ws_bytes, void* stream, const float* in_scale,
                         float* out_amax, int in_dtype, int out_dtype) {
+    return agan_conv_gather_form(in_v, wkv, bias, out_v, gg, ktable, prec, act, lrelu_mask_v, ws, ws_bytes, stream, in_scale, out_amax, in_dtype,
+                                 out_dtype, -1);
+}
+
+int agan_conv_gather_form(const void* in_v, const void* wkv, const float* bias, void* out_v, const agan_conv_geom* gg, const int32_t* ktable,
+                          int prec, int act, const void* lrelu_mask_v, void* ws, size_t ws_bytes, void* stream, const float* in_scale,
+                          float* out_amax, int in_dtype, int out_dtype, int weight_form) {
     if (int e = check_geom(gg)) return e;
     AGAN_REQUIRE(in_v && wkv && out_v && ktable, "conv_gather: null pointer");
     AGAN_REQUIRE(act == AGAN_ACT_NONE || (act == AGAN_ACT_LRELU && gg->Cout > 4),
@@ -1082,7 +1138,11 @@
                  "conv_gather: 16-bit activation storage (%d -> %d) is not available for this geometry / precision %d "
                  "(agan_conv_gather_dt_supported)", in_dtype, out_dtype, prec);
     AGAN_REQUIRE(prec != AGAN_PREC_F16X3 || in_scale != nullptr, "conv_gather: AGAN_PREC_F16X3 needs the operand's agan_absmax_scale pair");
-    if (int e = check_ws("conv_gather", r.ws_bytes, ws, ws_bytes)) return e;
+    const bool wk_is_u = pack_is_wino(weight_form);
+    AGAN_REQUIRE(!wk_is_u || (r.path == GatherPath::winograd && wino_form_of(r.wino.kind, pack_source_mode(weight_form)) == weight_form),
+                 "conv_gather: weight form %d is not what this call consumes (agan_conv_gather_weight_form)", weight_form);
+    const size_t u_bytes = wk_is_u ? 0 : r.wino.u_bytes;
+    if (int e = check_ws("conv_gather", wk_is_u ? r.ws_bytes - r.wino.u_bytes : r.ws_bytes, ws, ws_bytes)) return e;
     const Geom g = make_geom(gg);
     hipStream_t st = as_stream(stream);
     const float* in = static_cast<const float*>(in_v);
@@ -1109,8 +1169,8 @@
             break;
         case GatherPath::winograd:
             slab = r.wino.slab;
-            slabs = reinterpret_cast<const float*>(static_cast<const char*>(ws) + r.wino.u_bytes);
-            e = launch_main(st, r.split, "conv_gather/winograd", [&] { launch_wino(in, wk, static_cast<float*>(out_v), g, r.wino, ws, st); });
+            slabs = reinterpret_cast<const float*>(static_cast<const char*>(ws) + u_bytes);
+            e = launch_main(st, r.split, "conv_gather/winograd", [&] { launch_wino(in, wk, static_cast<float*>(out_v), g, r.wino, ws, st, wk_is_u); });
             break;
         case GatherPath::small_n:
             e = launch_main(st, r.split, "conv_gather/small_n", [&] { launch_gather_small_n(in_v, wk, bias, static_cast<float*>(out_v), g, st, in_dtype); });
diff --git a/attention-gan_amd/csrc/conv_common.h b/attention-gan_amd/csrc/conv_common.h
--- a/attention-gan_amd/csrc/conv_common.h
+++ b/attention-gan_amd/csrc/conv_common.h
@@ -327,7 +327,37 @@
 void launch_wino_wgrad(const float* x, const float* dy, float* part, const Geom& g, const WinoWgradPlan& p, hipStream_t st);
 void launch_wino_wgrad_sum(const float* part, const Geom& g, const WinoWgradPlan& p, float* dw, int accumulate, hipStream_t st);
 WinoPlan plan_wino(const Geom& g);
-void launch_wino(const float* in, const float* wk, float* out, const Geom& g, const WinoPlan& p, void* ws, hipStream_t st);
+void launch_wino(const float* in, const float* wk, float* out, const Geom& g, const WinoPlan& p, void* ws, hipStream_t st, bool wk_is_u = false);
+__host__ __device__ inline bool pack_is_wino(int mode) { return mode >= AGAN_PACK_WINO_FWD && mode <= AGAN_PACK_WINO_S2_UP_DGRAD; }
+__host__ __device__ inline int pack_source_mode(int mode) {
+    switch (mode) {
+        case AGAN_PACK_WINO_FWD: case AGAN_PACK_WINO_S2_FWD: return AGAN_PACK_FWD;
+        case AGAN_PACK_WINO_DGRAD_S1: return AGAN_PACK_DGRAD_S1;
+        case AGAN_PACK_WINO_CLS_DGRAD: return AGAN_PACK_DGRAD_4x4S2;
+        case AGAN_PACK_WINO_S2_UP_DGRAD: return AGAN_PACK_UP_DGRAD;
+    }
+    return mode;
+}
+__host__ __device__ inline int wino_form_dims(int mode, int cout, int cin, int kh, int kw, int& planes, int& Kin, int& N) {
+    switch (mode) {
+        case AGAN_PACK_WINO_FWD: if (kh != 3 || kw != 3) return -1; planes = 16; Kin = cin; N = cout; break;
+        case AGAN_PACK_WINO_DGRAD_S1: if (kh != 3 || kw != 3) return -1; planes = 16; Kin = cout; N = cin; break;
+        case AGAN_PACK_WINO_S2_FWD: if (kh != 4 || kw != 4) return -1; planes = 36; Kin = cin; N = cout; break;
+        case AGAN_PACK_WINO_CLS_DGRAD: if (kh != 4 || kw != 4) return -1; planes = 36; Kin = cout; N = cin; break;
+        case AGAN_PACK_WINO_S2_UP_DGRAD: if (kh != 3 || kw != 3) return -1; planes = 36; Kin = cout; N = cin; break;
+        default: return -1;
+    }
+    return (Kin & 7) ? -1 : 0;
+}
+__host__ __device__ inline int wino_transform_blocks(bool cls, int Kin, int Nld) {
+    const int total = (cls ? 4 : 1) * Kin * Nld, cap = cls ? 4096 : 2048, nb = (total + 255) / 256;
+    return nb < cap ? nb : cap;
+}
+__host__ __device__ inline int wino_form_blocks(int mode, int Kin, int Nld) { return wino_transform_blocks(mode == AGAN_PACK_WINO_CLS_DGRAD, Kin, Nld); }
+inline size_t wino_u_bytes(int planes, int Kin, int Nld) { return ((size_t)planes * (Kin / 8) * Nld * 8 * sizeof(float) + 255) / 256 * 256; }
+int wino_form_of(WinoKind kind, int pack_mode);
+void launch_wino_weight_form(const float* src, float* U, int mode, int Kin, int N, hipStream_t st);
+void launch_wino_weight_jobs(const agan_pack_job* jobs, int njobs, int total_blocks, hipStream_t st);
 int prec_planes(int prec);
 RowsPlan plan_rows_wgrad(const Geom& g, int prec, bool x16, bool y16, bool up = false);
 void launch_rows_wgrad(const void* x, const void* dy, float* part, const Geom& g, const RowsPlan& p, int prec, hipStream_t st,
diff --git a/attention-gan_amd/csrc/conv_wino.hip b/attention-gan_amd/csrc/conv_wino.hip
--- a/attention-gan_amd/csrc/conv_wino.hip
+++ b/attention-gan_amd/csrc/conv_wino.hip
@@ -11,9 +11,9 @@
 
 __device__ __forceinline__ void lds_barrier_w() { asm volatile("s_waitcnt lgkmcnt(0)\n\ts_barrier" ::: "memory"); }
 
-__global__ __launch_bounds__(256) void wino_weight_transform_kernel(const float* __restrict__ wk, float* __restrict__ U, int Kin, int Nld, int N) {
+__device__ __forceinline__ void wino_weight_transform(const float* __restrict__ wk, float* __restrict__ U, int Kin, int Nld, int N, int blk, int nblk) {
     const int total = Kin * Nld;
-    for (int e = blockIdx.x * 256 + threadIdx.x; e < total; e += gridDim.x * 256) {
+    for (int e = blk * 256 + threadIdx.x; e < total; e += nblk * 256) {
         const int n = e % Nld, c = e / Nld;
         float gk[3][3];
 #pragma unroll
@@ -37,6 +37,9 @@
             for (int nu = 0; nu < 4; ++nu) U[((size_t)((xi * 4 + nu) * nch8 + (c >> 3)) * Nld + n) * 8 + (c & 7)] = u[nu];
         }
     }
+}
+__global__ __launch_bounds__(256) void wino_weight_transform_kernel(const float* __restrict__ wk, float* __restrict__ U, int Kin, int Nld, int N) {
+    wino_weight_transform(wk, U, Kin, Nld, N, blockIdx.x, gridDim.x);
 }
 
 struct WinoTraits {
@@ -427,9 +430,9 @@
     }
 }
 
-__global__ __launch_bounds__(256) void wino_cls_weight_transform_kernel(const float* __restrict__ wk, float* __restrict__ U, int Kin, int Nld, int N) {
+__device__ __forceinline__ void wino_cls_weight_transform(const float* __restrict__ wk, float* __restrict__ U, int Kin, int Nld, int N, int blk, int nblk) {
     const int total = 4 * Kin * Nld, nch8 = Kin >> 3;
-    for (int e = blockIdx.x * 256 + threadIdx.x; e < total; e += gridDim.x * 256) {
+    for (int e = blk * 256 + threadIdx.x; e < total; e += nblk * 256) {
         const int n = e % Nld, t1 = e / Nld, c = t1 % Kin, cls = t1 / Kin;
         const float* wc = wk + (size_t)cls * Kin * 4 * Nld;
         float gk[2][2];
@@ -440,10 +443,13 @@
         wino_weights_f22(gk, U + ((size_t)(cls * 9 * nch8 + (c >> 3)) * Nld + n) * 8 + (c & 7), (size_t)nch8 * Nld * 8);
     }
 }
-
-__global__ __launch_bounds__(256) void wino_s2_weight_transform_kernel(const float* __restrict__ wk, float* __restrict__ U, int Kin, int Nld, int N) {
+__global__ __launch_bounds__(256) void wino_cls_weight_transform_kernel(const float* __restrict__ wk, float* __restrict__ U, int Kin, int Nld, int N) {
+    wino_cls_weight_transform(wk, U, Kin, Nld, N, blockIdx.x, gridDim.x);
+}
+
+__device__ __forceinline__ void wino_s2_weight_transform(const float* __restrict__ wk, float* __restrict__ U, int Kin, int Nld, int N, int blk, int nblk) {
     const int total = Kin * Nld, nch8 = Kin >> 3;
-    for (int e = blockIdx.x * 256 + threadIdx.x; e < total; e += gridDim.x * 256) {
+    for (int e = blk * 256 + threadIdx.x; e < total; e += nblk * 256) {
         const int n = e % Nld, c = e / Nld;
 #pragma unroll
         for (int p = 0; p < 2; ++p)
@@ -457,6 +463,27 @@
                 wino_weights_f22(gk, U + ((size_t)((p * 2 + q) * 9 * nch8 + (c >> 3)) * Nld + n) * 8 + (c & 7), (size_t)nch8 * Nld * 8);
             }
     }
+}
+__global__ __launch_bounds__(256) void wino_s2_weight_transform_kernel(const float* __restrict__ wk, float* __restrict__ U, int Kin, int Nld, int N) {
+    wino_s2_weight_transform(wk, U, Kin, Nld, N, blockIdx.x, gridDim.x);
+}
+
+__global__ __launch_bounds__(256) void wino_weight_jobs_kernel(const agan_pack_job* __restrict__ jobs, int njobs) {
+    __shared__ int which;
+    const int b = blockIdx.x;
+    for (int t = threadIdx.x; t < njobs; t += 256) {
+        const int lo = jobs[t].first_block, hi = t + 1 < njobs ? jobs[t + 1].first_block : 0x7fffffff;
+        if (b >= lo && b < hi) which = t;
+    }
+    __syncthreads();
+    const agan_pack_job j = jobs[which];
+    int planes, Kin, N;
+    if (wino_form_dims(j.mode, j.cout, j.cin, j.kh, j.kw, planes, Kin, N)) return;
+    const int Nld = (N + 31) / 32 * 32, blk = b - j.first_block, nblk = wino_form_blocks(j.mode, Kin, Nld);
+    float* U = static_cast<float*>(j.wk);
+    if (j.mode == AGAN_PACK_WINO_CLS_DGRAD) wino_cls_weight_transform(j.w, U, Kin, Nld, N, blk, nblk);
+    else if (j.mode == AGAN_PACK_WINO_FWD || j.mode == AGAN_PACK_WINO_DGRAD_S1) wino_weight_transform(j.w, U, Kin, Nld, N, blk, nblk);
+    else wino_s2_weight_transform(j.w, U, Kin, Nld, N, blk, nblk);
 }
 
 __global__ __launch_bounds__(256, 1) void conv_wino_wgrad_f32_kernel(const float* __restrict__ x, const float* __restrict__ dy, float* __restrict__ part,
@@ -721,30 +748,55 @@
 }
 }
 
-void launch_wino(const float* in, const float* wk, float* out, const Geom& g, const WinoPlan& p, void* ws, hipStream_t st) {
-    float* U = static_cast<float*>(ws);
-    const int total = g.Cin * g.Nld;
-    const dim3 grid(p.mtiles * p.ntiles * p.ksplit * wino_traits(p.kind).classes), tgrid(std::min(cdiv(total, 256), 2048));
+void launch_wino(const float* in, const float* wk, float* out, const Geom& g, const WinoPlan& p, void* ws, hipStream_t st, bool wk_is_u) {
+    float* Uw = static_cast<float*>(ws);
+    const float* U = wk_is_u ? wk : Uw;
+    const dim3 grid(p.mtiles * p.ntiles * p.ksplit * wino_traits(p.kind).classes), tgrid(wino_transform_blocks(false, g.Cin, g.Nld));
     switch (p.kind) {
     case WinoKind::dgrad2x2_class:
-        AGAN_LAUNCH(wino_cls_weight_transform_kernel, dim3(std::min(cdiv(4 * total, 256), 4096)), dim3(256), 0, st, wk, U, g.Cin, g.Nld, g.Cout);
+        if (!wk_is_u) AGAN_LAUNCH(wino_cls_weight_transform_kernel, dim3(wino_transform_blocks(true, g.Cin, g.Nld)), dim3(256), 0, st, wk, Uw, g.Cin, g.Nld, g.Cout);
         launch_gather_kernel<conv_wino_cls_f32_kernel<4>, WinoKind::dgrad2x2_class>(grid, in, U, out, g, p, st);
         break;
     case WinoKind::conv4x4_s2:
-        AGAN_LAUNCH(wino_s2_weight_transform_kernel, tgrid, dim3(256), 0, st, wk, U, g.Cin, g.Nld, g.Cout);
+        if (!wk_is_u) AGAN_LAUNCH(wino_s2_weight_transform_kernel, tgrid, dim3(256), 0, st, wk, Uw, g.Cin, g.Nld, g.Cout);
         launch_gather_kernel<conv_wino_s2_f32_kernel<4>, WinoKind::conv4x4_s2>(
-            grid, in, U, p.ksplit > 1 ? reinterpret_cast<float*>(static_cast<char*>(ws) + p.u_bytes) : out, g, p, st);
+            grid, in, U, p.ksplit > 1 ? reinterpret_cast<float*>(static_cast<char*>(ws) + (wk_is_u ? 0 : p.u_bytes)) : out, g, p, st);
         break;
     case WinoKind::conv3x3_half:
-        AGAN_LAUNCH(wino_weight_transform_kernel, tgrid, dim3(256), 0, st, wk, U, g.Cin, g.Nld, g.Cout);
+        if (!wk_is_u) AGAN_LAUNCH(wino_weight_transform_kernel, tgrid, dim3(256), 0, st, wk, Uw, g.Cin, g.Nld, g.Cout);
         launch_gather_kernel<conv_wino_h_f32_kernel, WinoKind::conv3x3_half>(grid, in, U, out, g, p, st);
         break;
     case WinoKind::conv3x3:
-        AGAN_LAUNCH(wino_weight_transform_kernel, tgrid, dim3(256), 0, st, wk, U, g.Cin, g.Nld, g.Cout);
+        if (!wk_is_u) AGAN_LAUNCH(wino_weight_transform_kernel, tgrid, dim3(256), 0, st, wk, Uw, g.Cin, g.Nld, g.Cout);
         if (p.nf == 4) launch_gather_kernel<conv_wino_f32_kernel<4>, WinoKind::conv3x3>(grid, in, U, out, g, p, st);
         else launch_gather_kernel<conv_wino_f32_kernel<2>, WinoKind::conv3x3>(grid, in, U, out, g, p, st);
         break;
     }
+}
+
+int wino_form_of(WinoKind kind, int pack_mode) {
+    switch (kind) {
+    case WinoKind::conv3x3:
+    case WinoKind::conv3x3_half:
+        return pack_mode == AGAN_PACK_FWD ? AGAN_PACK_WINO_FWD : (pack_mode == AGAN_PACK_DGRAD_S1 ? AGAN_PACK_WINO_DGRAD_S1 : pack_mode);
+    case WinoKind::conv4x4_s2:
+        return pack_mode == AGAN_PACK_FWD ? AGAN_PACK_WINO_S2_FWD : (pack_mode == AGAN_PACK_UP_DGRAD ? AGAN_PACK_WINO_S2_UP_DGRAD : pack_mode);
+    case WinoKind::dgrad2x2_class:
+        return pack_mode == AGAN_PACK_DGRAD_4x4S2 ? AGAN_PACK_WINO_CLS_DGRAD : pack_mode;
+    }
+    return pack_mode;
+}
+
+void launch_wino_weight_form(const float* src, float* U, int mode, int Kin, int N, hipStream_t st) {
+    const int Nld = (N + 31) / 32 * 32;
+    const dim3 grid(wino_form_blocks(mode, Kin, Nld));
+    if (mode == AGAN_PACK_WINO_CLS_DGRAD) AGAN_LAUNCH(wino_cls_weight_transform_kernel, grid, dim3(256), 0, st, src, U, Kin, Nld, N);
+    else if (mode == AGAN_PACK_WINO_FWD || mode == AGAN_PACK_WINO_DGRAD_S1) AGAN_LAUNCH(wino_weight_transform_kernel, grid, dim3(256), 0, st, src, U, Kin, Nld, N);
+    else AGAN_LAUNCH(wino_s2_weight_transform_kernel, grid, dim3(256), 0, st, src, U, Kin, Nld, N);
+}
+
+void launch_wino_weight_jobs(const agan_pack_job* jobs, int njobs, int total_blocks, hipStream_t st) {
+    AGAN_LAUNCH(wino_weight_jobs_kernel, dim3(total_blocks), dim3(256), 0, st, jobs, njobs);
 }
 
 WinoWgradPlan plan_wino_wgrad(const Geom& g) {
diff --git a/include/agan.h b/include/agan.h
--- a/include/agan.h
+++ b/include/agan.h
@@ -47,7 +47,12 @@
     AGAN_PACK_DGRAD_4x4S2 = 2,
     AGAN_PACK_UP_FWD = 3,
     AGAN_PACK_UP_DGRAD = 4,
-    AGAN_PACK_DGRAD_3x3S2 = 5
+    AGAN_PACK_DGRAD_3x3S2 = 5,
+    AGAN_PACK_WINO_FWD = 6,
+    AGAN_PACK_WINO_DGRAD_S1 = 7,
+    AGAN_PACK_WINO_S2_FWD = 8,
+    AGAN_PACK_WINO_CLS_DGRAD = 9,
+    AGAN_PACK_WINO_S2_UP_DGRAD = 10
 };
 
 size_t agan_packed_weight_bytes(int mode, int cout, int cin, int kh, int kw, int prec);
@@ -60,6 +65,9 @@
 int agan_pack_job_blocks(int mode, int cout, int cin, int kh, int kw);
 int agan_pack_job_blocks_prec(int mode, int cout, int cin, int kh, int kw, int prec);
 int agan_pack_weights(const agan_pack_job* jobs, int njobs, int total_blocks, int prec, void* stream);
+int agan_pack_source_mode(int mode);
+int agan_wino_pack_weight(const float* src, void* u, int mode, int cout, int cin, int kh, int kw, void* stream);
+int agan_pack_weights_wino(const agan_pack_job* jobs, int njobs, int total_blocks, void* stream);
 
 size_t agan_conv_ktable_elems(const agan_conv_geom* g);
 int agan_conv_ktable(const agan_conv_geom* g, int32_t* table, void* stream);
@@ -77,6 +85,13 @@
 int agan_conv_gather_dt(const void* in, const void* wk, const float* bias, void* out, const agan_conv_geom* g,
                         const int32_t* ktable, int prec, int act, const void* lrelu_mask, void* ws, size_t ws_bytes, void* stream,
                         const float* in_amax, float* out_amax, int in_dtype, int out_dtype);
+int agan_conv_gather_weight_form(const agan_conv_geom* g, int pack_mode, int prec, int in_dtype, int out_dtype, int epilogue);
+enum { AGAN_WINO_NONE = -1, AGAN_WINO_CONV3X3 = 0, AGAN_WINO_CONV3X3_HALF = 1, AGAN_WINO_CONV4X4_S2 = 2, AGAN_WINO_DGRAD2X2_CLASS = 3 };
+int agan_conv_gather_wino_kind(const agan_conv_geom* g, int prec, int in_dtype, int out_dtype, int epilogue);
+size_t agan_conv_gather_form_ws_bytes(const agan_conv_geom* g, int prec, int weight_form);
+int agan_conv_gather_form(const void* in, const void* wk, const float* bias, void* out, const agan_conv_geom* g,
+                          const int32_t* ktable, int prec, int act, const void* lrelu_mask, void* ws, size_t ws_bytes, void* stream,
+                          const float* in_amax, float* out_amax, int in_dtype, int out_dtype, int weight_form);
 
 #define AGAN_AMAX_SLOT 256
 int agan_absmax(const float* x, size_t n, float* amax_slot, void* stream);
```

After: 1005 images/s (median of 6 runs). About the same (+0.5%).
